# Alisah-Ozcan/HEonGPU

Hardware: AMD Instinct MI355X
Metric: homomorphic mults/sec (CKKS N=2^16, L=16) + NTT GB/s vs HBM roofline (higher is better)
Workload: dtype u64

## Files before the change

heongpu_amd/csrc/cabi.cpp:

```cpp
#include "../../include/hegpu.h"
#include "../../include/hegpu_bench.h"
#include "context.hpp"
#include "host_params.hpp"
#include "ops.hpp"
#include <cmath>
#include "tfhe.hpp"
#include <algorithm>
#include <cerrno>
#include <climits>
#include <mutex>
#include <unordered_map>
#include <vector>
#include <cstring>
#include <sys/random.h>
#include <new>
#include <stdexcept>
#include <string>

using namespace hegpu;

struct hegpu_context {
    Context c;
};

static thread_local std::string g_err;

static int fail(int code, const std::string& msg)
{
    g_err = msg;
    return code;
}

struct DevGuard {
    int prev = -1;
    bool switched = false;
    hipError_t err = hipSuccess;
    explicit DevGuard(int dev)
    {
        if (dev < 0) return;
        if ((err = hipGetDevice(&prev)) != hipSuccess) return;
        if (prev != dev) {
            err = hipSetDevice(dev);
            switched = err == hipSuccess;
        }
    }
    ~DevGuard()
    {
        if (switched) (void) hipSetDevice(prev);
    }
    DevGuard(const DevGuard&) = delete;
    DevGuard& operator=(const DevGuard&) = delete;
};
static int hip_ret(hipError_t e, const char* where)
{
    if (e == hipSuccess) return 0;
    g_err = std::string(where) + ": " + hipGetErrorString(e);
    return (int) e;
}

template <typename F>
static int guarded(F&& f)
{
    try {
        return f();
    } catch (const std::invalid_argument& e) {
        return fail(HEGPU_E_INVALID, e.what());
    } catch (const std::logic_error& e) {
        return fail(HEGPU_E_LOGIC, e.what());
    } catch (const std::runtime_error& e) {
        return fail(HEGPU_E_RUNTIME, e.what());
    } catch (const std::bad_alloc&) {
        return fail(HEGPU_E_RUNTIME, "out of host memory");
    }
}

extern "C" {

const char* hegpu_last_error(void) { return g_err.c_str(); }
const char* hegpu_version(void) { return "hegpu-mi355x 0.1 (gfx950)"; }

static bool coefficient_validator(const int* q, int qn, const int* p, int pn)
{
    int total_p = 0;
    for (int i = 0; i < pn; i++) total_p += p[i];
    int idx = 0;
    for (int g = 0; g < qn / pn; g++) {
        int s = 0;
        for (int j = 0; j < pn; j++) s += q[idx++];
        if (s > total_p) return false;
    }
    int s = 0;
    for (int j = 0; j < qn % pn; j++) s += q[idx++];
    return s <= total_p;
}

static void check_degree(int n, int& n_power)
{
    if (n <= 0 || (n & (n - 1))) throw std::logic_error("Poly modulus degree have to be power of two");
    if (n > 65536 || n < 4096) throw std::logic_error("Poly modulus degree is not supported");
    n_power = 31 - __builtin_clz((unsigned) n);
}

static int finish_create(hegpu_context* h, int scheme, int n_power, uint64_t plain_modulus, int q_count,
                         int p_count, hegpu_context** out)
{
    Context& c = h->c;
    c.scheme = scheme;
    c.n_power = n_power;
    c.Q_size = q_count;
    c.P_size = p_count;
    c.plain_modulus = plain_modulus;
    if (scheme == SCHEME_BFV && plain_modulus < 2) throw std::logic_error("plain modulus is not specified");
    c.build_host();
    c.seed_options_from_env();
    *out = h;
    return 0;
}

int hegpu_context_create(int scheme, int n, const int* qb, int qn, const int* pb, int pn, uint64_t plain_modulus,
                         int sec_level, hegpu_context** out)
{
    return guarded([&]() -> int {
        if (!out) throw std::invalid_argument("null output");
        if (scheme != SCHEME_BFV && scheme != SCHEME_CKKS) throw std::invalid_argument("unknown scheme");
        int n_power;
        check_degree(n, n_power);
        if (pn <= 0 || !pb) throw std::logic_error("log_P_bases_bit_sizes cannot be empty!");
        if (qn <= 0 || !qb) throw std::logic_error("log_Q_bases_bit_sizes cannot be empty!");
        if (!coefficient_validator(qb, qn, pb, pn)) throw std::logic_error("P should be bigger than Q pairs!");
        std::vector<int> bits(qb, qb + qn);
        bits.insert(bits.end(), pb, pb + pn);
        int total = 0;
        for (int b : bits) total += b;
        if (sec_level == HEGPU_SEC_128 || sec_level == HEGPU_SEC_192 || sec_level == HEGPU_SEC_256) {
            if (host::max_logq((u64) n, sec_level) < total)
                throw std::runtime_error("Parameters do not align with the security recommendations "
                                         "provided by the lattice-estimator");
        } else if (sec_level != HEGPU_SEC_NONE) {
            throw std::runtime_error("Invalid security level");
        }
        hegpu_context* h = new hegpu_context();
        try {
            h->c.primes = host::find_primes((u64) n, bits);
            return finish_create(h, scheme, n_power, plain_modulus, qn, pn, out);
        } catch (...) {
            delete h;
            throw;
        }
    });
}

int hegpu_context_create_default(int scheme, int n, int p_count, uint64_t plain_modulus, int sec_level,
                                 hegpu_context** out)
{
    return guarded([&]() -> int {
        if (!out) throw std::invalid_argument("null output");
        if (scheme != SCHEME_BFV && scheme != SCHEME_CKKS) throw std::invalid_argument("unknown scheme");
        int n_power;
        check_degree(n, n_power);
        if (p_count < 1) throw std::logic_error("P_modulus_size cannot be lower than 1!");
        if (sec_level != HEGPU_SEC_128 && sec_level != HEGPU_SEC_192 && sec_level != HEGPU_SEC_256)
            throw std::runtime_error("Invalid security level");
        std::vector<u64> chain = host::default_chain((u64) n, sec_level);
        if (chain.empty() || (int) chain.size() <= p_count) throw std::logic_error("no default chain");
        hegpu_context* h = new hegpu_context();
        try {
            h->c.primes = chain;
            return finish_create(h, scheme, n_power, plain_modulus, (int) chain.size() - p_count, p_count, out);
        } catch (...) {
            delete h;
            throw;
        }
    });
}

int hegpu_context_create_from_primes(int scheme, int n, const uint64_t* primes, int qn, int pn,
                                     uint64_t plain_modulus, hegpu_context** out)
{
    return guarded([&]() -> int {
        if (!out || !primes) throw std::invalid_argument("null argument");
        if (scheme != SCHEME_BFV && scheme != SCHEME_CKKS) throw std::invalid_argument("unknown scheme");
        int n_power;
        check_degree(n, n_power);
        if (pn <= 0 || qn <= 0) throw std::logic_error("log_P_bases_bit_sizes cannot be empty!");
        for (int i = 0; i < qn + pn; i++) {
            if (primes[i] >> 61) throw std::logic_error("invalid modulus bit size");
            if ((primes[i] - 1) % (2 * (u64) n)) throw std::logic_error("no sufficient root unity");
        }
        hegpu_context* h = new hegpu_context();
        try {
            h->c.primes.assign(primes, primes + qn + pn);
            return finish_create(h, scheme, n_power, plain_modulus, qn, pn, out);
        } catch (...) {
            delete h;
            throw;
        }
    });
}

int hegpu_validate_coeff_modulus_values(int n, const uint64_t* primes, int qn, int pn, int sec_level)
{
    return guarded([&]() -> int {
        if (!primes) throw std::invalid_argument("null argument");
        int n_power;
        check_degree(n, n_power);
        if (pn <= 0) throw std::logic_error("log_P_bases_bit_sizes cannot be empty!");
        if (qn <= 0) throw std::logic_error("log_Q_bases_bit_sizes cannot be empty!");
        std::vector<int> bits;
        int total = 0;
        for (int i = 0; i < qn + pn; i++) {
            if (primes[i] < 2 || primes[i] >> 61) throw std::logic_error("invalid modulus bit size");
            if ((primes[i] - 1) % (2 * (u64) n)) throw std::logic_error("no sufficient root unity");
            bits.push_back(64 - __builtin_clzll(primes[i]));
            total += bits.back();
        }
        if (!coefficient_validator(bits.data(), qn, bits.data() + qn, pn))
            throw std::logic_error("Invalid parameters, P should be bigger than Q pairs!");
        if (sec_level == HEGPU_SEC_128 || sec_level == HEGPU_SEC_192 || sec_level == HEGPU_SEC_256) {
            if (host::max_logq((u64) n, sec_level) < total)
                throw std::runtime_error("Parameters do not align with the security recommendations "
                                         "provided by the lattice-estimator");
        } else if (sec_level != HEGPU_SEC_NONE) {
            throw std::runtime_error("Invalid security level");
        }
        return 0;
    });
}

void hegpu_context_destroy(hegpu_context* ctx) { delete ctx; }

int hegpu_context_set_option(hegpu_context* ctx, const char* name, int value)
{
    if (!ctx || !name) return fail(HEGPU_E_INVALID, "null argument");
    switch (ctx->c.set_option(name, value)) {
        case 0: return 0;
        case 1: return fail(HEGPU_E_INVALID, std::string("unknown option: ") + name);
        case 2: return fail(HEGPU_E_INVALID, std::string("value out of range for option ") + name);
        default: return fail(HEGPU_E_LOGIC, std::string("option ") + name + " must be set before hegpu_context_upload");
    }
}

int hegpu_context_get_option(const hegpu_context* ctx, const char* name, int* value)
{
    if (!ctx || !name || !value) return fail(HEGPU_E_INVALID, "null argument");
    if (ctx->c.get_option(name, value)) return fail(HEGPU_E_INVALID, std::string("unknown option: ") + name);
    return 0;
}

int hegpu_context_upload(hegpu_context* ctx)
{
    if (!ctx) return fail(HEGPU_E_INVALID, "null context");
    int cnt = 0;
    if (hipGetDeviceCount(&cnt) != hipSuccess || cnt == 0) {
        (void) hipGetLastError();
        return fail(HEGPU_E_NODEVICE, "no HIP device available: the HIP backend cannot run (no CPU fallback)");
    }
    return hip_ret(ctx->c.upload(), "context upload");
}

int hegpu_context_upload_device(hegpu_context* ctx, int device)
{
    if (!ctx) return fail(HEGPU_E_INVALID, "null context");
    int cnt = 0;
    if (hipGetDeviceCount(&cnt) != hipSuccess || cnt == 0) {
        (void) hipGetLastError();
        return fail(HEGPU_E_NODEVICE, "no HIP device available: the HIP backend cannot run (no CPU fallback)");
    }
    if (device < 0 || device >= cnt) return fail(HEGPU_E_INVALID, "no such device");
    if (ctx->c.uploaded)
        return ctx->c.device == device ? 0 : fail(HEGPU_E_LOGIC, "the context is already uploaded to another device");
    DevGuard g(device);
    return hip_ret(ctx->c.upload(), "context upload");
}

int hegpu_context_device(const hegpu_context* ctx) { return (ctx && ctx->c.uploaded) ? ctx->c.device : -1; }

int hegpu_context_clone(const hegpu_context* src, hegpu_context** out)
{
    return guarded([&]() -> int {
        if (!src || !out) throw std::invalid_argument("null argument");
        hegpu_context* h = new hegpu_context();
        Context& c = h->c;
        const Context& s = src->c;
        c.scheme = s.scheme; c.n_power = s.n_power; c.n = s.n;
        c.Q_size = s.Q_size; c.P_size = s.P_size; c.Qp_size = s.Qp_size; c.bsk_size = s.bsk_size;
        c.plain_modulus = s.plain_modulus; c.primes = s.primes; c.host = s.host;
        c.m2_levels = s.m2_levels; c.m2_width = s.m2_width;
        c.fused_row_mac = s.fused_row_mac; c.fused_moddown = s.fused_moddown; c.col_multi = s.col_multi;
        c.single_pass = s.single_pass; c.ntt_galois = s.ntt_galois; c.galois_scatter = s.galois_scatter;
        c.digit_split = s.digit_split; c.copy_along = s.copy_along; c.fuse_inverse = s.fuse_inverse;
        c.fp_ntt = s.fp_ntt; c.behz_split = s.behz_split; c.fused_tensor = s.fused_tensor;
        *out = h;
        return 0;
    });
}

static thread_local int g_bcast_path = 0;
int hegpu_last_broadcast_path(void) { return g_bcast_path; }

static const size_t kBcastChunk = (size_t) 32 << 20;

static int peer_edge(int src, int dst, hipError_t* e)
{
    if (src == dst) return 1;
    int can = 0;
    if ((*e = hipDeviceCanAccessPeer(&can, dst, src)) != hipSuccess) return -1;
    if (!can) return 0;
    DevGuard g(dst);
    if (g.err != hipSuccess) {
        *e = g.err;
        return -1;
    }
    const hipError_t en = hipDeviceEnablePeerAccess(src, 0);
    if (en != hipSuccess && en != hipErrorPeerAccessAlreadyEnabled) {
        *e = en;
        return -1;
    }
    (void) hipGetLastError();
    return 1;
}

int hegpu_broadcast_bytes(const int* devices, int n, void* const* bufs, size_t bytes, const hegpu_stream* streams,
                          int* path_out)
{
    g_bcast_path = 0;
    if (path_out) *path_out = 0;
    if (!devices || !bufs || n < 1) return fail(HEGPU_E_INVALID, "null argument");
    int cnt = 0;
    if (hipGetDeviceCount(&cnt) != hipSuccess || cnt == 0) {
        (void) hipGetLastError();
        return fail(HEGPU_E_NODEVICE, "no HIP device available: the HIP backend cannot run (no CPU fallback)");
    }
    for (int i = 0; i < n; i++) {
        if (!bufs[i]) return fail(HEGPU_E_INVALID, "null buffer");
        if (devices[i] < 0 || devices[i] >= cnt) return fail(HEGPU_E_INVALID, "no such device");
    }
    if (n == 1 || bytes == 0) return 0;
    hipError_t e = hipSuccess;
    bool flat = true, same = true;
    for (int j = 1; j < n && flat; j++) {
        const int r = peer_edge(devices[0], devices[j], &e);
        if (r < 0) return hip_ret(e, "hegpu_broadcast: peer access");
        flat = r == 1;
    }
    for (int j = 1; j < n; j++) same = same && devices[j] == devices[0];
    std::vector<int> parent(n, 0);
    bool staged = false;
    if (!flat) {
        for (int span = 1; span < n; span <<= 1)
            for (int i = 0; i < span && i + span < n; i++) parent[i + span] = i;
        for (int j = 1; j < n; j++) {
            const int r = peer_edge(devices[parent[j]], devices[j], &e);
            if (r < 0) return hip_ret(e, "hegpu_broadcast: peer access");
            staged = staged || r == 0;
        }
    }
    const size_t nchunks = (bytes + kBcastChunk - 1) / kBcastChunk;
    auto stream_of = [&](int i) { return streams ? (hipStream_t) streams[i] : (hipStream_t) nullptr; };
    std::vector<hipEvent_t> events;
    auto mark = [&](int i, hipEvent_t* ev) {
        DevGuard g(devices[i]);
        if ((e = g.err) != hipSuccess) return;
        if ((e = hipEventCreateWithFlags(ev, hipEventDisableTiming)) != hipSuccess) return;
        events.push_back(*ev);
        e = hipEventRecord(*ev, stream_of(i));
    };
    std::vector<std::vector<hipEvent_t>> arrived(n, std::vector<hipEvent_t>(nchunks, nullptr));
    hipEvent_t src_ready = nullptr;
    mark(0, &src_ready);
    for (size_t c = 0; c < nchunks; c++) arrived[0][c] = src_ready;
    for (size_t c = 0; c < nchunks && e == hipSuccess; c++) {
        const size_t off = c * kBcastChunk, len = std::min(kBcastChunk, bytes - off);
        for (int j = 1; j < n && e == hipSuccess; j++) {
            const int pj = parent[j];
            DevGuard g(devices[j]);
            if ((e = g.err) != hipSuccess) break;
            if ((e = hipStreamWaitEvent(stream_of(j), arrived[pj][c], 0)) != hipSuccess) break;
            if ((e = hipMemcpyPeerAsync((char*) bufs[j] + off, devices[j], (const char*) bufs[pj] + off, devices[pj], len,
                                        stream_of(j))) != hipSuccess)
                break;
            bool has_child = false;
            for (int k = j + 1; k < n; k++) has_child = has_child || parent[k] == j;
            if (has_child) mark(j, &arrived[j][c]);
        }
    }
    for (hipEvent_t ev : events) (void) hipEventDestroy(ev);
    if (e != hipSuccess) return hip_ret(e, "hegpu_broadcast");
    int path = flat ? HEGPU_BCAST_FLAT : HEGPU_BCAST_TREE;
    if (staged) path |= HEGPU_BCAST_STAGED;
    if (same) path |= HEGPU_BCAST_SAME_DEVICE;
    g_bcast_path = path;
    if (path_out) *path_out = path;
    return 0;
}

int hegpu_broadcast_key(hegpu_context* const* ctxs, int n_ctx, uint64_t* const* keys, size_t elems,
                        const hegpu_stream* streams)
{
    g_bcast_path = 0;
    if (!ctxs || !keys || n_ctx < 1) return fail(HEGPU_E_INVALID, "null argument");
    std::vector<int> devs(n_ctx);
    std::vector<void*> bufs(n_ctx);
    for (int i = 0; i < n_ctx; i++) {
        if (!ctxs[i] || !keys[i]) return fail(HEGPU_E_INVALID, "null context or key pointer");
        if (!ctxs[i]->c.uploaded) return fail(HEGPU_E_LOGIC, "every context must be uploaded (hegpu_context_upload_device)");
        devs[i] = ctxs[i]->c.device;
        bufs[i] = keys[i];
    }
    return hegpu_broadcast_bytes(devs.data(), n_ctx, bufs.data(), elems * sizeof(u64), streams, nullptr);
}

long hegpu_context_int(const hegpu_context* ctx, const char* name)
{
    if (!ctx || !name) return -1;
    const Context& c = ctx->c;
    if (!strcmp(name, "n_power")) return c.n_power;
    if (!strcmp(name, "n")) return (long) c.n;
    if (!strcmp(name, "Q_size")) return c.Q_size;
    if (!strcmp(name, "P_size")) return c.P_size;
    if (!strcmp(name, "Q_prime_size")) return c.Qp_size;
    if (!strcmp(name, "bsk_modulus")) return c.bsk_size;
    if (!strcmp(name, "scheme")) return c.scheme;
    if (!strcmp(name, "max_logq_128")) return host::max_logq_128((int) c.n);
    if (!strcmp(name, "max_logq_192")) return host::max_logq(c.n, 192);
    if (!strcmp(name, "max_logq_256")) return host::max_logq(c.n, 256);
    return -1;
}

long hegpu_context_get(const hegpu_context* ctx, const char* name, uint64_t* out, long cap)
{
    if (!ctx || !name) return -1;
    auto it = ctx->c.host.find(name);
    if (it == ctx->c.host.end()) return -1;
    const long cnt = (long) it->second.size();
    if (!out) return cnt;
    if (cnt > cap) return -2;
    memcpy(out, it->second.data(), cnt * sizeof(uint64_t));
    return cnt;
}

const void* hegpu_context_device_ptr(const hegpu_context* ctx, const char* name)
{
    if (!ctx || !name) return nullptr;
    auto it = ctx->c.dev.find(name);
    return it == ctx->c.dev.end() ? nullptr : it->second;
}

int hegpu_steps_to_galois_elt(int steps, int coeff_count, int group_order)
{
    int elt = -1;
    (void) guarded([&]() -> int {
        elt = host::steps_to_galois_elt(steps, coeff_count, group_order);
        return 0;
    });
    return elt;
}

#define NEED_CTX(ctx)                                                                      \
    if (!(ctx)) return fail(HEGPU_E_INVALID, "null context");                              \
    if (!(ctx)->c.uploaded) {                                                              \
        int r__ = hegpu_context_upload(ctx);                                               \
        if (r__) return r__;                                                               \
    }                                                                                      \
    DevGuard dev_guard__((ctx)->c.device);                                                 \
    if (dev_guard__.err != hipSuccess) return hip_ret(dev_guard__.err, "switching to the context's device")

static const Mod* mods_of(const Context& c, int table_set)
{
    return table_set == HEGPU_TABLES_Q_BSK ? c.plan_merge.mods : c.plan_qp.mods;
}

int hegpu_ntt(hegpu_context* ctx, int table_set, const uint64_t* in, uint64_t* out, int inverse, int batch,
              int mod_count, int mod_offset, const int* mod_order, const int* poly_order, hegpu_stream stream)
{
    NEED_CTX(ctx);
    const Context& c = ctx->c;
    if (table_set == HEGPU_TABLES_Q_BSK && c.scheme != SCHEME_BFV)
        return fail(HEGPU_E_INVALID, "q|Bsk tables exist only in a BFV context");
    if (table_set < 0 || table_set > HEGPU_TABLES_PLAIN || (table_set == HEGPU_TABLES_PLAIN && !c.plan_plain.count))
        return fail(HEGPU_E_INVALID, "no such table set in this context");
    NttArgs a = c.ntt_args(table_set);
    const int avail = a.mod_count;
    if (mod_count <= 0 || mod_offset < 0 || (!mod_order && mod_offset + mod_count > avail))
        return fail(HEGPU_E_INVALID, "modulus range outside the table set");
    a.in = (const u64*) in;
    a.out = (u64*) out;
    a.mod_count = mod_count;
    a.mod_offset = mod_offset;
    a.mod_order = mod_order;
    a.poly_order = poly_order;
    return hip_ret(ntt_launch(a, batch, inverse != 0, (hipStream_t) stream), "hegpu_ntt");
}

int hegpu_GPU_NTT(hegpu_context* ctx, int table_set, const uint64_t* in, uint64_t* out, int mod_offset, int batch,
                  int mod_count, hegpu_stream stream)
{
    return hegpu_ntt(ctx, table_set, in, out, 0, batch, mod_count, mod_offset, nullptr, nullptr, stream);
}
int hegpu_GPU_NTT_Inplace(hegpu_context* ctx, int table_set, uint64_t* inout, int mod_offset, int batch, int mod_count,
                          hegpu_stream stream)
{
    return hegpu_ntt(ctx, table_set, inout, inout, 0, batch, mod_count, mod_offset, nullptr, nullptr, stream);
}
int hegpu_GPU_INTT(hegpu_context* ctx, int table_set, const uint64_t* in, uint64_t* out, int mod_offset, int batch,
                   int mod_count, hegpu_stream stream)
{
    return hegpu_ntt(ctx, table_set, in, out, 1, batch, mod_count, mod_offset, nullptr, nullptr, stream);
}
int hegpu_GPU_INTT_Inplace(hegpu_context* ctx, int table_set, uint64_t* inout, int mod_offset, int batch,
                           int mod_count, hegpu_stream stream)
{
    return hegpu_ntt(ctx, table_set, inout, inout, 1, batch, mod_count, mod_offset, nullptr, nullptr, stream);
}
int hegpu_GPU_NTT_Modulus_Ordered_Inplace(hegpu_context* ctx, int table_set, uint64_t* inout, int inverse,
                                          int mod_offset, int batch, int mod_count, const int* order,
                                          hegpu_stream stream)
{
    if (!order) return fail(HEGPU_E_INVALID, "modulus order table is required");
    return hegpu_ntt(ctx, table_set, inout, inout, inverse, batch, mod_count, mod_offset, order, nullptr, stream);
}
int hegpu_GPU_NTT_Poly_Ordered_Inplace(hegpu_context* ctx, int table_set, uint64_t* inout, int inverse, int mod_offset,
                                       int batch, int mod_count, const int* order, hegpu_stream stream)
{
    if (!order) return fail(HEGPU_E_INVALID, "polynomial order table is required");
    return hegpu_ntt(ctx, table_set, inout, inout, inverse, batch, mod_count, mod_offset, nullptr, order, stream);
}

int hegpu_addition(hegpu_context* ctx, const uint64_t* in1, const uint64_t* in2, uint64_t* out, int limbs,
                   int parts, int batch, int op, hegpu_stream stream)
{
    NEED_CTX(ctx);
    const Context& c = ctx->c;
    if (limbs <= 0 || limbs > c.Qp_size || op < 0 || op > 2) return fail(HEGPU_E_INVALID, "bad limbs/op");
    return hip_ret(rns_addition((const u64*) in1, (const u64*) in2, (u64*) out, c.plan_qp.mods, c.n_power, limbs,
                                parts, batch, op, (hipStream_t) stream),
                   "hegpu_addition");
}

int hegpu_cross_multiplication(hegpu_context* ctx, int table_set, const uint64_t* in1, uint64_t s1,
                               const uint64_t* in2, uint64_t s2, uint64_t* out, uint64_t so, int decomp_size,
                               int batch, hegpu_stream stream)
{
    NEED_CTX(ctx);
    const Context& c = ctx->c;
    const Mod* m = mods_of(c, table_set);
    if (!m) return fail(HEGPU_E_INVALID, "table set not available");
    return hip_ret(rns_cross_multiplication((const u64*) in1, s1, (const u64*) in2, s2, (u64*) out, so, m, c.n_power,
                                            decomp_size, batch, (hipStream_t) stream),
                   "hegpu_cross_multiplication");
}

int hegpu_cipher_broadcast(hegpu_context* ctx, const uint64_t* in, uint64_t in_stride, uint64_t* out,
                           uint64_t out_stride, int digits, int nmods, int split, int level, int batch,
                           hegpu_stream stream)
{
    NEED_CTX(ctx);
    const Context& c = ctx->c;
    return hip_ret(rns_decompose((const u64*) in, in_stride, (u64*) out, out_stride, c.plan_qp.mods, c.n_power,
                                 digits, nmods, split, level, batch, (hipStream_t) stream),
                   "hegpu_cipher_broadcast");
}

int hegpu_keyswitch_multiply_accumulate(hegpu_context* ctx, const uint64_t* in, uint64_t in_stride,
                                        const uint64_t* key, uint64_t* out, uint64_t out_stride, int digits,
                                        int nmods, int key_limbs, int split, int level, int batch,
                                        hegpu_stream stream)
{
    NEED_CTX(ctx);
    const Context& c = ctx->c;
    return hip_ret(rns_keyswitch_mac((const u64*) in, in_stride, (const u64*) key, (u64*) out, out_stride,
                                     c.plan_qp.mods, c.n_power, digits, nmods, key_limbs, split, level, batch,
                                     (hipStream_t) stream),
                   "hegpu_keyswitch_multiply_accumulate");
}

int hegpu_base_conversion_DtoQtilde(hegpu_context* ctx, const uint64_t* in, uint64_t in_stride, uint64_t* out,
                                    uint64_t out_stride, int depth, int batch, hegpu_stream stream)
{
    NEED_CTX(ctx);
    const Context& c = ctx->c;
    if (c.P_size < 2) return fail(HEGPU_E_LOGIC, "method II tables exist only when P_size > 1");
    if (depth < 0 || depth >= (int) c.m2_levels.size()) return fail(HEGPU_E_INVALID, "invalid depth");
    const Context::M2Level& L = c.m2_levels[depth];
    return hip_ret(rns_base_conversion_DtoQtilde((const u64*) in, in_stride, (u64*) out, out_stride, c.plan_qp.mods,
                                                 c.d64("m2_matrix_mg") + L.off_matrix, c.d64("m2_Mi_inv") + L.off_mi,
                                                 c.d64("m2_negprod_mg") + L.off_prod, c.d32("m2_I_j") + L.off_digits,
                                                 c.d32("m2_I_location") + L.off_digits, c.n_power, L.d, L.rc,
                                                 c.Q_size - depth, depth, c.m2_width, batch, (hipStream_t) stream),
                   "hegpu_base_conversion_DtoQtilde");
}

int hegpu_divide_round_lastq(hegpu_context* ctx, const uint64_t* in, uint64_t in_stride, const uint64_t* ct,
                             uint64_t ct_stride, uint64_t* out, uint64_t out_stride, int switchkey, int batch,
                             hegpu_stream stream)
// ... 1074 lines not shown
```

heongpu_amd/csrc/context.cpp:

```cpp
#include "context.hpp"
#include <cerrno>
#include <climits>
#include <cstdlib>
#include "host_params.hpp"
#include <algorithm>
#include <cmath>
#include <cstdlib>
#include <cstring>
#include <stdexcept>

namespace hegpu {

using host::inv_mod_prime;
using host::mul_mod;

typedef std::vector<u64> vec;

static void append(vec& dst, const vec& src) { dst.insert(dst.end(), src.begin(), src.end()); }

void Context::build_host()
{
    n = ((u64) 1) << n_power;
    Qp_size = Q_size + P_size;
    const int Q = Q_size, P = P_size, Qp = Qp_size;
// ... 386 lines not shown
                loc.push_back(brev((pos - 1) >> 1));
                pos = (pos * 3) & (m - 1);
            }
            for (u64 i = n / 2; i < n; i++) {
                loc.push_back(brev((m - pos - 1) >> 1));
                pos = (pos * 3) & (m - 1);
            }
            host["encoding_location"] = loc;
        }

        {
            u64 Q_mod_t = 1;
            for (int i = 0; i < Q; i++) Q_mod_t = mul_mod(Q_mod_t, primes[i] % t, t);
            host["Q_mod_t"] = vec{Q_mod_t};
            host["upper_threshold"] = vec{(t + 1) >> 1};
            vec inc;
            for (int i = 0; i < Q; i++) inc.push_back(primes[i] - t);
            host["upper_halfincrement"] = inc;
            std::vector<u64> big{1};
            for (int i = 0; i < Q; i++) {
                unsigned __int128 carry = 0;
                for (u64& w : big) {
                    unsigned __int128 v = (unsigned __int128) w * primes[i] + carry;
                    w = (u64) v;
                    carry = v >> 64;
                }
                if (carry) big.push_back((u64) carry);
            }
            {
                unsigned __int128 rem = 0;
                for (size_t k = big.size(); k-- > 0;) {
                    unsigned __int128 cur = (rem << 64) | big[k];
                    big[k] = (u64) (cur / t);
                    rem = cur % t;
                }
            }
            vec cdiv;
            for (int i = 0; i < Q; i++) {
                unsigned __int128 rem = 0;
                for (size_t k = big.size(); k-- > 0;) rem = ((rem << 64) | big[k]) % primes[i];
                cdiv.push_back((u64) rem);
            }
            host["coeff_div_plain_modulus"] = cdiv;
            vec Qi_t, Qi_gamma, Qi_inverse;
            for (int i = 0; i < Q; i++) {
                u64 a = 1, b = 1, c = 1;
                for (int j = 0; j < Q; j++)
                    if (j != i) {
                        a = mul_mod(a, primes[j] % t, t);
                        b = mul_mod(b, primes[j] % gamma, gamma);
                        c = mul_mod(c, inv_mod_prime(primes[j] % primes[i], primes[i]), primes[i]);
                    }
                Qi_t.push_back(a);
                Qi_gamma.push_back(b);
                Qi_inverse.push_back(c);
            }
            host["Qi_t"] = Qi_t;
            host["Qi_gamma"] = Qi_gamma;
            host["Qi_inverse"] = Qi_inverse;
            u64 mt_ = 1, mg_ = 1;
            for (int i = 0; i < Q; i++) {
                mt_ = mul_mod(mt_, inv_mod_prime(primes[i] % t, t), t);
                mg_ = mul_mod(mg_, inv_mod_prime(primes[i] % gamma, gamma), gamma);
            }
            host["mulq_inv_t"] = vec{t - mt_};
            host["mulq_inv_gamma"] = vec{gamma - mg_};
            host["inv_gamma"] = vec{inv_mod_prime(gamma % t, t)};
        }
    }
}

template <typename T>
static hipError_t to_device(const std::vector<T>& h, T** d)
{
    *d = nullptr;
    if (h.empty()) return hipSuccess;
    hipError_t e = hipMalloc((void**) d, h.size() * sizeof(T));
    if (e != hipSuccess) return e;
    return hipMemcpy(*d, h.data(), h.size() * sizeof(T), hipMemcpyHostToDevice);
}

static hipError_t build_plan(NttPlan& p, const vec& mods, const vec& fwd, const vec& inv, const vec& ninv,
                             int n_power, bool fp_on)
{
    const u64 n = ((u64) 1) << n_power;
    const int cnt = (int) mods.size();
    std::vector<Mod> hm(cnt);
    std::vector<ulonglong2> htw((size_t) cnt * n), hitw((size_t) cnt * n), hn(cnt), hw(cnt);
    const u64 rows = n / 256, perB = rows * 15 * 16;
    std::vector<ulonglong2> htwB((size_t) cnt * perB), hitwB((size_t) cnt * perB);
    std::vector<double> htwB8((size_t) cnt * perB, 0.0);
    for (int k = 0; k < cnt; k++) {
        const u64 q = mods[k];
        hm[k] = make_mod(q);
        static_assert(FP_MAX_MODULUS_BITS == 50, "the bounds in fpmod.cuh, ntt.hip and tests/fp_model.py are derived for q < 2^50");
        hm[k].fp = (fp_on && hm[k].bit <= FP_MAX_MODULUS_BITS && (q >> FP_MAX_MODULUS_BITS) == 0) ? 1 : 0;
        for (u64 j = 0; j < n; j++) {
            const u64 w = fwd[k * n + j], iw = inv[k * n + j];
            if (hm[k].fp) {
                const double wd = (double) w, wi = wd / (double) q;
                u64 a, b;
                memcpy(&a, &wd, 8);
                memcpy(&b, &wi, 8);
                htw[k * n + j] = make_ulonglong2(a, b);
            } else {
                htw[k * n + j] = make_ulonglong2(w, shoup_companion(w, q));
            }
            if (hm[k].fp) {
                const double wd = (double) iw, wi = wd / (double) q;
                u64 a, b;
                memcpy(&a, &wd, 8);
                memcpy(&b, &wi, 8);
                hitw[k * n + j] = make_ulonglong2(a, b);
            } else {
                hitw[k * n + j] = make_ulonglong2(iw, shoup_companion(iw, q));
            }
        }
        for (u64 c = 0; c < rows; c++)
            for (int st = 0; st < 4; st++)
                for (int b = 0; b < (1 << st); b++)
                    for (int j = 0; j < 16; j++) {
                        const u64 src = ((((rows + c) * 16 + j) << st) + b);
                        const u64 dst = k * perB + (c * 15 + ((1 << st) - 1 + b)) * 16 + j;
                        htwB[dst] = htw[k * n + src];
                        hitwB[dst] = hitw[k * n + src];
                        if (hm[k].fp) htwB8[dst] = (double) fwd[k * n + src];
                    }
        const u64 w1n = host::mul_mod(inv[k * n + 1], ninv[k], q);
        if (hm[k].fp) {
            auto pair = [&](u64 v) {
                const double vd = (double) v, vi = vd / (double) q;
                u64 a, b;
                memcpy(&a, &vd, 8);
                memcpy(&b, &vi, 8);
                return make_ulonglong2(a, b);
            };
            hn[k] = pair(ninv[k]);
            hw[k] = pair(w1n);
        } else {
            hn[k] = make_ulonglong2(ninv[k], shoup_companion(ninv[k], q));
            hw[k] = make_ulonglong2(w1n, shoup_companion(w1n, q));
        }
    }
    p.count = cnt;
    p.has_fp = p.has_int = 0;
    for (int k = 0; k < cnt; k++) (hm[k].fp ? p.has_fp : p.has_int) = 1;
    p.fp.assign(cnt, 0);
    for (int k = 0; k < cnt; k++) p.fp[k] = hm[k].fp ? 1 : 0;
    u64 qmax = 0;
    for (int k = 0; k < cnt; k++) qmax = mods[k] > qmax ? mods[k] : qmax;
    p.lazy_q_max = (~0ull - 2 * qmax) / (4ull * (u64) n_power);
    hipError_t e;
    if ((e = to_device(hm, &p.mods)) != hipSuccess) return e;
    if ((e = to_device(htw, &p.tw)) != hipSuccess) return e;
    if ((e = to_device(hitw, &p.itw)) != hipSuccess) return e;
    if ((e = to_device(htwB, &p.twB)) != hipSuccess) return e;
    if ((e = to_device(hitwB, &p.itwB)) != hipSuccess) return e;
    if ((e = to_device(htwB8, &p.twB8)) != hipSuccess) return e;
    if ((e = to_device(hn, &p.ninv)) != hipSuccess) return e;
    return to_device(hw, &p.w1ninv);
}

static void free_plan(NttPlan& p)
{
    if (p.mods) (void) hipFree(p.mods);
    if (p.tw) (void) hipFree(p.tw);
    if (p.itw) (void) hipFree(p.itw);
    if (p.twB) (void) hipFree(p.twB);
    if (p.itwB) (void) hipFree(p.itwB);
    if (p.twB8) (void) hipFree(p.twB8);
    if (p.ninv) (void) hipFree(p.ninv);
    if (p.w1ninv) (void) hipFree(p.w1ninv);
    p = NttPlan();
}

hipError_t Context::upload()
{
    if (uploaded) return hipSuccess;
    for (int k = 0; k < DRBG_GAUSS_MAX; k++)
        gauss_cdt.t[k] = (u64) (erf(((double) k + 0.5) / (3.2 * 1.4142135623730951)) * 9223372036854775808.0);
    hipError_t e = hipGetDevice(&device);
    if (e != hipSuccess) return e;
    if ((e = build_plan(plan_qp, host["modulus"], host["ntt_table"], host["intt_table"], host["n_inverse"],
                        n_power, fp_ntt)) != hipSuccess)
        return e;
    static const char* u64_tables[] = {"psi_half",
                                       "last_q_modinv",
                                       "half",
                                       "half_mod",
                                       "factor",
                                       "m2_md_W0",
                                       "m2_md_G",
                                       "m2_md_C",
                                       "rescaled_last_q_modinv",
                                       "rescaled_half_mod",
                                       "rescaled_half",
                                       "base_change_matrix_Bsk",
                                       "inv_punctured_prod_mod_base_array",
                                       "base_change_matrix_m_tilde",
                                       "inv_m_tilde_mod_Bsk",
                                       "prod_q_mod_Bsk",
                                       "inv_prod_q_mod_Bsk",
                                       "base_change_matrix_q",
                                       "base_change_matrix_msk",
                                       "inv_punctured_prod_mod_B_array",
                                       "behz_mtilde_inv_punct",
                                       "behz_t_inv_punct",
                                       "behz_invq_inv_punct_B",
                                       "behz_msk_mod_q",
                                       "behz_fc_matrix",
                                       "behz_fc_c1",
                                       "behz_ff_matrix",
                                       "behz_ff_tc",
                                       "behz_ff_q_matrix",
                                       "behz_ff_msk_matrix",
                                       "behz_ff_prod_B",
                                       "behz_ff_neg_prod_B",
                                       "prod_B_mod_q",
                                       "Mi",
                                       "Mi_inv",
                                       "upper_half_threshold",
                                       "decryption_modulus",
                                       "special_fft_roots_table",
                                       "special_ifft_roots_table",
                                       "coeff_div_plain_modulus",
                                       "upper_halfincrement",
                                       "Qi_t",
                                       "Qi_gamma",
                                       "Qi_inverse",
                                       "m2_Mi_inv",
                                       "m2_matrix",
                                       "m2_prod",
                                       "m2_matrix_mg",
                                       "m2_negprod_mg"};
    for (const char* nm : u64_tables) {
        auto it = host.find(nm);
        if (it == host.end()) continue;
        u64* d = nullptr;
        if ((e = to_device(it->second, &d)) != hipSuccess) return e;
        dev[nm] = d;
    }
    for (const char* nm : {"new_prime_locations", "new_input_locations", "m2_I_j", "m2_I_location", "encoding_location",
                           "reverse_order"}) {
        auto it = host.find(nm);
        if (it == host.end()) continue;
        std::vector<int> v(it->second.begin(), it->second.end());
        int* d = nullptr;
        if ((e = to_device(v, &d)) != hipSuccess) return e;
        dev[nm] = d;
    }
    if (scheme == SCHEME_BFV) {
        if ((e = build_plan(plan_merge, host["q_Bsk_merge_modulus"], host["q_Bsk_merge_ntt_tables"],
                            host["q_Bsk_merge_intt_tables"], host["q_Bsk_n_inverse"], n_power, fp_ntt)) != hipSuccess)
            return e;
        if (host.count("plain_modulus2") &&
            (e = build_plan(plan_plain, host["plain_modulus2"], host["plain_ntt_tables"], host["plain_intt_tables"],
                            host["n_plain_inverse"], n_power, fp_ntt)) != hipSuccess)
            return e;
        behz.ibase = plan_merge.mods;
        behz.obase = plan_merge.mods + Q_size;
        behz.m_tilde = make_mod(((u64) 1) << 32);
        behz.plain = make_mod(plain_modulus);
        behz.inv_prod_q_mod_m_tilde = host["inv_prod_q_mod_m_tilde"][0];
        behz.inv_prod_B_mod_m_sk = host["inv_prod_B_mod_m_sk"][0];
        behz.inv_m_tilde_mod_Bsk = d64("inv_m_tilde_mod_Bsk");
        behz.prod_q_mod_Bsk = d64("prod_q_mod_Bsk");
        behz.base_change_matrix_Bsk = d64("base_change_matrix_Bsk");
        behz.base_change_matrix_m_tilde = d64("base_change_matrix_m_tilde");
        behz.inv_punctured_prod_mod_base_array = d64("inv_punctured_prod_mod_base_array");
        behz.inv_prod_q_mod_Bsk = d64("inv_prod_q_mod_Bsk");
        behz.inv_punctured_prod_mod_B_array = d64("inv_punctured_prod_mod_B_array");
        behz.base_change_matrix_q = d64("base_change_matrix_q");
        behz.base_change_matrix_msk = d64("base_change_matrix_msk");
        behz.prod_B_mod_q = d64("prod_B_mod_q");
        behz.mtilde_inv_punct = d64("behz_mtilde_inv_punct");
        behz.t_inv_punct = d64("behz_t_inv_punct");
        behz.invq_inv_punct_B = d64("behz_invq_inv_punct_B");
        behz.msk_mod_q = d64("behz_msk_mod_q");
        behz.fc_matrix = d64("behz_fc_matrix");
        behz.fc_c1 = d64("behz_fc_c1");
        behz.ff_matrix = d64("behz_ff_matrix");
        behz.ff_tc = d64("behz_ff_tc");
        behz.ff_q_matrix = d64("behz_ff_q_matrix");
        behz.ff_msk_matrix = d64("behz_ff_msk_matrix");
        behz.ff_prod_B = d64("behz_ff_prod_B");
        behz.ff_neg_prod_B = d64("behz_ff_neg_prod_B");
        behz.ibase_size = Q_size;
        behz.obase_size = bsk_size;
        behz.split = behz_split;
    }
    uploaded = true;
    return hipDeviceSynchronize();
}

namespace {
struct OptDesc { const char* name; const char* env; int lo, hi; };
const OptDesc kOptions[] = {
    {"fused_row_mac", "HEGPU_FUSED_ROW_MAC", -1, 1}, {"fused_moddown", "HEGPU_FUSED_MODDOWN", 0, 1},
    {"col_multi", "HEGPU_COL_MULTI", -1, 1},         {"single_pass", "HEGPU_SINGLE_PASS", -1, 1},
    {"ntt_galois", "HEGPU_NTT_GALOIS", 0, 1},        {"galois_scatter", "HEGPU_GALOIS_SCATTER", 0, 1},
    {"fuse_inverse", "HEGPU_FUSE_INVERSE", 0, 1},    {"copy_along", "HEGPU_COPY_ALONG", 0, 1},
    {"digit_split", "HEGPU_DIGIT_SPLIT", -1, 4},     {"fp_ntt", "HEGPU_FP_NTT", 0, 1},
    {"behz_split", "HEGPU_BEHZ_SPLIT", -1, 1},       {"fused_tensor", "HEGPU_FUSED_TENSOR", 0, 1},
};
}

int Context::set_option(const char* name, int value)
{
    if (!name) return 1;
    const OptDesc* d = nullptr;
    for (const OptDesc& o : kOptions)
        if (!strcmp(o.name, name)) d = &o;
    if (!d) return 1;
    if (value < d->lo || value > d->hi) return 2;
    const std::string nm(name);
    if (nm == "fp_ntt") {
        if (uploaded) return 3;
        fp_ntt = value != 0;
    } else if (nm == "fused_row_mac") fused_row_mac = value;
    else if (nm == "fused_moddown") fused_moddown = value != 0;
    else if (nm == "col_multi") col_multi = value;
    else if (nm == "single_pass") single_pass = value;
    else if (nm == "ntt_galois") ntt_galois = value != 0;
    else if (nm == "galois_scatter") galois_scatter = value != 0;
    else if (nm == "fuse_inverse") fuse_inverse = value != 0;
    else if (nm == "copy_along") copy_along = value != 0;
    else if (nm == "fused_tensor") fused_tensor = value != 0;
    else if (nm == "digit_split") {
        if (value == 1 || value == 3) return 2;
        digit_split = value;
    } else if (nm == "behz_split") {
        behz_split = value;
        behz.split = value;
    }
    return 0;
}

int Context::get_option(const char* name, int* value) const
{
    if (!name || !value) return 1;
    const std::string nm(name);
    if (nm == "fp_ntt") *value = fp_ntt;
    else if (nm == "fused_row_mac") *value = fused_row_mac;
    else if (nm == "fused_moddown") *value = fused_moddown;
    else if (nm == "col_multi") *value = col_multi;
    else if (nm == "single_pass") *value = single_pass;
    else if (nm == "ntt_galois") *value = ntt_galois;
    else if (nm == "galois_scatter") *value = galois_scatter;
    else if (nm == "fuse_inverse") *value = fuse_inverse;
    else if (nm == "copy_along") *value = copy_along;
    else if (nm == "fused_tensor") *value = fused_tensor;
    else if (nm == "digit_split") *value = digit_split;
    else if (nm == "behz_split") *value = behz_split;
    else return 1;
    return 0;
}

bool env_long(const char* name, long* out)
{
    const char* e = getenv(name);
    if (!e || !*e) return false;
    char* end = nullptr;
    errno = 0;
    const long v = strtol(e, &end, 10);
    if (errno || end == e || *end) return false;
    *out = v;
    return true;
}

void Context::seed_options_from_env()
{
    for (const OptDesc& o : kOptions) {
        long v;
        if (env_long(o.env, &v) && v >= INT_MIN && v <= INT_MAX)
            (void) set_option(o.name, (int) v);
    }
}

void Context::release_device()
{
    free_plan(plan_qp);
    free_plan(plan_merge);
    free_plan(plan_plain);
    for (auto& kv : dev)
        if (kv.second) (void) hipFree(kv.second);
    dev.clear();
    uploaded = false;
}

Context::~Context()
{
    if (uploaded) release_device();
}

const u64* Context::d64(const char* name) const
{
    auto it = dev.find(name);
    return it == dev.end() ? nullptr : (const u64*) it->second;
}
const int* Context::d32(const char* name) const
{
    auto it = dev.find(name);
    return it == dev.end() ? nullptr : (const int*) it->second;
}

NttArgs Context::ntt_args(int table_set) const
{
    const NttPlan& p = table_set == 2 ? plan_plain : (table_set ? plan_merge : plan_qp);
    NttArgs a{};
    a.mods = p.mods;
    a.tw = p.tw;
    a.itw = p.itw;
    a.twB = p.twB;
    a.itwB = p.itwB;
    a.twB8 = p.twB8;
    a.ninv = p.ninv;
    a.w1ninv = p.w1ninv;
    a.n_power = n_power;
    a.mod_count = p.count;
    a.col_multi = col_multi;
    a.single_pass = single_pass;
    a.plan_has_fp = p.has_fp;
    a.plan_has_int = p.has_int;
    a.lazy_q_max = p.lazy_q_max;
    return a;
}

}
```

heongpu_amd/csrc/context.hpp:

```cpp
#pragma once
#include "modarith.cuh"
#include "ntt.hpp"
#include "rns.hpp"
#include <map>
#include <string>
#include "drbg.hpp"
#include <vector>

namespace hegpu {

bool env_long(const char* name, long* out);


enum Scheme { SCHEME_BFV = 1, SCHEME_CKKS = 2 };

struct NttPlan {
    Mod* mods = nullptr;
    ulonglong2* tw = nullptr;
    ulonglong2* itw = nullptr;
    ulonglong2* twB = nullptr;
    ulonglong2* itwB = nullptr;
    double* twB8 = nullptr;
    ulonglong2* ninv = nullptr;
    ulonglong2* w1ninv = nullptr;
    int count = 0;
    int has_fp = 0, has_int = 0;
    std::vector<unsigned char> fp;
    u64 lazy_q_max = 0;
};

struct Context {
    int scheme = 0;
    int n_power = 0;
    u64 n = 0;
    int Q_size = 0, P_size = 0, Qp_size = 0;
    int bsk_size = 0;
    u64 plain_modulus = 0;
    std::vector<u64> primes;
    std::map<std::string, std::vector<u64>> host;
    struct M2Level {
        int d = 0, rc = 0;
        int off_digits = 0;
        int off_mi = 0;
        int off_matrix = 0;
        int off_prod = 0;
    };
    std::vector<M2Level> m2_levels;
    int m2_width = 0;
    int fused_row_mac = -1;
    bool fused_moddown = true;
    int col_multi = -1;
    int single_pass = -1;
    bool ntt_galois = true;
    bool galois_scatter = true;
    int digit_split = -1;
    bool copy_along = true;
    bool fuse_inverse = true;
    bool fused_tensor = true;
    bool fp_ntt = true;
    int behz_split = -1;
    void seed_options_from_env();
    int set_option(const char* name, int value);
    int get_option(const char* name, int* value) const;
    GaussCdt gauss_cdt{};

    bool uploaded = false;
    int device = -1;
    NttPlan plan_qp;
    NttPlan plan_merge;
    NttPlan plan_plain;
    std::map<std::string, void*> dev;
    Mod* bsk_mods = nullptr;
    BehzDev behz{};

    ~Context();
    void build_host();
    hipError_t upload();
    void release_device();

    const u64* d64(const char* name) const;
    const std::vector<u64>& h64(const char* name) const { return host.at(name); }
    const int* d32(const char* name) const;
    NttArgs ntt_args(int table_set) const;
};

}
```

heongpu_amd/csrc/ntt.hip:

```cpp
#include "ntt.hpp"
#define HEGPU_FP_TU ntt
#include "fpmod.cuh"

namespace hegpu {

#define NTT_THREADS 256

#ifdef NTT_ABLATION_HEADER
#include NTT_ABLATION_HEADER
#else
__device__ __forceinline__ u64 gld(const u64* p) { return *p; }
__device__ __forceinline__ void gst(u64* p, u64 v) { *p = v; }
#define NTT_ABLATE_BFLY(x, y, w)
#define NTT_ABLATE_FPBFLY(x, y, w)
#define NTT_ABLATE_TW(load, root0, s) (load)
#define NTT_FP_TW(t, i, c) ((t)[i])
#endif

__device__ __forceinline__ u64 csub(u64 x, u64 m) { return (x >= m) ? x - m : x; }

typedef unsigned long long u64x2_t __attribute__((ext_vector_type(2)));
struct ConstTw {
    const u64x2_t __attribute__((address_space(4)))* p;
    __device__ __forceinline__ ulonglong2 operator[](u32 i) const
// ... 15 lines not shown
#pragma clang diagnostic push
#pragma clang diagnostic ignored "-Wold-style-cast"
    return *(const int __attribute__((address_space(4)))*) p;
#pragma clang diagnostic pop
}
__device__ __forceinline__ Mod ld_const_mod(const Mod* p)
{
#pragma clang diagnostic push
#pragma clang diagnostic ignored "-Wold-style-cast"
    const u64 __attribute__((address_space(4)))* w = (const u64 __attribute__((address_space(4)))*) reinterpret_cast<const u64*>(p);
#pragma clang diagnostic pop
    static_assert(sizeof(Mod) == 56, "seven words");
    Mod m;
    m.q = w[0];
    m.mu = w[1];
    m.r_hi = w[2];
    m.r_lo = w[3];
    m.r64 = w[4];
    m.qinv = w[5];
    const u64 bf = w[6];
    m.bit = (u32) bf;
    m.fp = (u32) (bf >> 32);
    return m;
}

__device__ __forceinline__ void fp_ct_bfly(double& x, double& y, ulonglong2 w, const FC& c)
{
    NTT_ABLATE_FPBFLY(x, y, w);
    const double t = fp_mul(y, as_f64(w.x), as_f64(w.y), c);
    y = x - t;
    x = x + t;
    FP_AUDIT_VAL(c, FPM_SUM, x);
    FP_AUDIT_VAL(c, FPM_SUM, y);
}
struct FpSched { unsigned before; bool at_end; };
#define FP_STAGE_GROW(b) (1.25 * (b) + 0.5)
#define FP_BOUND_LIMIT 7.9
#define FP_HANDOVER 0.51
#define FP_UNREDUCED_IN 1.05
constexpr FpSched fp_sched(int stages, double b_in, double b_out_max)
{
    unsigned m = 0;
    double b = b_in;
    for (int s = 0; s < stages; s++) {
        if (FP_STAGE_GROW(b) > FP_BOUND_LIMIT) {
            m |= 1u << s;
            b = 0.5;
        }
        b = FP_STAGE_GROW(b);
    }
    return FpSched{m, b > b_out_max};
}
template <int LOGR, typename TW>
__device__ __forceinline__ void fp_ct_radix(double (&x)[1 << LOGR], TW tw, u32 root0,
                                            const FC& c, unsigned before, bool at_end)
{
#pragma unroll
    for (int s = 0; s < LOGR; s++) {
        FP_STAGE(c, 31 - __builtin_clz(root0) + s);
        if ((before >> s) & 1u) {
#pragma unroll
            for (int k = 0; k < (1 << LOGR); k++) x[k] = fp_reduce(x[k], c);
        }
        const int half = (1 << LOGR) >> (s + 1);
#pragma unroll
        for (int b = 0; b < (1 << s); b++) {
            const ulonglong2 w = NTT_ABLATE_TW(NTT_FP_TW(tw, (root0 << s) + b, c), root0, s);
#pragma unroll
            for (int j = 0; j < half; j++) fp_ct_bfly(x[b * 2 * half + j], x[b * 2 * half + j + half], w, c);
        }
    }
    FP_STAGE(c, 31 - __builtin_clz(root0) + LOGR);
    if (at_end) {
#pragma unroll
        for (int k = 0; k < (1 << LOGR); k++) x[k] = fp_reduce(x[k], c);
    }
}
template <int S1> struct FpColSched {
    static constexpr FpSched s = fp_sched(S1, FP_UNREDUCED_IN, FP_HANDOVER);
    static constexpr unsigned a_before = s.before & ((1u << (S1 - 4)) - 1u);
    static constexpr unsigned b_before = (s.before >> (S1 - 4)) & 15u;
    static constexpr bool b_at_end = s.at_end;
};
__device__ __forceinline__ void fp_ct_radix16_tb(double (&x)[16], const ulonglong2* __restrict__ tb, const FC& c)
{
#pragma unroll
    for (int s = 0; s < 4; s++) {
        const int half = 8 >> s;
        if (s > 0) FP_STAGE(c, (c).stage + 1);
#pragma unroll
        for (int b = 0; b < (1 << s); b++) {
            const ulonglong2 w = NTT_ABLATE_TW(NTT_FP_TW(tb, ((1 << s) - 1 + b) * 16, c), (u32) b, s);
#pragma unroll
            for (int j = 0; j < half; j++) fp_ct_bfly(x[b * 2 * half + j], x[b * 2 * half + j + half], w, c);
        }
    }
    FP_STAGE(c, (c).stage + 1);
#pragma unroll
    for (int k = 0; k < 16; k++) x[k] = fp_canon(x[k], c);
}

__device__ __forceinline__ void fp_ct_radix16_tb8(double (&x)[16], const double* __restrict__ tb, const FC& c)
{
#pragma unroll
    for (int s = 0; s < 4; s++) {
        const int half = 8 >> s;
        if (s > 0) __builtin_amdgcn_sched_barrier(0);
        if (s > 0) FP_STAGE(c, (c).stage + 1);
#pragma unroll
        for (int b = 0; b < (1 << s); b++) {
            const double wd = tb[((1 << s) - 1 + b) * 16];
            const ulonglong2 w = make_ulonglong2(as_bits(wd), as_bits(wd * c.qi));
#pragma unroll
            for (int j = 0; j < half; j++) fp_ct_bfly(x[b * 2 * half + j], x[b * 2 * half + j + half], w, c);
        }
    }
    FP_STAGE(c, (c).stage + 1);
#pragma unroll
    for (int k = 0; k < 16; k++) x[k] = fp_canon(x[k], c);
}

struct QC {
    u64 q;
    u64 q4;
    u32 nq0, nq1;
};
__device__ __forceinline__ QC make_qc(u64 q)
{
    QC c;
    c.q = q;
    c.q4 = 4 * q;
    u64 nq = 0 - q;
    c.nq0 = (u32) nq;
    c.nq1 = (u32) (nq >> 32);
    return c;
}

__device__ __forceinline__ u64 shoup_lazy(u64 y, ulonglong2 w, const QC& c)
{
    const u32 y0 = (u32) y, y1 = (u32) (y >> 32);
    const u32 w0 = (u32) w.x, w1 = (u32) (w.x >> 32), p0 = (u32) w.y, p1 = (u32) (w.y >> 32);
    const u64 A = (u64) y0 * p1;
    const u64 B = (u64) y1 * p0 + (u32) A;
    const u64 qh = (u64) y1 * p1 + (A >> 32) + (B >> 32);
    const u32 h0 = (u32) qh, h1 = (u32) (qh >> 32);
    u64 acc = (u64) y0 * w0;
    acc += (u64) h0 * c.nq0;
    const u32 hi = y0 * w1 + y1 * w0 + h0 * c.nq1 + h1 * c.nq0;
    return acc + ((u64) hi << 32);
}

__device__ __forceinline__ u64 shoup_full(u64 y, ulonglong2 w, const QC& c)
{
    u64 r = shoup_lazy(y, w, c);
    r = csub(r, 2 * c.q);
    return csub(r, c.q);
}

template <bool LAZY>
__device__ __forceinline__ void ct_bfly(u64& x, u64& y, ulonglong2 w, const QC& c)
{
    NTT_ABLATE_BFLY(x, y, w);
    u64 u = LAZY ? x : csub(x, c.q4);
    u64 t = shoup_lazy(y, w, c);
    x = u + t;
    y = u + c.q4 - t;
}

__device__ __forceinline__ void gs_bfly(u64& x, u64& y, ulonglong2 w, const QC& c)
{
    NTT_ABLATE_BFLY(x, y, w);
    u64 s = x + y;
    u64 d = x + c.q4 - y;
    x = csub(s, c.q4);
    y = shoup_lazy(d, w, c);
}

template <int LOGR, bool LAZY, typename TW>
__device__ __forceinline__ void ct_radix(u64 (&x)[1 << LOGR], TW tw,
                                         u32 root0, const QC& c)
{
#pragma unroll
    for (int s = 0; s < LOGR; s++) {
        const int half = (1 << LOGR) >> (s + 1);
#pragma unroll
        for (int b = 0; b < (1 << s); b++) {
            ulonglong2 w = NTT_ABLATE_TW(tw[(root0 << s) + b], root0, s);
#pragma unroll
            for (int j = 0; j < half; j++)
                ct_bfly<LAZY>(x[b * 2 * half + j], x[b * 2 * half + j + half], w, c);
        }
    }
}

template <bool LAZY>
__device__ __forceinline__ void ct_radix16_tb(u64 (&x)[16], const ulonglong2* __restrict__ tb, const QC& c)
{
#pragma unroll
    for (int s = 0; s < 4; s++) {
        const int half = 8 >> s;
#pragma unroll
        for (int b = 0; b < (1 << s); b++) {
            ulonglong2 w = tb[((1 << s) - 1 + b) * 16];
#pragma unroll
            for (int j = 0; j < half; j++)
                ct_bfly<LAZY>(x[b * 2 * half + j], x[b * 2 * half + j + half], w, c);
        }
    }
}

template <int LOGR>
__device__ __forceinline__ void gs_radix(u64 (&x)[1 << LOGR], const ulonglong2* __restrict__ tw,
                                         u32 root0, const QC& c)
{
#pragma unroll
    for (int s = LOGR - 1; s >= 0; s--) {
        const int half = (1 << LOGR) >> (s + 1);
#pragma unroll
        for (int b = 0; b < (1 << s); b++) {
            ulonglong2 w = NTT_ABLATE_TW(tw[(root0 << s) + b], root0, s);
#pragma unroll
            for (int j = 0; j < half; j++)
                gs_bfly(x[b * 2 * half + j], x[b * 2 * half + j + half], w, c);
        }
    }
}

__device__ __forceinline__ void gs_radix16_tb(u64 (&x)[16], const ulonglong2* __restrict__ tb, const QC& c)
{
#pragma unroll
    for (int s = 3; s >= 0; s--) {
        const int half = 8 >> s;
#pragma unroll
        for (int b = 0; b < (1 << s); b++) {
            ulonglong2 w = tb[((1 << s) - 1 + b) * 16];
#pragma unroll
            for (int j = 0; j < half; j++)
                gs_bfly(x[b * 2 * half + j], x[b * 2 * half + j + half], w, c);
        }
    }
}

template <int LOGR>
__device__ __forceinline__ void gs_radix_last(u64 (&x)[1 << LOGR], const ulonglong2* __restrict__ tw,
                                              u32 root0, ulonglong2 ninv, ulonglong2 w1ninv, const QC& c)
{
#pragma unroll
    for (int s = LOGR - 1; s >= 1; s--) {
        const int half = (1 << LOGR) >> (s + 1);
#pragma unroll
        for (int b = 0; b < (1 << s); b++) {
            ulonglong2 w = NTT_ABLATE_TW(tw[(root0 << s) + b], root0, s);
#pragma unroll
            for (int j = 0; j < half; j++)
                gs_bfly(x[b * 2 * half + j], x[b * 2 * half + j + half], w, c);
        }
    }
    const int half = (1 << LOGR) >> 1;
#pragma unroll
    for (int j = 0; j < half; j++) {
        u64 s = x[j] + x[j + half];
        u64 d = x[j] + c.q4 - x[j + half];
        x[j] = shoup_full(s, ninv, c);
        x[j + half] = shoup_full(d, w1ninv, c);
    }
}

struct PolySel {
    u64 in_off, out_off;
    int mod;
    int digit;
    int item, j;
};

__device__ __forceinline__ int udiv16(int x, unsigned magic)
{
    return magic ? (int) __umulhi((unsigned) x, magic) : x;
}

__device__ __forceinline__ PolySel select_poly(const NttArgs& a, int poly)
{
    PolySel s;
    if (a.group_span) {
        const int k = udiv16(poly, a.mg_group_span), r = poly - k * a.group_span;
        if (a.polys_per_item) {
            const int per_item = udiv16(a.polys_per_item, a.mg_mod_count);
            const int it = udiv16(r, a.mg_per_item), d = r - it * per_item;
            poly = it * a.polys_per_item + d * a.mod_count + k;
        } else {
            poly = r * a.mod_count + k;
        }
    }
    int item = 0, j = poly;
    if (a.polys_per_item) {
        item = udiv16(poly, a.mg_polys_per_item);
        j = poly - item * a.polys_per_item;
    }
    int k = j - udiv16(j, a.mg_mod_count) * a.mod_count;
    if (a.mod_order) k = a.mod_order[k];
    s.mod = a.mod_offset + k;
    u64 slot = a.poly_order ? (u64) a.poly_order[j] : (u64) j;
    s.digit = a.decomp_mods ? udiv16(j, a.mg_decomp_mods) : -1;
    u64 in_slot = a.decomp_mods ? (u64) s.digit * (a.decomp_in_mul ? a.decomp_in_mul : 1) + a.decomp_in_add : slot;
    s.in_off = (u64) item * a.in_item_stride + (in_slot << a.n_power);
    s.out_off = (u64) item * a.out_item_stride + (slot << a.n_power);
    s.item = item;
    s.j = j;
    return s;
}

__device__ __forceinline__ int col_phys(int e) { return e ^ (((e >> 8) & 1) << 4); }
__device__ __forceinline__ int row_phys(int e) { return e ^ (((e >> 5) & 7) << 1); }

__device__ __forceinline__ void wave_lds_fence()
{
    __builtin_amdgcn_fence(__ATOMIC_RELEASE, "wavefront");
    __builtin_amdgcn_wave_barrier();
    __builtin_amdgcn_fence(__ATOMIC_ACQUIRE, "wavefront");
}

#define COL_LDS_ELEMS 4096
#define ROW_LDS_ELEMS 4096

__device__ __forceinline__ bool fwd_stages_lazy(const Mod& md, u64 lazy_q_max) { return md.q <= lazy_q_max; }
#define NTT_ROW_LAZY_MAX_Q 0x0666666666666666ull
__device__ __forceinline__ bool row_stages_lazy(const Mod& md, u64 lazy_q_max) { return md.q <= lazy_q_max || md.q <= NTT_ROW_LAZY_MAX_Q; }

template <int S1, bool DECOMP, bool LAZY, bool SREG = false>
__device__ __forceinline__ void fwd_col_body(const NttArgs& a, const PolySel& ps, const Mod& md, u64* lds,
                                             const u64* sreg = nullptr)
{
    constexpr int R = 1 << S1;
    constexpr int CT = 4096 / R;
    constexpr int NSA = S1 - 4;
    constexpr int RA = 1 << NSA;
    constexpr int G = 16 / RA;
    const int t = threadIdx.x;
    const QC qc = make_qc(md.q);
    const ulonglong2* __restrict__ tw = a.tw + ((u64) ps.mod << a.n_power);
    const u64* __restrict__ src = a.in + ps.in_off + blockIdx.x * CT;
    u64* __restrict__ dst = a.out + ps.out_off + blockIdx.x * CT;

    const u64 half_qP = a.half_on ? a.mods[a.half_src_mod].q : 0;
    const u64 half_hm = a.half_on ? a.half_mod[ps.mod] : 0;
    u64 x[16];
    const int col = t % CT, r1 = t / CT;
    u64 v[16];
    if constexpr (NSA > 0) {
#pragma unroll
        for (int g = 0; g < G; g++) {
            const int L = t + NTT_THREADS * g;
            const int c = L % CT, rb = L / CT;
#pragma unroll
            for (int k = 0; k < RA; k++) v[g * RA + k] = SREG ? sreg[g * RA + k] : gld(&src[(u64) (rb + 16 * k) * 256 + c]);
        }
    } else {
#pragma unroll
        for (int k = 0; k < 16; k++) v[k] = SREG ? sreg[k] : gld(&src[(u64) k * 256 + col]);
    }
    if (DECOMP && a.half_on) {
#pragma unroll
        for (int k = 0; k < 16; k++) v[k] = sub_mod(reduce64(add_mod(v[k], a.half, half_qP), md), half_hm, md.q);
    } else if (DECOMP && !LAZY && a.mods[ps.digit].q > 8 * md.q) {
#pragma unroll
        for (int k = 0; k < 16; k++) v[k] = reduce64(v[k], md);
    }
    if constexpr (NSA > 0) {
#pragma unroll
        for (int g = 0; g < G; g++) {
            const int L = t + NTT_THREADS * g;
            const int c = L % CT, rb = L / CT;
            u64 y[RA];
#pragma unroll
            for (int k = 0; k < RA; k++) y[k] = v[g * RA + k];
            ct_radix<NSA, LAZY>(y, tw, 1u, qc);
#pragma unroll
            for (int k = 0; k < RA; k++) lds[col_phys((rb + 16 * k) * CT + c)] = y[k];
        }
        __syncthreads();
#pragma unroll
        for (int k = 0; k < 16; k++) x[k] = lds[col_phys((16 * r1 + k) * CT + col)];
        if (SREG) __syncthreads();
    } else {
#pragma unroll
        for (int k = 0; k < 16; k++) x[k] = v[k];
    }
    ct_radix<4, LAZY>(x, tw, (u32) (RA + r1), qc);
#pragma unroll
    for (int k = 0; k < 16; k++) gst(&dst[(u64) (16 * r1 + k) * 256 + col], x[k]);
}

template <int S1, bool DECOMP, bool WIDE, bool SREG = false>
__device__ __forceinline__ void fwd_col_body_fp(const NttArgs& a, const PolySel& ps, const Mod& md, u64* lds,
                                                ulonglong2* twl, const u64* sreg = nullptr)
{
    constexpr int R = 1 << S1;
    constexpr int CT = 4096 / R;
    constexpr int NSA = S1 - 4;
    constexpr int RA = 1 << NSA;
    constexpr int G = 16 / RA;
    const int t = threadIdx.x;
    const FC fc = make_fc(md.q, FP_SITE(DECOMP ? FPS_FWD_COL_DECOMP : FPS_FWD_COL, S1 - 4));
    const ulonglong2* __restrict__ tw = a.tw + ((u64) ps.mod << a.n_power);
    const u64* __restrict__ src = a.in + ps.in_off + blockIdx.x * CT;
    u64* __restrict__ dst = a.out + ps.out_off + blockIdx.x * CT;

    double c32 = 0.0, c32i = 0.0;
    if constexpr (DECOMP && WIDE) {
        c32 = (double) reduce64(1ull << 32, md);
        c32i = c32 * fc.qi;
    }
    const u64 half_qP = (DECOMP && a.half_on) ? a.mods[a.half_src_mod].q : 0;
    const double half_hm = (DECOMP && a.half_on) ? fp_from_u64(a.half_mod[ps.mod]) : 0.0;
    const bool in_small = S1 != 7 && DECOMP && !WIDE && !a.half_on && a.mods[ps.digit].q <= md.q + (md.q >> 6);
    typedef FpColSched<S1> CS;
    auto load_all = [&](auto& y, auto addr, int si0) {
        constexpr int CNT = sizeof(y) / sizeof(y[0]);
        FP_STAGE(fc, FP_STAGE_INPUT);
        if constexpr (SREG && !WIDE) {
            if (in_small) {
#pragma unroll
                for (int k = 0; k < CNT; k++) y[k] = as_f64(sreg[si0 + k]);
            } else {
#pragma unroll
                for (int k = 0; k < CNT; k++) y[k] = fp_reduce(as_f64(sreg[si0 + k]), fc);
            }
        } else {
            u64 v[CNT];
#pragma unroll
            for (int k = 0; k < CNT; k++) {
                v[k] = SREG ? sreg[si0 + k] : *addr(k);
                if constexpr (SREG) asm volatile("" : "+v"(v[k]));
            }
            if (!SREG && DECOMP && a.half_on) {
#pragma unroll
                for (int k = 0; k < CNT; k++) v[k] = add_mod(v[k], a.half, half_qP);
            }
#pragma unroll
            for (int k = 0; k < CNT; k++) {
                if constexpr (DECOMP && WIDE) y[k] = fp_mul(fp_from_u32((u32) (v[k] >> 32)), c32, c32i, fc) + fp_from_u32((u32) v[k]);
                else if constexpr (DECOMP) y[k] = in_small ? fp_from_u64(v[k]) : fp_reduce(fp_from_u64(v[k]), fc);
                else y[k] = fp_from_u64(v[k]);
            }
        }
        if (DECOMP && a.half_on) {
#pragma unroll
            for (int k = 0; k < CNT; k++) y[k] = fp_reduce(y[k] - half_hm, fc);
        }
#pragma unroll
        for (int k = 0; k < CNT; k++) FP_AUDIT_VAL(fc, FPM_SUM, y[k]);
    };

    double x[16];
    const int col = t % CT, r1 = t / CT;
    if constexpr (NSA > 0) {
        const ulonglong2 mine = tw[t];
#pragma unroll
        for (int g = 0; g < G; g++) {
            const int L = t + NTT_THREADS * g;
            const int c = L % CT, rb = L / CT;
            double y[RA];
            load_all(y, [&](int k) { return &src[(u64) (rb + 16 * k) * 256 + c]; }, g * RA);
            if constexpr (SREG) fp_ct_radix<NSA>(y, const_tw(tw), 1u, fc, CS::a_before, false);
            else fp_ct_radix<NSA>(y, tw, 1u, fc, CS::a_before, false);
#pragma unroll
            for (int k = 0; k < RA; k++) lds[col_phys((rb + 16 * k) * CT + c)] = as_bits(y[k]);
        }
        twl[t] = mine;
        __syncthreads();
#pragma unroll
        for (int k = 0; k < 16; k++) x[k] = as_f64(lds[col_phys((16 * r1 + k) * CT + col)]);
        if (SREG) __syncthreads();
        fp_ct_radix<4>(x, twl, (u32) (RA + r1), fc, CS::b_before, CS::b_at_end);
    } else {
        load_all(x, [&](int k) { return &src[(u64) k * 256 + col]; }, 0);
        fp_ct_radix<4>(x, tw, (u32) (RA + r1), fc, CS::b_before, CS::b_at_end);
    }
#pragma unroll
    for (int k = 0; k < 16; k++) {
        if constexpr (SREG) __builtin_nontemporal_store(as_bits(x[k]), &dst[(u64) (16 * r1 + k) * 256 + col]);
        else dst[(u64) (16 * r1 + k) * 256 + col] = as_bits(x[k]);
    }
}

template <int S1, bool DECOMP>
__global__ __launch_bounds__(NTT_THREADS) void ntt_fwd_col(NttArgs a)
{
    __shared__ u64 lds[(S1 > 4) ? COL_LDS_ELEMS : 1];
    __shared__ ulonglong2 twl[(S1 > 4) ? 256 : 1];
    int poly = blockIdx.y;
    if (DECOMP && a.only_int && a.int_slot_count > 0) {
        const int cnt = a.int_slot_count, digits = a.polys_per_item / a.decomp_mods;
        const int per_item = digits * cnt;
        const int item = poly / per_item, r = poly - item * per_item;
        const int digit = r / cnt, w = r - digit * cnt;
        poly = item * a.polys_per_item + digit * a.decomp_mods + a.int_slots[w];
    }
    const PolySel ps = select_poly(a, poly);
    if (DECOMP && a.skip_identity && ps.mod == ps.digit) return;
    const Mod md = a.mods[ps.mod];
    if (DECOMP && a.only_int && md.fp) return;
    if (DECOMP && a.copy_src) {
        constexpr int CT = 4096 >> S1;
        const int t = threadIdx.x, col = t % CT, r1 = t / CT;
        const u64 limb = ((u64) (ps.digit * a.copy_part_limbs + (ps.j - ps.digit * a.decomp_mods)) << a.n_power) +
                         blockIdx.x * CT;
        const u64* __restrict__ cs = a.copy_src + (u64) ps.item * a.copy_src_item_stride + limb;
        u64* __restrict__ cd = a.copy_dst + (u64) ps.item * a.copy_dst_item_stride + limb;
        u64 c[16];
#pragma unroll
        for (int k = 0; k < 16; k++) c[k] = cs[(u64) (16 * r1 + k) * 256 + col];
#pragma unroll
        for (int k = 0; k < 16; k++) cd[(u64) (16 * r1 + k) * 256 + col] = c[k];
    }
    if (md.fp) {
        if (DECOMP && a.mods[a.half_on ? a.half_src_mod : ps.digit].bit > 52)
            fwd_col_body_fp<S1, DECOMP, true>(a, ps, md, lds, twl);
        else fwd_col_body_fp<S1, DECOMP, false>(a, ps, md, lds, twl);
    } else if (fwd_stages_lazy(md, a.lazy_q_max)) fwd_col_body<S1, DECOMP, true>(a, ps, md, lds);
    else fwd_col_body<S1, DECOMP, false>(a, ps, md, lds);
}

__device__ __forceinline__ void row_store_all(const NttArgs& a, const PolySel& ps, const Mod& md, u64* __restrict__ p,
                                              u64 e0, const u64* lds, int row, int i0)
{
    if (!a.epi.on) {
#pragma unroll
        for (int k = 0; k < 16; k++) gst(&p[e0 + 16 * k], lds[row_phys(row * 256 + i0 + 16 * k)]);
        return;
    }
    const NttEpilogue& ep = a.epi;
    const int part = udiv16(ps.j, ep.mg_limbs), limb = ps.j - part * ep.limbs;
    const u64* __restrict__ ks = ep.ks + ep.ks_item_stride * ps.item + ((u64) (part * ep.ks_part_limbs + limb) << a.n_power) + e0;
    const u64 off = ((u64) (part * ep.limbs + limb) << a.n_power);
    const bool with_ct = ep.ct && (!ep.ct_parts || part < ep.ct_parts);
    const u64* ct = with_ct ? ep.ct + ep.ct_item_stride * ps.item + off + e0 : nullptr;
    u64* out = ep.out + ep.out_item_stride * ps.item + off;
    const u64 inv = ep.inv[ps.mod];
#pragma unroll
    for (int h = 0; h < 2; h++) {
        u64 kv[8], cv[8];
#pragma unroll
        for (int k = 0; k < 8; k++) kv[k] = ks[16 * (8 * h + k)];
        if (with_ct) {
#pragma unroll
            for (int k = 0; k < 8; k++) cv[k] = ct[16 * (8 * h + k)];
        }
        u64 r[8];
#pragma unroll
        for (int k = 0; k < 8; k++)
            r[k] = mul_barrett(sub_mod(kv[k], lds[row_phys(row * 256 + i0 + 16 * (8 * h + k))], md.q), inv, md);
        if (with_ct) {
#pragma unroll
            for (int k = 0; k < 8; k++) r[k] = add_mod(cv[k], r[k], md.q);
        }
        if (ep.galois_inv) {
#pragma unroll
            for (int k = 0; k < 8; k++) {
                const u32 e = (u32) e0 + 16 * (8 * h + k);
                const u32 ex = ((2u * (__brev(e) >> (32 - a.n_power)) + 1u) * ep.galois_inv) & ((2u << a.n_power) - 1u);
                out[__brev((ex - 1u) >> 1) >> (32 - a.n_power)] = r[k];
            }
        } else {
#pragma unroll
            for (int k = 0; k < 8; k++) out[e0 + 16 * (8 * h + k)] = r[k];
        }
    }
}

template <bool LAZY>
__device__ __forceinline__ void fwd_row_body(const NttArgs& a, const PolySel& ps, const Mod& md, u64* lds)
{
    const int t = threadIdx.x;
    const QC qc = make_qc(md.q);
    const int s1 = a.n_power - 8;
    const ulonglong2* __restrict__ tw = a.tw + ((u64) ps.mod << a.n_power);
    u64* __restrict__ p = a.out + ps.out_off + (u64) blockIdx.x * 4096;

    const int row = t >> 4, i0 = t & 15;
    const u32 crow = blockIdx.x * 16 + row;
    u64 x[16];
#pragma unroll
    for (int k = 0; k < 16; k++) x[k] = gld(&p[row * 256 + i0 + 16 * k]);
    ct_radix<4, LAZY>(x, tw, (1u << s1) + crow, qc);
#pragma unroll
    for (int k = 0; k < 16; k++) lds[row_phys(row * 256 + i0 + 16 * k)] = x[k];
    wave_lds_fence();
#pragma unroll
    for (int k = 0; k < 8; k++) {
        ulonglong2 v = *reinterpret_cast<const ulonglong2*>(&lds[row_phys(row * 256 + 16 * i0 + 2 * k)]);
        x[2 * k] = v.x;
        x[2 * k + 1] = v.y;
    }
    ct_radix16_tb<LAZY>(x, a.twB + ((u64) ps.mod * (15u << (a.n_power - 4))) + ((u64) crow * 15 * 16 + i0), qc);
    if (LAZY) {
#pragma unroll
        for (int k = 0; k < 16; k++) x[k] = reduce64(x[k], md);
    } else {
#pragma unroll
        for (int k = 0; k < 16; k++) x[k] = csub(csub(csub(x[k], qc.q4), 2 * qc.q), qc.q);
    }
    wave_lds_fence();
#pragma unroll
    for (int k = 0; k < 8; k++)
        *reinterpret_cast<ulonglong2*>(&lds[row_phys(row * 256 + 16 * i0 + 2 * k)]) =
            make_ulonglong2(x[2 * k], x[2 * k + 1]);
    wave_lds_fence();
    row_store_all(a, ps, md, a.out + ps.out_off, (u64) blockIdx.x * 4096 + row * 256 + i0, lds, row, i0);
}

__device__ __forceinline__ void fwd_row_body_fp(const NttArgs& a, const PolySel& ps, const Mod& md, u64* lds)
{
    const int t = threadIdx.x;
    const FC fc = make_fc(md.q, FP_SITE(FPS_FWD_ROW, a.n_power - 12));
    const int s1 = a.n_power - 8;
    const ulonglong2* __restrict__ tw = a.tw + ((u64) ps.mod << a.n_power);
    u64* __restrict__ p = a.out + ps.out_off + (u64) blockIdx.x * 4096;

    const int row = t >> 4, i0 = t & 15;
    const u32 crow = blockIdx.x * 16 + row;
    double x[16];
#pragma unroll
    for (int k = 0; k < 16; k++) x[k] = as_f64(p[row * 256 + i0 + 16 * k]);
    fp_ct_radix<4>(x, tw, (1u << s1) + crow, fc, 0u, true);
#pragma unroll
    for (int k = 0; k < 16; k++) lds[row_phys(row * 256 + i0 + 16 * k)] = as_bits(x[k]);
    wave_lds_fence();
#pragma unroll
    for (int k = 0; k < 8; k++) {
        ulonglong2 v = *reinterpret_cast<const ulonglong2*>(&lds[row_phys(row * 256 + 16 * i0 + 2 * k)]);
        x[2 * k] = as_f64(v.x);
        x[2 * k + 1] = as_f64(v.y);
    }
    fp_ct_radix16_tb8(x, a.twB8 + ((u64) ps.mod * (15u << (a.n_power - 4))) + ((u64) crow * 15 * 16 + i0), fc);
    wave_lds_fence();
#pragma unroll
    for (int k = 0; k < 8; k++)
        *reinterpret_cast<ulonglong2*>(&lds[row_phys(row * 256 + 16 * i0 + 2 * k)]) =
            make_ulonglong2(fp_to_u64(x[2 * k]), fp_to_u64(x[2 * k + 1]));
    wave_lds_fence();
    row_store_all(a, ps, md, a.out + ps.out_off, (u64) blockIdx.x * 4096 + row * 256 + i0, lds, row, i0);
}

__global__ __launch_bounds__(NTT_THREADS) void ntt_fwd_row(NttArgs a)
{
    __shared__ __attribute__((aligned(16))) u64 lds[ROW_LDS_ELEMS];
    const PolySel ps = select_poly(a, blockIdx.y);
    if (a.skip_identity && ps.mod == ps.digit) return;
    const Mod md = a.mods[ps.mod];
    if (md.fp) fwd_row_body_fp(a, ps, md, lds);
    else if (row_stages_lazy(md, a.lazy_q_max)) fwd_row_body<true>(a, ps, md, lds);
    else fwd_row_body<false>(a, ps, md, lds);
}

template <int S1>
__device__ __forceinline__ int single_pos(int row, int col)
{
    return (row >> 4) * 4096 + row_phys((row & 15) * 256 + col);
}

template <int S1, bool FP, bool LAZY, bool DECOMP = false>
__device__ __forceinline__ void fwd_single_body(const NttArgs& a, const PolySel& ps, const Mod& md, u64* limb)
{
    constexpr int R = 1 << S1;
    constexpr int CT = 4096 / R;
    constexpr int NSA = S1 - 4;
    constexpr int RA = 1 << NSA;
    constexpr int G = 16 / RA;
    const int t = threadIdx.x, g = t >> 8, tt = t & 255;
    const QC qc = make_qc(md.q);
    const FC fc = make_fc(md.q, FP_SITE(FPS_FWD_SINGLE, S1 - 4));
    const ulonglong2* __restrict__ tw = a.tw + ((u64) ps.mod << a.n_power);
    const u64* __restrict__ src = a.in + ps.in_off + g * CT;
    const int col = tt % CT, r1 = tt / CT;
    u64 dv[DECOMP ? 16 : 1];
    double dy[(DECOMP && FP) ? 16 : 1];
    if constexpr (DECOMP) {
        if constexpr (NSA > 0) {
#pragma unroll
            for (int gi = 0; gi < G; gi++) {
                const int L = tt + 256 * gi;
                const int c = L % CT, rb = L / CT;
#pragma unroll
                for (int k = 0; k < RA; k++) dv[gi * RA + k] = src[(u64) (rb + 16 * k) * 256 + c];
            }
        } else {
#pragma unroll
            for (int k = 0; k < 16; k++) dv[k] = src[(u64) k * 256 + col];
        }
        const u64 half_qP = a.half_on ? a.mods[a.half_src_mod].q : 0;
        if constexpr (FP) {
            FP_STAGE(fc, FP_STAGE_INPUT);
            if (a.half_on) {
#pragma unroll
                for (int k = 0; k < 16; k++) dv[k] = add_mod(dv[k], a.half, half_qP);
            }
            if (a.mods[a.half_on ? a.half_src_mod : ps.digit].bit > 52) {
                const double c32 = (double) reduce64(1ull << 32, md), c32i = c32 * fc.qi;
#pragma unroll
                for (int k = 0; k < 16; k++)
                    dy[k] = fp_mul(fp_from_u32((u32) (dv[k] >> 32)), c32, c32i, fc) + fp_from_u32((u32) dv[k]);
            } else {
#pragma unroll
                for (int k = 0; k < 16; k++) dy[k] = fp_reduce(fp_from_u64(dv[k]), fc);
            }
            if (a.half_on) {
                const double half_hm = fp_from_u64(a.half_mod[ps.mod]);
#pragma unroll
                for (int k = 0; k < 16; k++) dy[k] = fp_reduce(dy[k] - half_hm, fc);
            }
#pragma unroll
            for (int k = 0; k < 16; k++) FP_AUDIT_VAL(fc, FPM_SUM, dy[k]);
        } else {
            if (a.half_on) {
                const u64 half_hm = a.half_mod[ps.mod];
#pragma unroll
                for (int k = 0; k < 16; k++) dv[k] = sub_mod(reduce64(add_mod(dv[k], a.half, half_qP), md), half_hm, md.q);
            } else if (!LAZY && a.mods[ps.digit].q > 8 * md.q) {
#pragma unroll
                for (int k = 0; k < 16; k++) dv[k] = reduce64(dv[k], md);
            }
        }
    }
    if constexpr (FP) {
        double x[16];
        if constexpr (NSA > 0) {
#pragma unroll
            for (int gi = 0; gi < G; gi++) {
                const int L = tt + 256 * gi;
                const int c = L % CT, rb = L / CT;
                double y[RA];
#pragma unroll
                for (int k = 0; k < RA; k++) {
                    if constexpr (DECOMP) y[k] = dy[gi * RA + k];
                    else y[k] = fp_from_u64(gld(&src[(u64) (rb + 16 * k) * 256 + c]));
                }
                fp_ct_radix<NSA>(y, tw, 1u, fc, FpColSched<S1>::a_before, false);
#pragma unroll
                for (int k = 0; k < RA; k++) limb[single_pos<S1>(rb + 16 * k, g * CT + c)] = as_bits(y[k]);
            }
            __syncthreads();
#pragma unroll
            for (int k = 0; k < 16; k++) x[k] = as_f64(limb[single_pos<S1>(16 * r1 + k, g * CT + col)]);
        } else {
#pragma unroll
            for (int k = 0; k < 16; k++) {
                if constexpr (DECOMP) x[k] = dy[k];
                else x[k] = fp_from_u64(src[(u64) k * 256 + col]);
            }
        }
        fp_ct_radix<4>(x, tw, (u32) (RA + r1), fc, FpColSched<S1>::b_before, FpColSched<S1>::b_at_end);
#pragma unroll
        for (int k = 0; k < 16; k++) limb[single_pos<S1>(16 * r1 + k, g * CT + col)] = as_bits(x[k]);
    } else {
        u64 x[16];
        if constexpr (NSA > 0) {
#pragma unroll
            for (int gi = 0; gi < G; gi++) {
                const int L = tt + 256 * gi;
                const int c = L % CT, rb = L / CT;
                u64 y[RA];
#pragma unroll
                for (int k = 0; k < RA; k++) {
                    if constexpr (DECOMP) y[k] = dv[gi * RA + k];
                    else y[k] = gld(&src[(u64) (rb + 16 * k) * 256 + c]);
                }
                ct_radix<NSA, LAZY>(y, tw, 1u, qc);
#pragma unroll
                for (int k = 0; k < RA; k++) limb[single_pos<S1>(rb + 16 * k, g * CT + c)] = y[k];
            }
            __syncthreads();
#pragma unroll
            for (int k = 0; k < 16; k++) x[k] = limb[single_pos<S1>(16 * r1 + k, g * CT + col)];
        } else {
#pragma unroll
            for (int k = 0; k < 16; k++) {
                if constexpr (DECOMP) x[k] = dv[k];
                else x[k] = src[(u64) k * 256 + col];
            }
        }
        ct_radix<4, LAZY>(x, tw, (u32) (RA + r1), qc);
#pragma unroll
        for (int k = 0; k < 16; k++) limb[single_pos<S1>(16 * r1 + k, g * CT + col)] = x[k];
    }
    __syncthreads();
    u64* lds = limb + g * 4096;
    const int row = tt >> 4, i0 = tt & 15;
    const u32 crow = g * 16 + row;
    const ulonglong2* __restrict__ tb = a.twB + ((u64) ps.mod * (15u << (a.n_power - 4))) + ((u64) crow * 15 * 16 + i0);
    u64 r[16];
    if constexpr (FP) {
        double x[16];
#pragma unroll
        for (int k = 0; k < 16; k++) x[k] = as_f64(lds[row_phys(row * 256 + i0 + 16 * k)]);
        fp_ct_radix<4>(x, tw, (1u << S1) + crow, fc, 0u, true);
#pragma unroll
        for (int k = 0; k < 16; k++) lds[row_phys(row * 256 + i0 + 16 * k)] = as_bits(x[k]);
        wave_lds_fence();
#pragma unroll
        for (int k = 0; k < 8; k++) {
            ulonglong2 v = *reinterpret_cast<const ulonglong2*>(&lds[row_phys(row * 256 + 16 * i0 + 2 * k)]);
            x[2 * k] = as_f64(v.x);
            x[2 * k + 1] = as_f64(v.y);
        }
        fp_ct_radix16_tb8(x, a.twB8 + ((u64) ps.mod * (15u << (a.n_power - 4))) + ((u64) crow * 15 * 16 + i0), fc);
#pragma unroll
        for (int k = 0; k < 16; k++) r[k] = fp_to_u64(x[k]);
    } else {
        u64 x[16];
#pragma unroll
        for (int k = 0; k < 16; k++) x[k] = lds[row_phys(row * 256 + i0 + 16 * k)];
        ct_radix<4, LAZY>(x, tw, (1u << S1) + crow, qc);
#pragma unroll
        for (int k = 0; k < 16; k++) lds[row_phys(row * 256 + i0 + 16 * k)] = x[k];
        wave_lds_fence();
#pragma unroll
        for (int k = 0; k < 8; k++) {
            ulonglong2 v = *reinterpret_cast<const ulonglong2*>(&lds[row_phys(row * 256 + 16 * i0 + 2 * k)]);
            x[2 * k] = v.x;
            x[2 * k + 1] = v.y;
        }
        ct_radix16_tb<LAZY>(x, tb, qc);
        if (LAZY) {
#pragma unroll
            for (int k = 0; k < 16; k++) r[k] = reduce64(x[k], md);
        } else {
#pragma unroll
            for (int k = 0; k < 16; k++) r[k] = csub(csub(csub(x[k], qc.q4), 2 * qc.q), qc.q);
        }
    }
    wave_lds_fence();
#pragma unroll
    for (int k = 0; k < 8; k++)
        *reinterpret_cast<ulonglong2*>(&lds[row_phys(row * 256 + 16 * i0 + 2 * k)]) = make_ulonglong2(r[2 * k], r[2 * k + 1]);
    wave_lds_fence();
    row_store_all(a, ps, md, a.out + ps.out_off, (u64) g * 4096 + row * 256 + i0, lds, row, i0);
}

template <int S1, bool DECOMP = false>
__global__ __launch_bounds__(16 << S1, 4) void ntt_fwd_single(NttArgs a)
{
    extern __shared__ __attribute__((aligned(16))) u64 limb[];
    const PolySel ps = select_poly(a, blockIdx.x);
    if (DECOMP && a.skip_identity && ps.mod == ps.digit) return;
    const Mod md = a.mods[ps.mod];
    if (md.fp) fwd_single_body<S1, true, false, DECOMP>(a, ps, md, limb);
    else if (fwd_stages_lazy(md, a.lazy_q_max)) fwd_single_body<S1, false, true, DECOMP>(a, ps, md, limb);
    else fwd_single_body<S1, false, false, DECOMP>(a, ps, md, limb);
}

__device__ __forceinline__ void acc128(u64& hi, u64& lo, u64 a, u64 b)
{
    u64 h, l;
    mul64wide(a, b, h, l);
    lo += l;
    hi += h + (lo < l);
}

template <bool LAZY>
__device__ __forceinline__ void ks_row_digit(u64 (&x)[16], const u64* __restrict__ p, u64* lds,
                                             const ulonglong2* twa, const ulonglong2* __restrict__ tb,
                                             const QC& qc, const Mod& md, int row, int i0)
{
#pragma unroll
    for (int k = 0; k < 16; k++) x[k] = gld(&p[row * 256 + i0 + 16 * k]);
#pragma unroll
    for (int s = 0; s < 4; s++) {
        const int half = 8 >> s;
#pragma unroll
        for (int b = 0; b < (1 << s); b++) {
            const ulonglong2 w = twa[((1 << s) - 1 + b) * 16 + row];
#pragma unroll
            for (int j = 0; j < half; j++) ct_bfly<LAZY>(x[b * 2 * half + j], x[b * 2 * half + j + half], w, qc);
        }
    }
#pragma unroll
    for (int k = 0; k < 16; k++) lds[row_phys(row * 256 + i0 + 16 * k)] = x[k];
    wave_lds_fence();
#pragma unroll
    for (int k = 0; k < 8; k++) {
        ulonglong2 v = *reinterpret_cast<const ulonglong2*>(&lds[row_phys(row * 256 + 16 * i0 + 2 * k)]);
        x[2 * k] = v.x;
        x[2 * k + 1] = v.y;
    }
    ct_radix16_tb<LAZY>(x, tb, qc);
    if (!LAZY) {
#pragma unroll
        for (int k = 0; k < 16; k++) x[k] = csub(csub(csub(x[k], qc.q4), 2 * qc.q), qc.q);
    }
    wave_lds_fence();
#pragma unroll
    for (int k = 0; k < 8; k++)
        *reinterpret_cast<ulonglong2*>(&lds[row_phys(row * 256 + 16 * i0 + 2 * k)]) =
            make_ulonglong2(x[2 * k], x[2 * k + 1]);
    wave_lds_fence();
#pragma unroll
    for (int k = 0; k < 16; k++) x[k] = lds[row_phys(row * 256 + i0 + 16 * k)];
    wave_lds_fence();
}

struct KsIdx { int item, tile, slot; bool valid; int d0, d1; };
__host__ __device__ __forceinline__ unsigned ks_slots(const KsMacArgs& a, int kind)
{
    if (a.int_slot_count <= 0 || kind == 0) return (unsigned) a.rc;
    return kind == 1 ? (unsigned) a.int_slot_count : (unsigned) (a.rc - a.int_slot_count);
}
template <bool SPLIT, int KIND = 0>
__device__ __forceinline__ KsIdx ks_index(const KsMacArgs& a)
{
    const unsigned b = blockIdx.x, xcd = b & 7u, j = b >> 3;
    const unsigned splits = SPLIT ? (unsigned) a.splits : 1u;
    const unsigned units = (unsigned) a.items * splits;
    const unsigned tiles = 1u << (a.n_power - 12);
    const unsigned total = ks_slots(a, KIND) * tiles * units, chunk = (total + 7u) >> 3;
    const unsigned lin = xcd * chunk + j;
    const unsigned g = lin / units, unit = lin - g * units;
    const unsigned item = SPLIT ? unit / splits : unit, sp = SPLIT ? unit - item * splits : 0u;
    const unsigned nslots = ks_slots(a, KIND), gt = g / nslots;
    KsIdx r;
    r.valid = lin < total;
    r.item = (int) item;
    r.tile = (int) gt;
    int si = (int) (g - gt * nslots);
    if (KIND == 1 && a.int_slot_count > 0) {
        si = a.int_slots[r.valid ? si : 0];
    } else if (KIND == 2 && a.int_slot_count > 0) {
#pragma unroll
        for (int q = 0; q < 8; q++)
            if (q < a.int_slot_count && a.int_slots[q] <= si) si++;
    }
    r.slot = si;
    r.d0 = SPLIT ? (int) (sp * (unsigned) a.digits / splits) : 0;
    r.d1 = SPLIT ? (int) ((sp + 1) * (unsigned) a.digits / splits) : a.digits;
    return r;
}

#define KS_TW_LDS_BYTES ((15 * 256 + 15 * 16) * 8)
template <bool SPLIT>
__device__ __forceinline__ void ks_row_mac_int_body(const KsMacArgs& a, const KsIdx& ki, const Mod& md, int midx,
                                                    u64* lds, void* twbuf)
{
    const int t = threadIdx.x;
    const int item = ki.item, tile = ki.tile, slot = ki.slot;
    const QC qc = make_qc(md.q);
    const int s1 = a.n_power - 8;
    const ulonglong2* __restrict__ tw = a.tw + ((u64) midx << a.n_power);
    const int row = t >> 4, i0 = t & 15;
    const u32 crow = tile * 16 + row;
    const ulonglong2* __restrict__ tb = a.twB + ((u64) midx * (15u << (a.n_power - 4))) + ((u64) crow * 15 * 16 + i0);
    const u64 n = (u64) 1 << a.n_power;
    const u64* __restrict__ pin = a.in + a.in_item_stride * item + ((u64) slot << a.n_power) + (u64) tile * 4096;
    const u64* __restrict__ pk = a.key + ((u64) midx << a.n_power) + (u64) tile * 4096 + row * 256 + i0;
    const u64 dig_off = (u64) a.rc << a.n_power;
    const u64 key_off1 = (u64) a.key_limbs << a.n_power, key_off2 = (u64) a.key_limbs << (a.n_power + 1);
    const bool lazy = row_stages_lazy(md, a.lazy_q_max) && md.q <= ~0ull / (u64) a.digits;
    ulonglong2* twa = reinterpret_cast<ulonglong2*>(twbuf);
    if (i0 < 15) {
        const int s = (i0 >= 7) ? 3 : (i0 >= 3) ? 2 : (i0 >= 1) ? 1 : 0;
        twa[i0 * 16 + row] = tw[((((u32) 1 << s1) + crow) << s) + (i0 - ((1 << s) - 1))];
    }
    wave_lds_fence();

    u64 h0[16], l0[16], h1[16], l1[16];
#pragma unroll
    for (int k = 0; k < 16; k++) h0[k] = l0[k] = h1[k] = l1[k] = 0;
    for (int i = ki.d0; i < ki.d1; i++) {
        u64 x[16];
        const u64* p = pin + dig_off * i;
        if (a.skip_identity && i == midx) {
            const u64* pi = a.ident + a.ident_item_stride * item + ((u64) i << a.n_power) + (u64) tile * 4096;
#pragma unroll
            for (int k = 0; k < 16; k++) x[k] = gld(&pi[row * 256 + i0 + 16 * k]);
        } else if (lazy) {
            ks_row_digit<true>(x, p, lds, twa, tb, qc, md, row, i0);
        } else {
            ks_row_digit<false>(x, p, lds, twa, tb, qc, md, row, i0);
        }
        const u64* k0 = pk + key_off2 * i;
        const u64* k1 = k0 + key_off1;
#pragma unroll
        for (int k = 0; k < 16; k++) {
            acc128(h0[k], l0[k], x[k], k0[16 * k]);
            acc128(h1[k], l1[k], x[k], k1[16 * k]);
        }
    }
    u64* po = (SPLIT ? const_cast<u64*>(pin) + dig_off * ki.d0 - (u64) tile * 4096
                     : a.out + a.out_item_stride * item + ((u64) slot << a.n_power)) +
              (u64) tile * 4096 + row * 256 + i0;
#pragma unroll
    for (int k = 0; k < 16; k++) {
        po[16 * k] = reduce128(h0[k], l0[k], md);
        po[dig_off + 16 * k] = reduce128(h1[k], l1[k], md);
    }
    (void) n;
}

template <bool SPLIT>
__global__ __launch_bounds__(NTT_THREADS, SPLIT ? 2 : 1) void ks_row_mac(KsMacArgs a)
{
    __shared__ __attribute__((aligned(16))) u64 lds[ROW_LDS_ELEMS];
    __shared__ ulonglong2 twa[15 * 16];
    const KsIdx ki = ks_index<SPLIT, SPLIT ? 0 : 1>(a);
    if (!ki.valid) return;
    const int midx = a.mod_order ? a.mod_order[ki.slot] : ki.slot;
    const Mod md = a.mods[midx];
    if (md.fp) return;
    ks_row_mac_int_body<SPLIT>(a, ki, md, midx, lds, twa);
}

template <bool SPLIT>
__device__ __forceinline__ void ks_row_mac_fp_body(const KsMacArgs& a, const KsIdx& ki, const Mod& md, int midx,
                                                   u64* lds, void* twbuf)
{
    const int t = threadIdx.x;
    const int item = ki.item, tile = ki.tile, slot = ki.slot;
    const FC fc = make_fc(md.q, FP_SITE(SPLIT ? FPS_KS_ROW_SPLIT : FPS_KS_ROW, a.n_power - 12));
    const int s1 = a.n_power - 8;
    const ulonglong2* __restrict__ tw = a.tw + ((u64) midx << a.n_power);
    const int row = t >> 4, i0 = t & 15;
    const u32 crow = tile * 16 + row;
    const double* __restrict__ tb8 = a.twB8 + ((u64) midx * (15u << (a.n_power - 4))) + ((u64) crow * 15 * 16 + i0);
    const u64* __restrict__ pin = a.in + a.in_item_stride * item + ((u64) slot << a.n_power) + (u64) tile * 4096;
    const u64* __restrict__ pk = a.key + ((u64) midx << a.n_power) + (u64) tile * 4096 + row * 256 + i0;
    const u64 dig_off = (u64) a.rc << a.n_power;
    const u64 key_off1 = (u64) a.key_limbs << a.n_power, key_off2 = (u64) a.key_limbs << (a.n_power + 1);

    double* twl = reinterpret_cast<double*>(twbuf);
#pragma unroll
    for (int k = 0; k < 15; k++) twl[k * 256 + t] = tb8[k * 16];
    if (i0 < 15) {
        const int s = (i0 >= 7) ? 3 : (i0 >= 3) ? 2 : (i0 >= 1) ? 1 : 0;
        const int b = i0 - ((1 << s) - 1);
        twl[15 * 256 + i0 * 16 + row] = as_f64(tw[((((u32) 1 << s1) + crow) << s) + b].x);
    }
    wave_lds_fence();

    double a0[16], a1[16];
#pragma unroll
    for (int k = 0; k < 16; k++) a0[k] = a1[k] = 0.0;
    int since = 0;
    for (int i = ki.d0; i < ki.d1; i++) {
        double x[16];
        const u64* p = pin + dig_off * i;
        const bool ident = a.skip_identity && i == midx;
        const u64* px = ident ? a.ident + a.ident_item_stride * item + ((u64) i << a.n_power) + (u64) tile * 4096 : p;
        u64 xr[16];
#pragma unroll
        for (int k = 0; k < 16; k++) {
            if constexpr (!SPLIT) xr[k] = __builtin_nontemporal_load(&px[row * 256 + i0 + 16 * k]);
            else xr[k] = px[row * 256 + i0 + 16 * k];
        }
        const u64* k0 = pk + key_off2 * i;
        const u64* k1 = k0 + key_off1;
        u64 kv0[16], kv1[16];
#pragma unroll
        for (int k = 0; k < 16; k++) {
            kv0[k] = k0[16 * k];
            kv1[k] = k1[16 * k];
        }
        if (ident) {
            FP_STAGE(fc, FP_STAGE_INPUT);
#pragma unroll
            for (int k = 0; k < 16; k++) x[k] = fp_reduce(fp_from_u64(xr[k]), fc);
        } else {
            if constexpr (SPLIT) {
#pragma unroll
                for (int k = 0; k < 16; k++) x[k] = as_f64(xr[k]);
#pragma unroll
                for (int s = 0; s < 4; s++) {
                    const int half = 8 >> s;
                    FP_STAGE(fc, s1 + s);
#pragma unroll
                    for (int b = 0; b < (1 << s); b++) {
                        const double w = twl[15 * 256 + ((1 << s) - 1 + b) * 16 + row];
                        const ulonglong2 wp = make_ulonglong2(as_bits(w), as_bits(w * fc.qi));
#pragma unroll
                        for (int j = 0; j < half; j++) fp_ct_bfly(x[b * 2 * half + j], x[b * 2 * half + j + half], wp, fc);
                    }
                }
                FP_STAGE(fc, s1 + 4);
#pragma unroll
                for (int k = 0; k < 16; k++) x[k] = fp_reduce(x[k], fc);
#pragma unroll
                for (int k = 0; k < 16; k++) lds[row_phys(row * 256 + i0 + 16 * k)] = as_bits(x[k]);
                wave_lds_fence();
#pragma unroll
                for (int k = 0; k < 8; k++) {
                    ulonglong2 v = *reinterpret_cast<const ulonglong2*>(&lds[row_phys(row * 256 + 16 * i0 + 2 * k)]);
                    x[2 * k] = as_f64(v.x);
                    x[2 * k + 1] = as_f64(v.y);
                }
#pragma unroll
                for (int s = 0; s < 4; s++) {
                    const int half = 8 >> s;
                    FP_STAGE(fc, s1 + 4 + s);
#pragma unroll
                    for (int b = 0; b < (1 << s); b++) {
                        const double wd = twl[((1 << s) - 1 + b) * 256 + t];
                        const ulonglong2 w = make_ulonglong2(as_bits(wd), as_bits(wd * fc.qi));
#pragma unroll
                        for (int j = 0; j < half; j++) fp_ct_bfly(x[b * 2 * half + j], x[b * 2 * half + j + half], w, fc);
                    }
                }
            } else {
                int row_o = row, t_o = t;
                asm volatile("" : "+v"(row_o), "+v"(t_o));
                const double* twa = twl + 15 * 256 + row_o;
                const double* twb = twl + t_o;
                double wn[8], wc[8];
                wc[0] = twa[0];
                wn[0] = twa[16];
                wn[1] = twa[32];
                __builtin_amdgcn_sched_barrier(0);
#pragma unroll
                for (int k = 0; k < 16; k++) x[k] = as_f64(xr[k]);
#pragma unroll
                for (int s = 0; s < 4; s++) {
                    const int half = 8 >> s;
                    FP_STAGE(fc, s1 + s);
                    if (s > 0) {
#pragma unroll
                        for (int b = 0; b < (1 << s); b++) wc[b] = wn[b];
                    }
                    if (s < 3) {
                        if (s > 0) {
#pragma unroll
                            for (int b = 0; b < (2 << s); b++) wn[b] = twa[((2 << s) - 1 + b) * 16];
                        }
                    } else {
                        wn[0] = twb[0];
                    }
                    __builtin_amdgcn_sched_barrier(0);
#pragma unroll
                    for (int b = 0; b < (1 << s); b++) {
                        const double w = wc[b];
                        const ulonglong2 wp = make_ulonglong2(as_bits(w), as_bits(w * fc.qi));
#pragma unroll
                        for (int j = 0; j < half; j++) fp_ct_bfly(x[b * 2 * half + j], x[b * 2 * half + j + half], wp, fc);
                    }
                }
                FP_STAGE(fc, s1 + 4);
#pragma unroll
                for (int k = 0; k < 16; k++) x[k] = fp_reduce(x[k], fc);
#pragma unroll
                for (int k = 0; k < 16; k++) lds[row_phys(row * 256 + i0 + 16 * k)] = as_bits(x[k]);
                wave_lds_fence();
#pragma unroll
                for (int k = 0; k < 8; k++) {
                    ulonglong2 v = *reinterpret_cast<const ulonglong2*>(&lds[row_phys(row * 256 + 16 * i0 + 2 * k)]);
                    x[2 * k] = as_f64(v.x);
                    x[2 * k + 1] = as_f64(v.y);
                }
#pragma unroll
                for (int s = 0; s < 4; s++) {
                    const int half = 8 >> s;
                    FP_STAGE(fc, s1 + 4 + s);
#pragma unroll
                    for (int b = 0; b < (1 << s); b++) wc[b] = wn[b];
                    if (s < 3) {
#pragma unroll
                        for (int b = 0; b < (2 << s); b++) wn[b] = twb[((2 << s) - 1 + b) * 256];
                    }
                    __builtin_amdgcn_sched_barrier(0);
#pragma unroll
                    for (int b = 0; b < (1 << s); b++) {
                        const double wd = wc[b];
                        const ulonglong2 w = make_ulonglong2(as_bits(wd), as_bits(wd * fc.qi));
#pragma unroll
                        for (int j = 0; j < half; j++) fp_ct_bfly(x[b * 2 * half + j], x[b * 2 * half + j + half], w, fc);
                    }
                }
            }
            wave_lds_fence();
#pragma unroll
            for (int k = 0; k < 8; k++)
                *reinterpret_cast<ulonglong2*>(&lds[row_phys(row * 256 + 16 * i0 + 2 * k)]) =
                    make_ulonglong2(as_bits(x[2 * k]), as_bits(x[2 * k + 1]));
            wave_lds_fence();
#pragma unroll
            for (int k = 0; k < 16; k++) x[k] = as_f64(lds[row_phys(row * 256 + i0 + 16 * k)]);
            wave_lds_fence();
        }
#pragma unroll
        for (int k = 0; k < 16; k++) {
            const double xi = x[k] * fc.qi;
            FP_STAGE(fc, FP_STAGE_PRODUCT);
            a0[k] += fp_mul(fp_from_u64(kv0[k]), x[k], xi, fc);
            a1[k] += fp_mul(fp_from_u64(kv1[k]), x[k], xi, fc);
            FP_STAGE(fc, FP_STAGE_SUMS + since);
            FP_AUDIT_VAL(fc, FPM_SUM, a0[k]);
            FP_AUDIT_VAL(fc, FPM_SUM, a1[k]);
        }
        if (++since == 3) {
            since = 0;
            FP_STAGE(fc, FP_STAGE_SUMS + 3);
#pragma unroll
            for (int k = 0; k < 16; k++) {
                a0[k] = fp_reduce(a0[k], fc);
                a1[k] = fp_reduce(a1[k], fc);
            }
        }
    }
    u64* po = (SPLIT ? const_cast<u64*>(pin) + dig_off * ki.d0 - (u64) tile * 4096
                     : a.out + a.out_item_stride * item + ((u64) slot << a.n_power)) +
              (u64) tile * 4096 + row * 256 + i0;
    FP_STAGE(fc, FP_STAGE_OUT);
#pragma unroll
    for (int k = 0; k < 16; k++) {
        if constexpr (!SPLIT) {
            __builtin_nontemporal_store(fp_to_u64(fp_canon(a0[k], fc)), &po[16 * k]);
            __builtin_nontemporal_store(fp_to_u64(fp_canon(a1[k], fc)), &po[dig_off + 16 * k]);
        } else {
            po[16 * k] = fp_to_u64(fp_canon(a0[k], fc));
            po[dig_off + 16 * k] = fp_to_u64(fp_canon(a1[k], fc));
        }
    }
}

template <bool SPLIT>
__global__ __launch_bounds__(NTT_THREADS) void ks_row_mac_fp(KsMacArgs a)
{
    __shared__ __attribute__((aligned(16))) u64 lds[ROW_LDS_ELEMS];
    __shared__ double twl[15 * 256 + 15 * 16];
    const KsIdx ki = ks_index<SPLIT, SPLIT ? 0 : 2>(a);
    if (!ki.valid) return;
    const int midx = a.mod_order ? a.mod_order[ki.slot] : ki.slot;
    const Mod md = a.mods[midx];
    if (!md.fp) return;
    ks_row_mac_fp_body<SPLIT>(a, ki, md, midx, lds, twl);
}

__global__ __launch_bounds__(NTT_THREADS, 2) void ks_row_mac_split(KsMacArgs a)
{
    __shared__ __attribute__((aligned(16))) u64 lds[ROW_LDS_ELEMS];
    __shared__ double twl[15 * 256 + 15 * 16];
    const KsIdx ki = ks_index<true>(a);
    if (!ki.valid) return;
    const int midx = a.mod_order ? a.mod_order[ki.slot] : ki.slot;
    const Mod md = a.mods[midx];
    if (md.fp) ks_row_mac_fp_body<true>(a, ki, md, midx, lds, twl);
    else ks_row_mac_int_body<true>(a, ki, md, midx, lds, twl);
}

hipError_t ks_row_mac_launch(const KsMacArgs& a, int items, hipStream_t st)
{
    if (a.digits > 64 || items <= 0) return hipErrorInvalidValue;
    if (a.splits > 1 && a.digits < 2 * a.splits) return hipErrorInvalidValue;
    KsMacArgs k = a;
    k.items = items;
    if (k.int_slot_count < 0 || k.int_slot_count > 8) k.int_slot_count = 0;
    const unsigned tiles = (1u << a.n_power) / 4096, units = (unsigned) items * (a.splits > 1 ? (unsigned) a.splits : 1u);
    auto grid_of = [&](int kind) { return dim3(8u * ((ks_slots(k, kind) * tiles * units + 7u) / 8u)); };
    if (a.splits > 1) {
        hipLaunchKernelGGL(ks_row_mac_split, grid_of(0), dim3(NTT_THREADS), 0, st, k);
    } else {
        if (!a.no_fp && ks_slots(k, 2) > 0)
            hipLaunchKernelGGL(ks_row_mac_fp<false>, grid_of(2), dim3(NTT_THREADS), 0, st, k);
        if (!a.no_int && ks_slots(k, 1) > 0)
            hipLaunchKernelGGL(ks_row_mac<false>, grid_of(1), dim3(NTT_THREADS), 0, st, k);
    }
    return hipGetLastError();
}

__device__ __forceinline__ void fp_gs_bfly(double& x, double& y, ulonglong2 w, const FC& c)
{
    const double s = x + y, d = x - y;
    x = s;
    y = fp_mul(d, as_f64(w.x), as_f64(w.y), c);
    FP_AUDIT_VAL(c, FPM_SUM, s);
}

struct ArInt {
    typedef u64 T;
    QC qc;
    __device__ __forceinline__ explicit ArInt(const Mod& md) : qc(make_qc(md.q)) {}
    __device__ __forceinline__ T from_canon(u64 v) const { return v; }
    __device__ __forceinline__ T from_bits(u64 v) const { return v; }
    __device__ __forceinline__ u64 to_bits(T v) const { return v; }
    template <int LOGR>
    __device__ __forceinline__ void radix(T (&x)[1 << LOGR], const ulonglong2* __restrict__ tw, u32 root0) const
    {
        gs_radix<LOGR>(x, tw, root0, qc);
    }
    __device__ __forceinline__ void radix16_tb(T (&x)[16], const ulonglong2* __restrict__ tb) const { gs_radix16_tb(x, tb, qc); }
    template <int LOGR>
    __device__ __forceinline__ void radix_last(T (&x)[1 << LOGR], const ulonglong2* __restrict__ tw, ulonglong2 ninv,
                                               ulonglong2 w1ninv, u64 (&out)[1 << LOGR]) const
    {
        gs_radix_last<LOGR>(x, tw, 1u, ninv, w1ninv, qc);
#pragma unroll
        for (int k = 0; k < (1 << LOGR); k++) out[k] = x[k];
    }
};

struct ArFp {
    typedef double T;
    FC fc;
    int s1;
    __device__ __forceinline__ explicit ArFp(const Mod& md, int n_power) : fc(make_fc(md.q, FP_SITE(FPS_INV, n_power - 12))), s1(n_power - 8) {}
    __device__ __forceinline__ T from_canon(u64 v) const { return fp_from_u64(v); }
    __device__ __forceinline__ T from_bits(u64 v) const { return as_f64(v); }
    __device__ __forceinline__ u64 to_bits(T v) const { return as_bits(v); }
    template <int N>
    __device__ __forceinline__ void reduce_all(T (&x)[N]) const
    {
#pragma unroll
        for (int k = 0; k < N; k++) x[k] = fp_reduce(x[k], fc);
    }
    template <int LOGR>
    __device__ __forceinline__ void radix(T (&x)[1 << LOGR], const ulonglong2* __restrict__ tw, u32 root0) const
    {
        int done = 0;
#pragma unroll
        for (int s = LOGR - 1; s >= 0; s--) {
            const int half = (1 << LOGR) >> (s + 1);
            FP_STAGE(fc, 31 - __builtin_clz(root0) + s);
#pragma unroll
            for (int b = 0; b < (1 << s); b++) {
                const ulonglong2 w = tw[(root0 << s) + b];
#pragma unroll
                for (int j = 0; j < half; j++) fp_gs_bfly(x[b * 2 * half + j], x[b * 2 * half + j + half], w, fc);
            }
            if ((++done & 1) == 0 || s == 0) reduce_all(x);
        }
    }
    __device__ __forceinline__ void radix16_tb(T (&x)[16], const ulonglong2* __restrict__ tb) const
    {
#pragma unroll
        for (int s = 3; s >= 0; s--) {
            const int half = 8 >> s;
            FP_STAGE(fc, s1 + 4 + s);
#pragma unroll
            for (int b = 0; b < (1 << s); b++) {
                const ulonglong2 w = tb[((1 << s) - 1 + b) * 16];
#pragma unroll
                for (int j = 0; j < half; j++) fp_gs_bfly(x[b * 2 * half + j], x[b * 2 * half + j + half], w, fc);
            }
            if (s == 2 || s == 0) reduce_all(x);
        }
    }
    template <int LOGR>
    __device__ __forceinline__ void radix_last(T (&x)[1 << LOGR], const ulonglong2* __restrict__ tw, ulonglong2 ninv,
                                               ulonglong2 w1ninv, u64 (&out)[1 << LOGR]) const
    {
        int done = 0;
#pragma unroll
        for (int s = LOGR - 1; s >= 1; s--) {
            const int half = (1 << LOGR) >> (s + 1);
            FP_STAGE(fc, s);
#pragma unroll
            for (int b = 0; b < (1 << s); b++) {
                const ulonglong2 w = tw[(1u << s) + b];
#pragma unroll
                for (int j = 0; j < half; j++) fp_gs_bfly(x[b * 2 * half + j], x[b * 2 * half + j + half], w, fc);
            }
            if ((++done & 1) == 0) reduce_all(x);
        }
        constexpr int half = (1 << LOGR) >> 1;
        FP_STAGE(fc, 0);
#pragma unroll
        for (int j = 0; j < half; j++) {
            const double sum = x[j] + x[j + half], d = x[j] - x[j + half];
            out[j] = fp_to_u64(fp_canon(fp_mul(sum, as_f64(ninv.x), as_f64(ninv.y), fc), fc));
            out[j + half] = fp_to_u64(fp_canon(fp_mul(d, as_f64(w1ninv.x), as_f64(w1ninv.y), fc), fc));
        }
    }
};

template <typename AR, bool TO_LDS, bool TENSOR = false>
__device__ __forceinline__ void inv_row_part(const AR& ar, const NttArgs& a, int mod, int tt, u32 crow0,
                                             const u64* __restrict__ src, u64* __restrict__ dst, u64* lds,
                                             int tensor_part = 0)
{
    typedef typename AR::T T;
    const int s1 = a.n_power - 8;
    const ulonglong2* __restrict__ tw = a.itw + ((u64) mod << a.n_power);
    const int row = tt >> 4, i0 = tt & 15;
    const u32 crow = crow0 + row;
    if (TENSOR) {
        const Mod md = a.mods[mod];
        const u64 part_off = (u64) a.tensor_limbs << a.n_power;
        const u64* __restrict__ a0 = src, * __restrict__ a1 = src + part_off, * __restrict__ b0 = src + 2 * part_off,
                 * __restrict__ b1 = src + 3 * part_off;
#pragma unroll
        for (int k0 = 0; k0 < 16; k0 += 4) {
            u64 r[4];
            if (tensor_part == 1) {
                u64 va0[4], va1[4], vb0[4], vb1[4];
#pragma unroll
                for (int k = 0; k < 4; k++) {
                    const int e = row * 256 + i0 + 16 * (k0 + k);
                    va0[k] = a0[e]; va1[k] = a1[e]; vb0[k] = b0[e]; vb1[k] = b1[e];
                }
#pragma unroll
                for (int k = 0; k < 4; k++) {
                    u64 h1, l1, h2, l2;
                    mul64wide(va0[k], vb1[k], h1, l1);
                    mul64wide(va1[k], vb0[k], h2, l2);
                    const u64 lo = l1 + l2;
                    r[k] = reduce128(h1 + h2 + (lo < l1), lo, md);
                }
            } else {
                const u64* __restrict__ pa = tensor_part == 0 ? a0 : a1;
                const u64* __restrict__ pb = tensor_part == 0 ? b0 : b1;
                u64 va[4], vb[4];
#pragma unroll
                for (int k = 0; k < 4; k++) {
                    const int e = row * 256 + i0 + 16 * (k0 + k);
                    va[k] = pa[e]; vb[k] = pb[e];
                }
#pragma unroll
                for (int k = 0; k < 4; k++) r[k] = mul_barrett(va[k], vb[k], md);
            }
#pragma unroll
            for (int k = 0; k < 4; k++) lds[row_phys(row * 256 + i0 + 16 * (k0 + k))] = r[k];
        }
    } else {
#pragma unroll
        for (int k = 0; k < 16; k++) lds[row_phys(row * 256 + i0 + 16 * k)] = gld(&src[row * 256 + i0 + 16 * k]);
    }
    wave_lds_fence();
    T x[16];
#pragma unroll
    for (int k = 0; k < 8; k++) {
        ulonglong2 v = *reinterpret_cast<const ulonglong2*>(&lds[row_phys(row * 256 + 16 * i0 + 2 * k)]);
        x[2 * k] = ar.from_canon(v.x);
        x[2 * k + 1] = ar.from_canon(v.y);
    }
    ar.radix16_tb(x, a.itwB + ((u64) mod * (15u << (a.n_power - 4))) + ((u64) crow * 15 * 16 + i0));
    wave_lds_fence();
#pragma unroll
    for (int k = 0; k < 8; k++)
        *reinterpret_cast<ulonglong2*>(&lds[row_phys(row * 256 + 16 * i0 + 2 * k)]) =
            make_ulonglong2(ar.to_bits(x[2 * k]), ar.to_bits(x[2 * k + 1]));
    wave_lds_fence();
#pragma unroll
    for (int k = 0; k < 16; k++) x[k] = ar.from_bits(lds[row_phys(row * 256 + i0 + 16 * k)]);
    ar.template radix<4>(x, tw, (1u << s1) + crow);
    if constexpr (TO_LDS) {
#pragma unroll
        for (int k = 0; k < 16; k++) lds[row_phys(row * 256 + i0 + 16 * k)] = ar.to_bits(x[k]);
    } else {
#pragma unroll
        for (int k = 0; k < 16; k++) gst(&dst[row * 256 + i0 + 16 * k], ar.to_bits(x[k]));
    }
}

struct InvEpi {
    const u64* last;
    const u64* ct;
    u64* out;
    Mod md;
    u64 half, qP, hm, inv;
    int galois, n_power;
    bool pre;
};
__device__ __forceinline__ bool inv_epi_setup(const NttArgs& a, const PolySel& ps, InvEpi& e, bool& skip)
{
    skip = false;
    if (!a.iepi.on) return false;
    const NttInvEpilogue& ep = a.iepi;
    const int pc = ep.p_count ? ep.p_count : 1;
    const int part = udiv16(ps.j, ep.mg_slots), limb = ps.j - part * (ep.limbs + pc);
    if (limb >= ep.limbs) { skip = true; return true; }
    const u64 item_in = a.out_item_stride * ps.item;
    const u64 off = (u64) (part * ep.limbs + limb) << a.n_power;
    e.pre = ep.u != nullptr;
    e.last = e.pre ? ep.u + ep.u_item_stride * ps.item + off
                   : a.out + item_in + ((u64) (part * (ep.limbs + 1) + ep.limbs) << a.n_power);
    e.ct = (ep.ct && part < ep.add_parts) ? ep.ct + ep.ct_item_stride * ps.item + off : nullptr;
    e.out = ep.out + ep.out_item_stride * ps.item + off;
    e.md = a.mods[ps.mod];
    e.half = ep.half;
    e.qP = a.mods[ep.p_mod].q;
    e.hm = e.pre ? 0 : ep.half_mod[limb];
    e.inv = ep.inv[limb];
    e.galois = ep.galois_elt;
    e.n_power = a.n_power;
    return true;
}
template <int CNT, bool EPI, typename POS>
__device__ __forceinline__ void inv_store(const InvEpi& epr, u64* __restrict__ p, u32 e0, POS pos, const u64 (&o)[CNT])
{
    if constexpr (!EPI) {
#pragma unroll
        for (int k = 0; k < CNT; k++) gst(&p[pos(k)], o[k]);
        return;
    }
    const InvEpi* ep = &epr;
    u64 lv[CNT], cv[CNT], r[CNT];
#pragma unroll
    for (int k = 0; k < CNT; k++) lv[k] = ep->last[e0 + pos(k)];
    if (ep->ct) {
#pragma unroll
        for (int k = 0; k < CNT; k++) cv[k] = ep->ct[e0 + pos(k)];
    }
    if (!ep->pre) {
#pragma unroll
        for (int k = 0; k < CNT; k++) {
            u64 l = add_mod(lv[k], ep->half, ep->qP);
            l = reduce64(l, ep->md);
            lv[k] = sub_mod(l, ep->hm, ep->md.q);
        }
    }
#pragma unroll
    for (int k = 0; k < CNT; k++) r[k] = mul_barrett(sub_mod(o[k], lv[k], ep->md.q), ep->inv, ep->md);
    if (ep->ct) {
#pragma unroll
        for (int k = 0; k < CNT; k++) r[k] = add_mod(cv[k], r[k], ep->md.q);
    }
    if (ep->galois) {
#pragma unroll
        for (int k = 0; k < CNT; k++) {
            const u32 raw = (e0 + (u32) pos(k)) * (u32) ep->galois;
            ep->out[raw & ((1u << ep->n_power) - 1u)] = ((raw >> ep->n_power) & 1u) ? ep->md.q - r[k] : r[k];
        }
    } else {
#pragma unroll
        for (int k = 0; k < CNT; k++) ep->out[e0 + pos(k)] = r[k];
    }
}

template <int S1, typename AR, bool FROM_LDS, bool KEEP = false, bool EPI = false>
__device__ __forceinline__ void inv_col_part(const AR& ar, const NttArgs& a, int mod, int tt, int g, u64* __restrict__ p,
                                             u64* buf, u64 (&keep)[16], const InvEpi& ep = InvEpi(), u32 e0 = 0)
{
    typedef typename AR::T T;
    constexpr int R = 1 << S1;
    constexpr int CT = 4096 / R;
    constexpr int NSA = S1 - 4;
    constexpr int RA = 1 << NSA;
    constexpr int G = 16 / RA;
    const ulonglong2* __restrict__ tw = a.itw + ((u64) mod << a.n_power);
    const ulonglong2 ninv = a.ninv[mod], w1ninv = a.w1ninv[mod];
    const int col = tt % CT, r1 = tt / CT;
    auto pos = [&](int row, int c) -> int {
        if constexpr (FROM_LDS) return single_pos<S1>(row, g * CT + c);
        else return col_phys(row * CT + c);
    };
    T x[16];
#pragma unroll
    for (int k = 0; k < 16; k++)
        x[k] = ar.from_bits(FROM_LDS ? buf[pos(16 * r1 + k, col)] : gld(&p[(u64) (16 * r1 + k) * 256 + col]));
    if constexpr (NSA > 0) {
        ar.template radix<4>(x, tw, (u32) (RA + r1));
#pragma unroll
        for (int k = 0; k < 16; k++) buf[pos(16 * r1 + k, col)] = ar.to_bits(x[k]);
        __syncthreads();
#pragma unroll
        for (int gi = 0; gi < G; gi++) {
            const int L = tt + NTT_THREADS * gi;
            const int c = L % CT, rb = L / CT;
            T y[RA];
            u64 o[RA];
#pragma unroll
            for (int k = 0; k < RA; k++) y[k] = ar.from_bits(buf[pos(rb + 16 * k, c)]);
            ar.template radix_last<NSA>(y, tw, ninv, w1ninv, o);
            if constexpr (RA == 16) {
                u64 oa[8], ob[8];
#pragma unroll
                for (int k = 0; k < 8; k++) { oa[k] = o[k]; ob[k] = o[8 + k]; }
                inv_store<8, EPI>(ep, p, e0, [&](int k) { return (u32) ((rb + 16 * k) * 256 + c); }, oa);
                inv_store<8, EPI>(ep, p, e0, [&](int k) { return (u32) ((rb + 16 * (8 + k)) * 256 + c); }, ob);
            } else {
                inv_store<RA, EPI>(ep, p, e0, [&](int k) { return (u32) ((rb + 16 * k) * 256 + c); }, o);
            }
            if constexpr (KEEP) {
#pragma unroll
                for (int k = 0; k < RA; k++) keep[gi * RA + k] = o[k];
            }
        }
    } else {
        u64 o[16];
        ar.template radix_last<4>(x, tw, ninv, w1ninv, o);
        {
            u64 oa[8], ob[8];
#pragma unroll
            for (int k = 0; k < 8; k++) { oa[k] = o[k]; ob[k] = o[8 + k]; }
            inv_store<8, EPI>(ep, p, e0, [&](int k) { return (u32) (k * 256 + col); }, oa);
            inv_store<8, EPI>(ep, p, e0, [&](int k) { return (u32) ((8 + k) * 256 + col); }, ob);
        }
        if constexpr (KEEP) {
#pragma unroll
            for (int k = 0; k < 16; k++) keep[k] = o[k];
        }
    }
}

__global__ __launch_bounds__(NTT_THREADS) void ntt_inv_row(NttArgs a)
{
    __shared__ __attribute__((aligned(16))) u64 lds[ROW_LDS_ELEMS];
    const PolySel ps = select_poly(a, blockIdx.y);
    if (a.iepi.on && ps.j - udiv16(ps.j, a.iepi.mg_slots) * (a.iepi.limbs + (a.iepi.p_count ? a.iepi.p_count : 1)) >= a.iepi.limbs)
        return;
    const Mod md = a.mods[ps.mod];
    const u64* __restrict__ src = a.in + ps.in_off + (u64) blockIdx.x * 4096;
    u64* __restrict__ dst = a.out + ps.out_off + (u64) blockIdx.x * 4096;
    if (md.fp) inv_row_part<ArFp, false>(ArFp(md, a.n_power), a, ps.mod, threadIdx.x, blockIdx.x * 16, src, dst, lds);
    else inv_row_part<ArInt, false>(ArInt(md), a, ps.mod, threadIdx.x, blockIdx.x * 16, src, dst, lds);
}

__device__ __forceinline__ const u64* tensor_src(const NttArgs& a, const PolySel& ps, int& part)
{
    part = udiv16(ps.j, a.mg_tensor_limbs);
    const int limb = ps.j - part * a.tensor_limbs;
    return a.tensor_in + (u64) ps.item * a.tensor_item_stride + ((u64) limb << a.n_power);
}
__global__ __launch_bounds__(NTT_THREADS) void ntt_inv_row_tensor(NttArgs a)
{
    __shared__ __attribute__((aligned(16))) u64 lds[ROW_LDS_ELEMS];
    const PolySel ps = select_poly(a, blockIdx.y);
    const Mod md = a.mods[ps.mod];
    int part;
    const u64* __restrict__ src = tensor_src(a, ps, part) + (u64) blockIdx.x * 4096;
    u64* __restrict__ dst = a.out + ps.out_off + (u64) blockIdx.x * 4096;
    if (md.fp) inv_row_part<ArFp, false, true>(ArFp(md, a.n_power), a, ps.mod, threadIdx.x, blockIdx.x * 16, src, dst, lds, part);
    else inv_row_part<ArInt, false, true>(ArInt(md), a, ps.mod, threadIdx.x, blockIdx.x * 16, src, dst, lds, part);
}

template <int S1, bool EPI = false>
__global__ __launch_bounds__(NTT_THREADS) void ntt_inv_col(NttArgs a)
{
    constexpr int CT = 4096 >> S1;
    __shared__ u64 lds[(S1 > 4) ? COL_LDS_ELEMS : 1];
    const PolySel ps = select_poly(a, blockIdx.y);
    const Mod md = a.mods[ps.mod];
    if (a.only_int && md.fp) return;
    u64* __restrict__ p = a.out + ps.out_off + blockIdx.x * CT;
    u64 unused[16];
    if constexpr (EPI) {
        InvEpi epi;
        bool skip;
        inv_epi_setup(a, ps, epi, skip);
        if (skip) return;
        if (md.fp) inv_col_part<S1, ArFp, false, false, true>(ArFp(md, a.n_power), a, ps.mod, threadIdx.x, 0, p, lds, unused, epi, blockIdx.x * CT);
        else inv_col_part<S1, ArInt, false, false, true>(ArInt(md), a, ps.mod, threadIdx.x, 0, p, lds, unused, epi, blockIdx.x * CT);
    } else {
        if (md.fp) inv_col_part<S1, ArFp, false>(ArFp(md, a.n_power), a, ps.mod, threadIdx.x, 0, p, lds, unused);
        else inv_col_part<S1, ArInt, false>(ArInt(md), a, ps.mod, threadIdx.x, 0, p, lds, unused);
    }
}

template <int S1, bool EPI, bool TENSOR, typename AR>
__device__ __forceinline__ void inv_single_body(const AR& ar, const NttArgs& a, const PolySel& ps, u64* limb)
{
    constexpr int CT = 4096 >> S1;
    const int t = threadIdx.x, g = t >> 8, tt = t & 255;
    InvEpi epi;
    if constexpr (EPI) {
        bool skip;
        inv_epi_setup(a, ps, epi, skip);
        if (skip) return;
    }
    if constexpr (TENSOR) {
        int part;
        const u64* src = tensor_src(a, ps, part) + (u64) g * 4096;
        inv_row_part<AR, true, true>(ar, a, ps.mod, tt, g * 16, src, nullptr, limb + g * 4096, part);
    } else {
        inv_row_part<AR, true>(ar, a, ps.mod, tt, g * 16, a.in + ps.in_off + (u64) g * 4096, nullptr, limb + g * 4096);
    }
    __syncthreads();
    u64 unused[16];
    if constexpr (EPI) inv_col_part<S1, AR, true, false, true>(ar, a, ps.mod, tt, g, a.out + ps.out_off + g * CT, limb, unused, epi, g * CT);
    else inv_col_part<S1, AR, true>(ar, a, ps.mod, tt, g, a.out + ps.out_off + g * CT, limb, unused);
}

template <int S1, bool EPI = false, bool TENSOR = false>
__global__ __launch_bounds__(16 << S1, 4) void ntt_inv_single(NttArgs a)
{
    extern __shared__ __attribute__((aligned(16))) u64 limb[];
    const PolySel ps = select_poly(a, blockIdx.x);
    const Mod md = a.mods[ps.mod];
    if (md.fp) inv_single_body<S1, EPI, TENSOR>(ArFp(md, a.n_power), a, ps, limb);
    else inv_single_body<S1, EPI, TENSOR>(ArInt(md), a, ps, limb);
}

template <int S1>
__global__ __launch_bounds__(NTT_THREADS) void ntt_fwd_col_multi(NttArgs a)
{
    constexpr int R = 1 << S1;
    constexpr int CT = 4096 / R;
    constexpr int NSA = S1 - 4;
    constexpr int RA = 1 << NSA;
    constexpr int G = 16 / RA;
    __shared__ u64 lds[(S1 > 4) ? COL_LDS_ELEMS : 1];
    __shared__ ulonglong2 twl[(S1 > 4) ? 512 : 1];
    const int t = threadIdx.x;
    const int rc = a.decomp_mods;
    const int digits = udiv16(a.polys_per_item, a.mg_decomp_mods);
    const int item = udiv16(blockIdx.y, a.mg_per_item), digit = blockIdx.y - item * digits;
    const u64 in_slot = (u64) digit * (a.decomp_in_mul ? a.decomp_in_mul : 1) + a.decomp_in_add;
    const u64* __restrict__ src = a.in + (u64) item * a.in_item_stride + (in_slot << a.n_power) + blockIdx.x * CT;
    u64 sreg[16];
    const int smod = a.half_on ? a.half_src_mod : digit;
    if (a.src_inv && a.mods[smod].fp) {
        const Mod im = a.mods[smod];
        inv_col_part<S1, ArFp, false, true>(ArFp(im, a.n_power), a, smod, t, 0, const_cast<u64*>(src), lds, sreg);
        __syncthreads();
    } else if constexpr (NSA > 0) {
#pragma unroll
        for (int g = 0; g < G; g++) {
            const int L = t + NTT_THREADS * g;
            const int c = L % CT, rb = L / CT;
#pragma unroll
            for (int k = 0; k < RA; k++) sreg[g * RA + k] = src[(u64) (rb + 16 * k) * 256 + c];
        }
    } else {
#pragma unroll
        for (int k = 0; k < 16; k++) sreg[k] = src[(u64) k * 256 + (t % CT)];
    }
    const Mod smd = a.mods[a.half_on ? a.half_src_mod : digit];
    if (a.half_on) {
#pragma unroll
        for (int k = 0; k < 16; k++) sreg[k] = add_mod(sreg[k], a.half, smd.q);
    }
    const bool wide = smd.bit > 52;
    if (!wide) {
#pragma unroll
        for (int k = 0; k < 16; k++) sreg[k] = as_bits(fp_from_u64(sreg[k]));
    }
    int done = 0;
    for (int k = 0; k < rc; k++) {
        PolySel ps;
        ps.mod = a.mod_offset + (a.mod_order ? ld_const_i32(a.mod_order + k) : k);
        ps.digit = digit;
        ps.item = item;
        ps.j = digit * rc + k;
        ps.in_off = 0;
        ps.out_off = (u64) item * a.out_item_stride + ((u64) ps.j << a.n_power);
        if (a.skip_identity && ps.mod == digit) continue;
        const Mod md = ld_const_mod(a.mods + ps.mod);
        if (!md.fp) continue;
        ulonglong2* tl = twl + ((S1 > 4) ? 256 * (done & 1) : 0);
        done++;
        if (wide) fwd_col_body_fp<S1, true, true, true>(a, ps, md, lds, tl, sreg);
        else fwd_col_body_fp<S1, true, false, true>(a, ps, md, lds, tl, sreg);
    }
}

template <int S1>
static bool use_col_multi(const NttArgs& a, int batch)
{
    constexpr int CT = 4096 >> S1;
    if (!a.decomp_mods || a.col_multi == 0 || batch % a.decomp_mods) return false;
    if (a.copy_src) return false;
    if (a.col_multi == 1) return true;
    return (long) (256 / CT) * (batch / a.decomp_mods) >= 2048;
}

template <int S1>
static void launch_col_multi(const NttArgs& a, int batch, hipStream_t st)
{
    constexpr int CT = 4096 >> S1;
    if (a.plan_has_fp)
        hipLaunchKernelGGL((ntt_fwd_col_multi<S1>), dim3(256 / CT, batch / a.decomp_mods), dim3(NTT_THREADS), 0, st, a);
    if ((a.plan_has_int || !a.plan_has_fp) && !(a.plan_has_fp && a.int_slot_count < 0)) {
        NttArgs c = a;
        c.group_span = 0;
        c.mg_group_span = 0;
        c.only_int = a.plan_has_fp;
        int polys = batch;
        if (c.only_int && a.int_slot_count > 0) polys = batch / a.decomp_mods * a.int_slot_count;
        else c.int_slot_count = 0;
        hipLaunchKernelGGL((ntt_fwd_col<S1, true>), dim3(256 / CT, polys), dim3(NTT_THREADS), 0, st, c);
    }
}

static bool use_single_pass(const NttArgs& a, int batch)
{
    if (a.single_pass == 1) return true;
    if (a.single_pass == 0) return false;
    const int s1 = a.n_power - 8;
    if (s1 <= 4) return true;
    if (s1 == 5) return batch >= 64;
    if (batch < 48) return false;
    const long rounds = ((long) batch + 255) / 256;
    return (long) batch * 4 >= rounds * 256 * 3;
}

template <int S1>
static void launch_fwd_col_only(const NttArgs& a, int batch, hipStream_t st)
{
    constexpr int CT = 4096 >> S1;
    if (use_col_multi<S1>(a, batch)) launch_col_multi<S1>(a, batch, st);
    else if (a.decomp_mods)
        hipLaunchKernelGGL((ntt_fwd_col<S1, true>), dim3(256 / CT, batch), dim3(NTT_THREADS), 0, st, a);
    else
        hipLaunchKernelGGL((ntt_fwd_col<S1, false>), dim3(256 / CT, batch), dim3(NTT_THREADS), 0, st, a);
}

template <int S1>
static void launch_fwd(const NttArgs& a, int batch, hipStream_t st)
{
    constexpr int CT = 4096 >> S1;
    if constexpr (S1 <= 6) {
        if (!a.decomp_mods && use_single_pass(a, batch)) {
            static const hipError_t attr = hipFuncSetAttribute((const void*) ntt_fwd_single<S1>,
                                                               hipFuncAttributeMaxDynamicSharedMemorySize, 8 << (S1 + 8));
            (void) attr;
            hipLaunchKernelGGL((ntt_fwd_single<S1>), dim3(batch), dim3(16 << S1), (size_t) 8 << (S1 + 8), st, a);
            return;
        }
        if (a.decomp_mods && a.single_decomp_ok && !a.copy_src && !a.src_inv && !use_col_multi<S1>(a, batch) &&
            use_single_pass(a, batch)) {
            static const hipError_t attr_d = hipFuncSetAttribute((const void*) ntt_fwd_single<S1, true>,
                                                                 hipFuncAttributeMaxDynamicSharedMemorySize, 8 << (S1 + 8));
            (void) attr_d;
            NttArgs c = a;
            c.group_span = 0;
            c.mg_group_span = 0;
            hipLaunchKernelGGL((ntt_fwd_single<S1, true>), dim3(batch), dim3(16 << S1), (size_t) 8 << (S1 + 8), st, c);
            return;
        }
    }
    if (use_col_multi<S1>(a, batch)) {
        launch_col_multi<S1>(a, batch, st);
    } else if (a.decomp_mods) {
        NttArgs c = a;
        c.group_span = 0;
        c.mg_group_span = 0;
        hipLaunchKernelGGL((ntt_fwd_col<S1, true>), dim3(256 / CT, batch), dim3(NTT_THREADS), 0, st, c);
    } else
        hipLaunchKernelGGL((ntt_fwd_col<S1, false>), dim3(256 / CT, batch), dim3(NTT_THREADS), 0, st, a);
    NttArgs b = a;
    b.in = a.out;
    b.in_item_stride = a.out_item_stride;
    hipLaunchKernelGGL(ntt_fwd_row, dim3((1u << a.n_power) / 4096, batch), dim3(NTT_THREADS), 0, st, b);
}

template <int S1>
static void launch_inv(const NttArgs& a, int batch, hipStream_t st)
{
    constexpr int CT = 4096 >> S1;
    if constexpr (S1 <= 6) {
        if (use_single_pass(a, batch) && !a.poly_order) {
            static const hipError_t attr = hipFuncSetAttribute((const void*) ntt_inv_single<S1, false>,
                                                               hipFuncAttributeMaxDynamicSharedMemorySize, 8 << (S1 + 8));
            static const hipError_t attr_e = hipFuncSetAttribute((const void*) ntt_inv_single<S1, true>,
                                                                 hipFuncAttributeMaxDynamicSharedMemorySize, 8 << (S1 + 8));
            static const hipError_t attr_t = hipFuncSetAttribute((const void*) ntt_inv_single<S1, false, true>,
                                                                 hipFuncAttributeMaxDynamicSharedMemorySize, 8 << (S1 + 8));
            (void) attr;
            (void) attr_e;
            (void) attr_t;
            if (a.tensor_in)
                hipLaunchKernelGGL((ntt_inv_single<S1, false, true>), dim3(batch), dim3(16 << S1), (size_t) 8 << (S1 + 8), st, a);
            else if (a.iepi.on)
                hipLaunchKernelGGL((ntt_inv_single<S1, true>), dim3(batch), dim3(16 << S1), (size_t) 8 << (S1 + 8), st, a);
            else
                hipLaunchKernelGGL((ntt_inv_single<S1, false>), dim3(batch), dim3(16 << S1), (size_t) 8 << (S1 + 8), st, a);
            return;
        }
    }
    if (a.tensor_in) hipLaunchKernelGGL(ntt_inv_row_tensor, dim3((1u << a.n_power) / 4096, batch), dim3(NTT_THREADS), 0, st, a);
    else hipLaunchKernelGGL(ntt_inv_row, dim3((1u << a.n_power) / 4096, batch), dim3(NTT_THREADS), 0, st, a);
    NttArgs b = a;
    b.in = a.out;
    b.in_item_stride = a.out_item_stride;
    if (a.iepi.on) hipLaunchKernelGGL((ntt_inv_col<S1, true>), dim3(256 / CT, batch), dim3(NTT_THREADS), 0, st, b);
    else hipLaunchKernelGGL((ntt_inv_col<S1, false>), dim3(256 / CT, batch), dim3(NTT_THREADS), 0, st, b);
}

static unsigned magic16(int d) { return d <= 1 ? 0u : (unsigned) ((0x100000000ull + (unsigned) d - 1) / (unsigned) d); }
static void fill_magics(NttArgs& g)
{
    g.mg_group_span = magic16(g.group_span);
    g.mg_mod_count = magic16(g.mod_count);
    g.mg_per_item = magic16(g.mod_count ? g.polys_per_item / g.mod_count : 0);
    g.mg_polys_per_item = magic16(g.polys_per_item);
    g.mg_decomp_mods = magic16(g.decomp_mods);
    g.epi.mg_limbs = magic16(g.epi.limbs);
    g.iepi.mg_slots = magic16(g.iepi.limbs + (g.iepi.p_count ? g.iepi.p_count : 1));
    g.mg_tensor_limbs = magic16(g.tensor_limbs);
}

bool ntt_decomp_uses_multi(const NttArgs& a, int batch)
{
    if (!a.plan_has_fp) return false;
    switch (a.n_power - 8) {
        case 4: return use_col_multi<4>(a, batch);
        case 5: return use_col_multi<5>(a, batch);
        case 6: return use_col_multi<6>(a, batch);
        case 7: return use_col_multi<7>(a, batch);
        case 8: return use_col_multi<8>(a, batch);
    }
    return false;
}

hipError_t ntt_launch_inv_rows(const NttArgs& a, int batch, hipStream_t st)
{
    if (batch <= 0) return hipSuccess;
    if (a.n_power < 12 || a.n_power > 16 || batch > 65535) return hipErrorInvalidValue;
    NttArgs g = a;
    g.group_span = 0;
    if (!a.poly_order && a.mod_count > 1 && batch % a.mod_count == 0 &&
        (!a.polys_per_item || a.polys_per_item % a.mod_count == 0))
        g.group_span = batch / a.mod_count;
    fill_magics(g);
    hipLaunchKernelGGL(ntt_inv_row, dim3((1u << a.n_power) / 4096, batch), dim3(NTT_THREADS), 0, st, g);
    if (a.plan_has_int) {
        NttArgs b = g;
        b.in = g.out;
        b.in_item_stride = g.out_item_stride;
        b.only_int = 1;
        switch (a.n_power - 8) {
#define CASE(S) case S: hipLaunchKernelGGL((ntt_inv_col<S, false>), dim3(256 / (4096 >> S), batch), dim3(NTT_THREADS), 0, st, b); break;
            CASE(4) CASE(5) CASE(6) CASE(7) CASE(8)
#undef CASE
        }
    }
    return hipGetLastError();
}

hipError_t ntt_launch_fwd_col(const NttArgs& a, int batch, hipStream_t st)
{
    if (batch <= 0) return hipSuccess;
    if (a.n_power < 12 || a.n_power > 16 || batch > 65535 || a.poly_order) return hipErrorInvalidValue;
    if (a.src_inv && !ntt_decomp_uses_multi(a, batch)) return hipErrorInvalidValue;
    NttArgs g = a;
    g.group_span = 0;
    if (!a.decomp_mods && a.mod_count > 1 && batch % a.mod_count == 0 &&
        (!a.polys_per_item || a.polys_per_item % a.mod_count == 0))
        g.group_span = batch / a.mod_count;
    fill_magics(g);
    switch (a.n_power - 8) {
        case 4: launch_fwd_col_only<4>(g, batch, st); break;
        case 5: launch_fwd_col_only<5>(g, batch, st); break;
        case 6: launch_fwd_col_only<6>(g, batch, st); break;
        case 7: launch_fwd_col_only<7>(g, batch, st); break;
        case 8: launch_fwd_col_only<8>(g, batch, st); break;
    }
    return hipGetLastError();
}

hipError_t ntt_launch(const NttArgs& a, int batch, bool inverse, hipStream_t st)
{
    if (batch <= 0) return hipSuccess;
    if (a.n_power < 12 || a.n_power > 16) return hipErrorInvalidValue;
    if (a.decomp_mods && (inverse || a.poly_order || !a.polys_per_item)) return hipErrorInvalidValue;
    if (a.src_inv && (!a.decomp_mods || batch > 65535 || !ntt_decomp_uses_multi(a, batch))) return hipErrorInvalidValue;
    if (a.copy_src && (!a.decomp_mods || inverse)) return hipErrorInvalidValue;
    if (a.tensor_in && (!inverse || a.poly_order || a.iepi.on || a.polys_per_item != 3 * a.tensor_limbs || batch % a.polys_per_item))
        return hipErrorInvalidValue;
    if (a.iepi.on && (!inverse || a.poly_order || batch % a.polys_per_item ||
                      a.polys_per_item != 2 * (a.iepi.limbs + (a.iepi.p_count ? a.iepi.p_count : 1)) ||
                      ((a.iepi.p_count > 1) != (a.iepi.u != nullptr))))
        return hipErrorInvalidValue;
    if (batch > 65535) {
        const int unit = a.polys_per_item ? a.polys_per_item : a.mod_count;
        if ((!a.polys_per_item && a.poly_order) || (batch % unit) || unit > 65535) return hipErrorInvalidValue;
        int done = 0;
        while (done < batch) {
            int chunk = batch - done;
            int maxc = (65535 / unit) * unit;
            if (chunk > maxc) chunk = maxc;
            NttArgs c = a;
            if (a.polys_per_item) {
                const u64 items_done = (u64) (done / unit);
                c.in = a.in + items_done * a.in_item_stride;
                c.out = a.out + items_done * a.out_item_stride;
                if (a.epi.on) {
                    c.epi.ks = a.epi.ks + items_done * a.epi.ks_item_stride;
                    if (a.epi.ct) c.epi.ct = a.epi.ct + items_done * a.epi.ct_item_stride;
                    c.epi.out = a.epi.out + items_done * a.epi.out_item_stride;
                }
                if (a.iepi.on) {
                    if (a.iepi.ct) c.iepi.ct = a.iepi.ct + items_done * a.iepi.ct_item_stride;
                    c.iepi.out = a.iepi.out + items_done * a.iepi.out_item_stride;
                    if (a.iepi.u) c.iepi.u = a.iepi.u + items_done * a.iepi.u_item_stride;
                }
                if (a.copy_src) {
                    c.copy_src = a.copy_src + items_done * a.copy_src_item_stride;
                    c.copy_dst = a.copy_dst + items_done * a.copy_dst_item_stride;
                }
                if (a.tensor_in) c.tensor_in = a.tensor_in + items_done * a.tensor_item_stride;
            } else {
                c.in = a.in + ((u64) done << a.n_power);
                c.out = a.out + ((u64) done << a.n_power);
            }
            hipError_t e = ntt_launch(c, chunk, inverse, st);
            if (e != hipSuccess) return e;
            done += chunk;
        }
        return hipSuccess;
    }
    NttArgs g = a;
    g.group_span = 0;
    if (!a.poly_order && a.mod_count > 1 && batch % a.mod_count == 0 &&
        (!a.polys_per_item || a.polys_per_item % a.mod_count == 0))
        g.group_span = batch / a.mod_count;
    fill_magics(g);
    switch (a.n_power - 8) {
#define CASE(S)                                   \
    case S:                                       \
        if (inverse) launch_inv<S>(g, batch, st); \
        else launch_fwd<S>(g, batch, st);         \
        break;
        CASE(4) CASE(5) CASE(6) CASE(7) CASE(8)
#undef CASE
    }
    return hipGetLastError();
}

}
```

heongpu_amd/csrc/ntt.hpp:

```cpp
#pragma once
#include "modarith.cuh"

namespace hegpu {

struct NttEpilogue {
    const u64* ks;
    u64 ks_item_stride;
    int ks_part_limbs;
    const u64* ct;
    u64 ct_item_stride;
    int ct_parts;
    unsigned galois_inv;
    u64* out;
    u64 out_item_stride;
    const u64* inv;
    int limbs;
    int on;
    unsigned mg_limbs;
};

struct NttInvEpilogue {
    int on;
    int limbs;
    int add_parts;
    int p_mod;
    int galois_elt;
    unsigned mg_slots;
    u64 half;
    const u64* half_mod;
    const u64* inv;
    const u64* ct;
    u64 ct_item_stride;
    u64* out;
    u64 out_item_stride;
    int p_count;
    const u64* u;
    u64 u_item_stride;
};

struct NttArgs {
    const u64* in;
    u64* out;
    const Mod* mods;
    const ulonglong2* tw;
    const ulonglong2* itw;
    const ulonglong2* twB;
    const ulonglong2* itwB;
    const double* twB8;
    const ulonglong2* ninv;
    const ulonglong2* w1ninv;
    const int* mod_order;
    const int* poly_order;
    int n_power;
    int mod_count;
    int mod_offset;
    int polys_per_item;
    u64 in_item_stride;
    u64 out_item_stride;
    int decomp_mods;
    int skip_identity;
    int group_span;
    unsigned mg_group_span, mg_per_item, mg_polys_per_item, mg_mod_count, mg_decomp_mods;
    NttEpilogue epi;
    NttInvEpilogue iepi;
    int decomp_in_mul, decomp_in_add;
    int half_on, half_src_mod;
    u64 half;
    const u64* half_mod;
    int col_multi;
    int single_pass;
    int plan_has_fp, plan_has_int;
    u64 lazy_q_max;
    int only_int;
    int single_decomp_ok;
    int int_slot_count;
    int int_slots[8];
    int src_inv;
    const u64* copy_src;
    u64* copy_dst;
    u64 copy_src_item_stride, copy_dst_item_stride;
    int copy_part_limbs;
    const u64* tensor_in;
    u64 tensor_item_stride;
    int tensor_limbs;
    unsigned mg_tensor_limbs;
};

hipError_t ntt_launch(const NttArgs& a, int batch, bool inverse, hipStream_t st);
bool ntt_decomp_uses_multi(const NttArgs& a, int batch);
hipError_t ntt_launch_inv_rows(const NttArgs& a, int batch, hipStream_t st);
hipError_t ntt_launch_fwd_col(const NttArgs& a, int batch, hipStream_t st);

struct KsMacArgs {
    const u64* in;
    u64 in_item_stride;
    const u64* key;
    u64* out;
    u64 out_item_stride;
    const Mod* mods;
    const ulonglong2* tw;
    const ulonglong2* twB;
    const double* twB8;
    const int* mod_order;
    int n_power, digits, rc, key_limbs;
    u64 lazy_q_max;
    int skip_identity;
    const u64* ident;
    u64 ident_item_stride;
    int items;
    int splits;
    int no_fp, no_int;
    int int_slot_count;
    int int_slots[8];
};
hipError_t ks_row_mac_launch(const KsMacArgs& a, int items, hipStream_t st);

}
```

heongpu_amd/csrc/ops.cpp:

```cpp
#include "ops.hpp"
#include <vector>
#include <utility>

namespace hegpu {

#define TRY(x)                           \
    do {                                 \
        hipError_t e__ = (x);            \
        if (e__ != hipSuccess) return e__; \
    } while (0)

static u64 inv_mod_2n(u64 g, u64 two_n)
{
    u64 x = g;
    for (int i = 0; i < 6; i++) x *= 2 - g * x;
    return x & (two_n - 1);
}

static long fused_row_mac_need(const Context& c)
{
    size_t fp = 0;
    for (unsigned char f : c.plan_qp.fp) fp += f ? 1 : 0;
    return (2 * fp > c.plan_qp.fp.size()) ? 768 : 400;
}
static int fused_digit_splits(const Context& c, int rc, int digits, int batch)
{
    if (c.digit_split == 0) return 0;
    if (c.digit_split > 0) return digits >= 2 * c.digit_split ? c.digit_split : 0;
    if (c.fused_row_mac >= 0 || c.n_power < 16 || digits < 8) return 0;
    const long wgs = (long) batch * rc * (long) (c.n >> 12), need = fused_row_mac_need(c);
    return (need == 768 && wgs < 2 * need && 4 * wgs >= need) ? 4 : 0;
}
static bool use_fused_row_mac(const Context& c, int rc, int batch)
{
    if (c.fused_row_mac >= 0) return c.fused_row_mac != 0;
    return (long) batch * rc * (long) (c.n >> 12) >= fused_row_mac_need(c);
}

static void fill_int_slots(const Context& c, NttArgs& a, const u64* order)
{
    int cnt = 0;
    for (int k = 0; k < a.decomp_mods; k++) {
        const int m = a.mod_offset + (order ? (int) order[k] : k);
        if (m < 0 || m >= (int) c.plan_qp.fp.size()) { a.int_slot_count = 0; return; }
        if (c.plan_qp.fp[m]) continue;
        if (cnt == 8) { a.int_slot_count = 0; return; }
        a.int_slots[cnt++] = k;
    }
    a.int_slot_count = cnt ? cnt : -1;
}

static hipError_t keyswitch_ntt_mac(const Context& c, NttArgs a, const u64* key, u64* acc, u64 acc_stride,
                                    int digits, int rc, int split, int level, const u64* ident, u64 ident_stride,
                                    int batch, hipStream_t st, int which = 3)
{
    const int ppi = digits * rc;
    const int skip_identity = ident ? 1 : 0;
    a.skip_identity = skip_identity;
    const int splits = fused_digit_splits(c, rc, digits, batch);
    if (!splits && !use_fused_row_mac(c, rc, batch)) {
        if (ident && c.fused_row_mac == 0)
            TRY(rns_copy_diag(ident, ident_stride, a.out, a.out_item_stride, c.n_power, digits, rc, batch, st));
        else a.skip_identity = 0;
        TRY(ntt_launch(a, ppi * batch, false, st));
        return rns_keyswitch_mac(a.out, a.out_item_stride, key, acc, acc_stride, c.plan_qp.mods, c.n_power, digits, rc,
                                 c.Qp_size, split, level, batch, st);
    }
    const int chunk = 65535 / ppi;
    if (chunk < 1) return hipErrorInvalidValue;
    for (int b0 = 0; b0 < batch; b0 += chunk) {
        const int nb = (batch - b0 < chunk) ? batch - b0 : chunk;
        NttArgs ca = a;
        ca.in = a.in + (u64) b0 * a.in_item_stride;
        ca.out = a.out + (u64) b0 * a.out_item_stride;
        if (which & 1) TRY(ntt_launch_fwd_col(ca, ppi * nb, st));
        if (!(which & 2)) continue;
        KsMacArgs k{};
        k.in = ca.out; k.in_item_stride = a.out_item_stride; k.key = key;
        k.out = acc + (u64) b0 * acc_stride; k.out_item_stride = acc_stride;
        k.mods = c.plan_qp.mods; k.tw = c.plan_qp.tw; k.twB = c.plan_qp.twB; k.twB8 = c.plan_qp.twB8; k.mod_order = a.mod_order;
        k.lazy_q_max = a.lazy_q_max; k.n_power = c.n_power; k.digits = digits; k.rc = rc; k.key_limbs = c.Qp_size; k.skip_identity = skip_identity;
        k.ident = ident ? ident + (u64) b0 * ident_stride : nullptr; k.ident_item_stride = ident_stride;
        k.splits = splits;
        k.no_fp = !a.plan_has_fp;
        k.no_int = !a.plan_has_int || a.int_slot_count < 0;
        k.int_slot_count = a.int_slot_count > 0 ? a.int_slot_count : 0;
        for (int q = 0; q < 8; q++) k.int_slots[q] = a.int_slots[q];
        TRY(ks_row_mac_launch(k, nb, st));
        if (splits > 1)
            TRY(rns_sum_partials(ca.out, a.out_item_stride, k.out, acc_stride, c.plan_qp.mods, a.mod_order, c.n_power,
                                 digits, rc, splits, nb, st));
    }
    return hipSuccess;
}

size_t ops_workspace_elems(const Context& c, int op, int depth, int batch)
{
    const u64 n = c.n;
    const int Q = c.Q_size, Qp = c.Qp_size;
    const int l = Q - depth, rc = Qp - depth;
    const int L = Q + c.bsk_size;
    u64 per = 0;
    switch (op) {
        case OP_CKKS_RELIN: per = ((u64) l * rc + 2 * rc) * n; break;
        case OP_CKKS_RESCALE: per = ((u64) 2 * (l - 1) + 2 * l) * n; break;
        case OP_CKKS_GALOIS: per = ((u64) 2 * l + (u64) l * rc + 2 * rc) * n; break;
        case OP_CKKS_ROTATE_HOISTED: per = ((u64) 2 * l + (u64) l * rc + 4 * 2 * rc) * n; break;
        case OP_BFV_MULTIPLY: per = (u64) 7 * L * n; break;
        case OP_BFV_RELIN: per = ((u64) Q * Qp + 2 * Qp) * n; break;
        case OP_BFV_GALOIS: per = ((u64) Q * Qp + 2 * Qp) * n; break;
        case OP_KEYGEN_SECRET: per = n; break;
        case OP_KEYGEN_PUBLIC: per = (u64) 2 * Qp * n; break;
        case OP_KEYGEN_SWITCH: per = (u64) 2 * Q * Qp * n; break;
        case OP_CKKS_ENCRYPT:
        case OP_BFV_ENCRYPT: per = (u64) 5 * Qp * n; break;
        case OP_BFV_DECRYPT: per = (u64) Q * n; break;
        case OP_BFV_DECODE: per = n; break;
        case OP_BFV_MULTIPLY_PLAIN: per = (u64) Q * n; break;
        case OP_CKKS_ENCODE: per = n; break;
        case OP_CKKS_DECODE: per = (u64) (l + 1) * n; break;
        default: return 0;
    }
    return per * (u64) batch;
}

hipError_t op_ckks_multiply(const Context& c, const u64* ct1, u64 s1, const u64* ct2, u64 s2, u64* out, u64 so,
                            int depth, int batch, hipStream_t st)
{
    if (batch <= 0) return hipSuccess;
    return rns_cross_multiplication(ct1, s1, ct2, s2, out, so, c.plan_qp.mods, c.n_power, c.Q_size - depth, batch,
                                    st);
}

static hipError_t ckks_keyswitch_core(const Context& c, const u64* src, u64 src_stride, const u64* add, u64 add_stride,
                                      int add_parts, u64* outp, u64 out_stride, const u64* key, int depth, int batch,
                                      u64* temp1, u64* temp2, u64 per, hipStream_t st, unsigned phases,
                                      int galois_elt = 0)
{
    const int np = c.n_power;
    const int Q = c.Q_size, Qp = c.Qp_size;
    const int l = Q - depth, rc = Qp - depth;
    const Mod* mods = c.plan_qp.mods;

    NttArgs a = c.ntt_args(0);
    a.in = src; a.out = temp2; a.mod_count = l; a.polys_per_item = l;
    a.in_item_stride = src_stride; a.out_item_stride = per;
    NttArgs dgt = c.ntt_args(0);
    dgt.in = temp2; dgt.out = temp1; dgt.mod_count = rc; dgt.polys_per_item = l * rc; dgt.decomp_mods = rc;
    dgt.in_item_stride = per; dgt.out_item_stride = per;
    dgt.mod_order = c.d32("new_prime_locations") + triangle_offset(Qp, depth);
    fill_int_slots(c, dgt, c.h64("new_prime_locations").data() + triangle_offset(Qp, depth));
    const bool fuse_inv = use_fused_row_mac(c, rc, batch) && c.fuse_inverse && (long) l * rc * batch <= 65535 &&
                          ntt_decomp_uses_multi(dgt, l * rc * batch);
    if (phases & RELIN_PHASE_INTT_C2) {
        if (fuse_inv) TRY(ntt_launch_inv_rows(a, l * batch, st));
        else TRY(ntt_launch(a, l * batch, true, st));
    }
    dgt.src_inv = fuse_inv ? 1 : 0;
    dgt.single_decomp_ok = 1;
    a = dgt;
    const int which = ((phases & RELIN_PHASE_COLUMN) ? 1 : 0) | ((phases & RELIN_PHASE_ROW_MAC) ? 2 : 0);
    if (which) TRY(keyswitch_ntt_mac(c, a, key, temp2, per, l, rc, l, depth, src, src_stride, batch, st, which));
    a = c.ntt_args(0);
    a.in = temp2; a.out = temp2; a.mod_count = 1; a.mod_offset = Q; a.polys_per_item = 2;
    a.in_item_stride = a.out_item_stride = per;
    a.poly_order = c.d32("new_input_locations") + 2 * depth;
    NttArgs md = c.ntt_args(0);
    md.in = temp2; md.out = temp1; md.mod_count = l; md.polys_per_item = 2 * l;
    md.in_item_stride = md.out_item_stride = per;
    md.decomp_mods = l; md.decomp_in_mul = l + 1; md.decomp_in_add = l;
    md.half_on = 1; md.half_src_mod = Q;
    fill_int_slots(c, md, nullptr);
    const bool fuse_inv_p = c.fused_moddown && c.fuse_inverse && (long) 2 * l * batch <= 65535 &&
                            ntt_decomp_uses_multi(md, 2 * l * batch);
    if (phases & RELIN_PHASE_INTT_P) {
        if (fuse_inv_p) TRY(ntt_launch_inv_rows(a, 2 * batch, st));
        else TRY(ntt_launch(a, 2 * batch, true, st));
    }
    if (!(phases & RELIN_PHASE_MODDOWN)) return hipSuccess;
    if (!c.fused_moddown)
        TRY(rns_moddown_stage_one(temp2, per, temp1, per, mods, c.d64("half"), c.d64("half_mod"), np, Q, l, batch,
                                  st));
    a = c.ntt_args(0);
    a.in = temp1; a.out = temp1; a.mod_count = l; a.polys_per_item = 2 * l;
    a.in_item_stride = a.out_item_stride = per;
    if (c.fused_moddown) {
        a.in = temp2; a.decomp_mods = l; a.decomp_in_mul = l + 1; a.decomp_in_add = l;
        a.half_on = 1; a.half_src_mod = Q; a.half = c.h64("half")[0]; a.half_mod = c.d64("half_mod");
        a.epi.on = 1;
        a.epi.ks = temp2; a.epi.ks_item_stride = per; a.epi.ks_part_limbs = l + 1;
        a.epi.ct = add; a.epi.ct_item_stride = add_stride; a.epi.ct_parts = add_parts;
        a.epi.out = outp; a.epi.out_item_stride = out_stride;
        a.epi.inv = c.d64("last_q_modinv");
        a.epi.limbs = l;
        a.epi.galois_inv = galois_elt ? (unsigned) inv_mod_2n((u64) galois_elt, 2 * c.n) : 0u;
        a.src_inv = fuse_inv_p ? 1 : 0;
        a.single_decomp_ok = 1;
        fill_int_slots(c, a, nullptr);
        return ntt_launch(a, 2 * l * batch, false, st);
    }
    if (add_parts != 2 || galois_elt) return hipErrorInvalidValue;
    TRY(ntt_launch(a, 2 * l * batch, false, st));
    return rns_moddown_stage_two(temp1, per, temp2, per, l + 1, add, add_stride, outp, out_stride, mods,
                                 c.d64("last_q_modinv"), np, l, 1, batch, st);
}

static hipError_t dtoq(const Context& c, int lvl, const u64* in, u64 in_stride, u64* out, u64 out_stride, int l,
                       int level, int batch, hipStream_t st)
{
    const Context::M2Level& L = c.m2_levels[lvl];
    return rns_base_conversion_DtoQtilde(in, in_stride, out, out_stride, c.plan_qp.mods,
                                         c.d64("m2_matrix_mg") + L.off_matrix, c.d64("m2_Mi_inv") + L.off_mi,
                                         c.d64("m2_negprod_mg") + L.off_prod, c.d32("m2_I_j") + L.off_digits,
                                         c.d32("m2_I_location") + L.off_digits, c.n_power, L.d, L.rc, l, level,
                                         c.m2_width, batch, st);
}

static hipError_t ckks_moddown_multi(const Context& c, u64* acc, u64* scratch, u64 per, const u64* ct, u64 cs,
                                     int add_parts, u64* out, u64 so, int depth, int galois_elt, int batch,
                                     hipStream_t st)
{
    const u64 n = c.n;
    const int Q = c.Q_size, Qp = c.Qp_size, P = c.P_size;
    const int l = Q - depth, rc = Qp - depth;
    for (int part = 0; part < 2; part++) {
        NttArgs a = c.ntt_args(0);
        a.in = a.out = acc + (u64) (part * rc + l) * n;
        a.mod_count = P; a.mod_offset = Q; a.polys_per_item = P;
        a.in_item_stride = a.out_item_stride = per;
        TRY(ntt_launch(a, P * batch, true, st));
    }
    TRY(rns_moddown_multi_stage_one(acc, per, scratch, per, c.plan_qp.mods, c.d64("half"), c.d64("half_mod"),
                                    c.d64("last_q_modinv"), c.d64("m2_md_G"), c.d64("m2_md_C"), c.n_power, rc, l, Qp, Q,
                                    P, batch, st));
    NttArgs a = c.ntt_args(0);
    a.in = a.out = scratch; a.mod_count = l; a.polys_per_item = 2 * l;
    a.in_item_stride = a.out_item_stride = per;
    a.epi.on = 1;
    a.epi.ks = acc; a.epi.ks_item_stride = per; a.epi.ks_part_limbs = rc;
    a.epi.ct = ct; a.epi.ct_item_stride = cs; a.epi.ct_parts = add_parts;
    a.epi.out = out; a.epi.out_item_stride = so;
    a.epi.inv = c.d64("m2_md_W0");
    a.epi.limbs = l;
    a.epi.galois_inv = galois_elt ? (unsigned) inv_mod_2n((u64) galois_elt, 2 * c.n) : 0u;
    return ntt_launch(a, 2 * l * batch, false, st);
}

static hipError_t ckks_rotate_tail(const Context& c, u64* acc, const u64* coef, u64 per, u64* out, u64 so, int galois_elt,
                                   int depth, int batch, hipStream_t st)
{
    const int Q = c.Q_size, Qp = c.Qp_size;
    const int l = Q - depth, rc = Qp - depth;
    NttArgs a = c.ntt_args(0);
    a.in = acc; a.out = acc; a.mod_count = rc; a.polys_per_item = 2 * rc;
    a.mod_order = c.d32("new_prime_locations") + triangle_offset(Qp, depth);
    a.in_item_stride = a.out_item_stride = per;
    TRY(ntt_launch(a, 2 * rc * batch, true, st));
    TRY(rns_moddown_permute(acc, per, coef, per, out, so, c.plan_qp.mods, c.d64("half"), c.d64("half_mod"),
                            c.d64("last_q_modinv"), galois_elt, c.n_power, rc, l, Qp, Q, c.P_size, batch, st));
    a = c.ntt_args(0);
    a.in = out; a.out = out; a.mod_count = l; a.polys_per_item = 2 * l;
    a.in_item_stride = a.out_item_stride = so;
    return ntt_launch(a, 2 * l * batch, false, st);
}

static hipError_t ckks_keyswitch_II(const Context& c, const u64* ct, u64 cs, int add_parts, u64* out, u64 so,
                                    const u64* key, int galois_elt, int depth, int batch, u64* ws, hipStream_t st)
{
    const int np = c.n_power;
    const u64 n = c.n;
    const int Q = c.Q_size, Qp = c.Qp_size;
    const int l = Q - depth, rc = Qp - depth;
    const int d = c.m2_levels[depth].d;
    const bool relin = add_parts == 2;
    const bool ntt_domain = c.fused_moddown && (relin || c.ntt_galois);
    const u64 copy = relin ? 0 : (u64) 2 * l * n;
    const u64 per = copy + ((u64) l * rc + 2 * rc) * n;
    u64* coef = relin ? out : ws;
    const u64 coef_stride = relin ? so : per;
    u64* digits = ws + copy;
    u64* acc = digits + (u64) l * rc * n;
    const int first = (relin || ntt_domain) ? add_parts : 0;
    NttArgs a = c.ntt_args(0);
    a.in = ct + (u64) first * l * n; a.out = coef + (u64) first * l * n; a.mod_count = l;
    a.polys_per_item = (add_parts + 1 - first) * l;
    a.in_item_stride = cs; a.out_item_stride = coef_stride;
    TRY(ntt_launch(a, a.polys_per_item * batch, true, st));
    TRY(dtoq(c, depth, coef + (u64) add_parts * l * n, coef_stride, digits, per, l, depth, batch, st));
    a = c.ntt_args(0);
    a.in = digits; a.out = digits; a.mod_count = rc; a.polys_per_item = d * rc;
    a.mod_order = c.d32("new_prime_locations") + triangle_offset(Qp, depth);
    a.in_item_stride = a.out_item_stride = per;
    TRY(keyswitch_ntt_mac(c, a, key, acc, per, d, rc, l, depth, nullptr, 0, batch, st));
    if (ntt_domain)
        return ckks_moddown_multi(c, acc, ws, per, ct, cs, relin ? 0 : add_parts, out, so, depth, galois_elt, batch, st);
    if (!relin) return ckks_rotate_tail(c, acc, ws, per, out, so, galois_elt, depth, batch, st);
    a.in = acc; a.out = acc; a.polys_per_item = 2 * rc;
    TRY(ntt_launch(a, 2 * rc * batch, true, st));
    TRY(rns_moddown_extended(acc, per, nullptr, 0, ws, per, c.plan_qp.mods, c.d64("half"), c.d64("half_mod"),
                             c.d64("last_q_modinv"), np, rc, l, Qp, Q, c.P_size, 0, batch, st));
    a = c.ntt_args(0);
    a.in = ws; a.out = ws; a.mod_count = l; a.polys_per_item = 2 * l;
    a.in_item_stride = a.out_item_stride = per;
    TRY(ntt_launch(a, 2 * l * batch, false, st));
    return rns_addition_strided(ws, per, ct, cs, out, so, c.plan_qp.mods, np, l, 2, batch, st);
}

hipError_t op_ckks_relinearize(const Context& c, u64* ct, u64 cs, const u64* key, int depth, int batch, u64* ws,
                               hipStream_t st, unsigned phases)
{
    if (batch <= 0) return hipSuccess;
    if (c.P_size > 1) return ckks_keyswitch_II(c, ct, cs, 2, ct, cs, key, 0, depth, batch, ws, st);
    const u64 n = c.n;
    const int l = c.Q_size - depth, rc = c.Qp_size - depth;
    const u64 per = ((u64) l * rc + 2 * rc) * n;
    u64* temp1 = ws;
    u64* temp2 = ws + (u64) l * rc * n;
    return ckks_keyswitch_core(c, ct + ((u64) l << (c.n_power + 1)), cs, ct, cs, 2, ct, cs, key, depth, batch, temp1,
                               temp2, per, st, phases);
}

hipError_t op_ckks_rescale(const Context& c, u64* ct, u64 cs, int depth, int batch, u64* ws, hipStream_t st)
{
    if (batch <= 0) return hipSuccess;
    const int np = c.n_power;
    const u64 n = c.n;
    const int Q = c.Q_size, P = c.P_size;
    const int l = Q - depth;
    const int location = triangle_offset(Q - 1, depth);
    const u64 per = ((u64) 2 * (l - 1) + 2 * l) * n;
    u64* temp1 = ws;
    u64* temp2 = ws + (u64) 2 * (l - 1) * n;
    const Mod* mods = c.plan_qp.mods;

    NttArgs a = c.ntt_args(0);
    a.in = ct; a.out = ct; a.mod_count = 1; a.mod_offset = l - 1; a.polys_per_item = 2;
    a.in_item_stride = a.out_item_stride = cs;
    a.poly_order = c.d32("new_input_locations") + (depth + P) * 2;
    TRY(ntt_launch(a, 2 * batch, true, st));
    if (c.fused_moddown) {
        a = c.ntt_args(0);
        a.in = ct; a.out = temp1; a.mod_count = l - 1; a.polys_per_item = 2 * (l - 1);
        a.in_item_stride = cs; a.out_item_stride = per;
        a.decomp_mods = l - 1; a.decomp_in_mul = l; a.decomp_in_add = l - 1;
        a.half_on = 1; a.half_src_mod = l - 1; a.half = c.h64("rescaled_half")[depth];
        a.half_mod = c.d64("rescaled_half_mod") + location;
        if (c.copy_along && !ntt_decomp_uses_multi(a, 2 * (l - 1) * batch)) {
            a.copy_src = ct; a.copy_src_item_stride = cs;
            a.copy_dst = temp2; a.copy_dst_item_stride = per;
            a.copy_part_limbs = l;
        } else {
            TRY(rns_copy_limbs(ct, (u64) l * n, cs, temp2, (u64) l * n, per, np, l - 1, 2, batch, st));
        }
        a.epi.on = 1;
        a.epi.ks = temp2; a.epi.ks_item_stride = per; a.epi.ks_part_limbs = l;
        a.epi.ct = nullptr; a.epi.ct_item_stride = 0;
        a.epi.out = ct; a.epi.out_item_stride = cs;
        a.epi.inv = c.d64("rescaled_last_q_modinv") + location;
        a.epi.limbs = l - 1;
        return ntt_launch(a, 2 * (l - 1) * batch, false, st);
    }
    TRY(rns_moddown_stage_one(ct, cs, temp1, per, mods, c.d64("rescaled_half") + depth,
                              c.d64("rescaled_half_mod") + location, np, l - 1, l - 1, batch, st));
    a = c.ntt_args(0);
    a.in = temp1; a.out = temp1; a.mod_count = l - 1; a.polys_per_item = 2 * (l - 1);
    a.in_item_stride = a.out_item_stride = per;
    TRY(ntt_launch(a, 2 * (l - 1) * batch, false, st));
    TRY(rns_copy_limbs(ct, (u64) l * n, cs, temp2, (u64) l * n, per, np, l - 1, 2, batch, st));
    return rns_moddown_stage_two(temp1, per, temp2, per, l, nullptr, 0, ct, cs, mods,
                                 c.d64("rescaled_last_q_modinv") + location, np, l - 1, 0, batch, st);
}

hipError_t op_ckks_apply_galois(const Context& c, const u64* ct, u64 cs, u64* out, u64 so, const u64* key,
                                int galois_elt, int depth, int batch, u64* ws, hipStream_t st)
{
    if (batch <= 0) return hipSuccess;
    if (c.P_size > 1) return ckks_keyswitch_II(c, ct, cs, 1, out, so, key, galois_elt, depth, batch, ws, st);
    const int np = c.n_power;
    const u64 n = c.n;
    const int Q = c.Q_size, Qp = c.Qp_size;
    const int l = Q - depth, rc = Qp - depth;
    const u64 per = ((u64) 2 * l + (u64) l * rc + 2 * rc) * n;
    u64* temp0 = ws;
    u64* temp2 = temp0 + (u64) 2 * l * n;
    u64* temp3 = temp2 + (u64) l * rc * n;

    if (c.fused_moddown && c.ntt_galois) {
        if (c.galois_scatter)
            return ckks_keyswitch_core(c, ct + (u64) l * n, cs, ct, cs, 1, out, so, key, depth, batch, temp2, temp3, per, st,
                                       RELIN_PHASE_ALL, galois_elt);
        TRY(ckks_keyswitch_core(c, ct + (u64) l * n, cs, ct, cs, 1, temp0, per, key, depth, batch, temp2, temp3, per, st,
                                RELIN_PHASE_ALL));
        return rns_permute_ntt(temp0, per, out, so, galois_elt, np, 2 * l, batch, st);
    }
    NttArgs a = c.ntt_args(0);
    a.in = ct; a.out = temp0; a.mod_count = l; a.polys_per_item = 2 * l;
    a.in_item_stride = cs; a.out_item_stride = per;
    TRY(ntt_launch(a, 2 * l * batch, true, st));
    a = c.ntt_args(0);
    a.in = temp0 + (u64) l * n; a.out = temp2; a.mod_count = rc; a.polys_per_item = l * rc; a.decomp_mods = rc;
    a.in_item_stride = a.out_item_stride = per;
    a.mod_order = c.d32("new_prime_locations") + triangle_offset(Qp, depth);
    TRY(keyswitch_ntt_mac(c, a, key, temp3, per, l, rc, l, depth, ct + (u64) l * n, cs, batch, st));
    return ckks_rotate_tail(c, temp3, temp0, per, out, so, galois_elt, depth, batch, st);
}

hipError_t op_bfv_multiply(const Context& c, const u64* ct1, u64 s1, const u64* ct2, u64 s2, u64* out, u64 so,
                           int batch, u64* ws, hipStream_t st)
{
    if (batch <= 0) return hipSuccess;
    const int np = c.n_power;
    const u64 n = c.n;
    const int L = c.Q_size + c.bsk_size;
    const u64 per = (u64) 7 * L * n;
    u64* temp1 = ws;
    u64* temp2 = ws + (u64) 4 * L * n;
    TRY(rns_fast_convertion(ct1, s1, ct2, s2, temp1, per, c.behz, np, batch, st));
    NttArgs a = c.ntt_args(1);
    a.in = temp1; a.out = temp1; a.mod_count = L; a.polys_per_item = 4 * L;
    a.in_item_stride = a.out_item_stride = per;
    TRY(ntt_launch(a, 4 * L * batch, false, st));
    a.in = temp2; a.out = temp2; a.polys_per_item = 3 * L;
    if (c.fused_tensor) {
        a.tensor_in = temp1; a.tensor_item_stride = per; a.tensor_limbs = L;
    } else {
        TRY(rns_cross_multiplication(temp1, per, temp1 + (u64) 2 * L * n, per, temp2, per, c.plan_merge.mods, np, L,
                                     batch, st));
    }
    TRY(ntt_launch(a, 3 * L * batch, true, st));
    return rns_fast_floor(temp2, per, out, so, c.behz, np, batch, st);
}

static hipError_t bfv_intt_moddown(const Context& c, u64* acc, u64 per, const u64* ct, u64 cs, int add_parts, u64* out,
                                   u64 so, int galois_elt, int batch, hipStream_t st)
{
    const u64 n = c.n;
    const int Q = c.Q_size, Qp = c.Qp_size;
    for (int part = 0; part < 2; part++) {
        NttArgs a = c.ntt_args(0);
        a.in = a.out = acc + (u64) (part * Qp + Q) * n;
        a.mod_count = 1; a.mod_offset = Q; a.polys_per_item = 1;
        a.in_item_stride = a.out_item_stride = per;
        TRY(ntt_launch(a, batch, true, st));
    }
    NttArgs a = c.ntt_args(0);
    a.in = a.out = acc; a.mod_count = Qp; a.polys_per_item = 2 * Qp;
    a.in_item_stride = a.out_item_stride = per;
    a.iepi.on = 1; a.iepi.limbs = Q; a.iepi.add_parts = add_parts; a.iepi.p_mod = Q; a.iepi.galois_elt = galois_elt;
    a.iepi.half = c.h64("half")[0]; a.iepi.half_mod = c.d64("half_mod"); a.iepi.inv = c.d64("last_q_modinv");
    a.iepi.ct = ct; a.iepi.ct_item_stride = cs;
    a.iepi.out = out; a.iepi.out_item_stride = so;
    return ntt_launch(a, 2 * Qp * batch, true, st);
}

static hipError_t bfv_intt_moddown_multi(const Context& c, u64* acc, u64* scratch, u64 per, const u64* ct, u64 cs,
                                         int add_parts, u64* out, u64 so, int galois_elt, int batch, hipStream_t st)
{
    const u64 n = c.n;
    const int Q = c.Q_size, Qp = c.Qp_size, P = c.P_size;
    for (int part = 0; part < 2; part++) {
        NttArgs a = c.ntt_args(0);
        a.in = a.out = acc + (u64) (part * Qp + Q) * n;
        a.mod_count = P; a.mod_offset = Q; a.polys_per_item = P;
        a.in_item_stride = a.out_item_stride = per;
        TRY(ntt_launch(a, P * batch, true, st));
    }
    TRY(rns_moddown_multi_stage_one(acc, per, scratch, per, c.plan_qp.mods, c.d64("half"), c.d64("half_mod"),
                                    c.d64("last_q_modinv"), c.d64("m2_md_G"), c.d64("m2_md_C"), c.n_power, Qp, Q, Qp, Q, P,
                                    batch, st));
    NttArgs a = c.ntt_args(0);
    a.in = a.out = acc; a.mod_count = Qp; a.polys_per_item = 2 * Qp;
    a.in_item_stride = a.out_item_stride = per;
    a.iepi.on = 1; a.iepi.limbs = Q; a.iepi.p_count = P; a.iepi.add_parts = add_parts; a.iepi.p_mod = Q;
    a.iepi.galois_elt = galois_elt;
    a.iepi.inv = c.d64("m2_md_W0");
    a.iepi.u = scratch; a.iepi.u_item_stride = per;
    a.iepi.ct = ct; a.iepi.ct_item_stride = cs;
    a.iepi.out = out; a.iepi.out_item_stride = so;
    return ntt_launch(a, 2 * Qp * batch, true, st);
}
// ... 375 lines not shown
```

Before: 7988.

## Fuse CKKS keyswitch moddown tail into row MAC kernel

Splits the fused row-MAC so the special-prime slot runs first. Its inverse NTT and the moddown forward column NTT then run, and the remaining Q slots finish the row NTT, subtract the moddown term, scale by q_last inverse, add the ciphertext and optionally apply a Galois permutation inside the MAC kernel. This removes a separate moddown row-NTT/epilogue pass and the round trip of accumulator data through global memory. In exchange it launches two MAC kernels, which adds a launch and more register pressure at occupancy 1, and it only applies when P_size==1 and digit splitting is off.

```diff
diff --git a/heongpu_amd/csrc/cabi.cpp b/heongpu_amd/csrc/cabi.cpp
--- a/heongpu_amd/csrc/cabi.cpp
+++ b/heongpu_amd/csrc/cabi.cpp
@@ -290,6 +290,7 @@
         c.single_pass = s.single_pass; c.ntt_galois = s.ntt_galois; c.galois_scatter = s.galois_scatter;
         c.digit_split = s.digit_split; c.copy_along = s.copy_along; c.fuse_inverse = s.fuse_inverse;
         c.fp_ntt = s.fp_ntt; c.behz_split = s.behz_split; c.fused_tensor = s.fused_tensor;
+        c.moddown_in_mac = s.moddown_in_mac;
         *out = h;
         return 0;
     });
diff --git a/heongpu_amd/csrc/context.cpp b/heongpu_amd/csrc/context.cpp
--- a/heongpu_amd/csrc/context.cpp
+++ b/heongpu_amd/csrc/context.cpp
@@ -712,6 +712,7 @@
     {"fuse_inverse", "HEGPU_FUSE_INVERSE", 0, 1},    {"copy_along", "HEGPU_COPY_ALONG", 0, 1},
     {"digit_split", "HEGPU_DIGIT_SPLIT", -1, 4},     {"fp_ntt", "HEGPU_FP_NTT", 0, 1},
     {"behz_split", "HEGPU_BEHZ_SPLIT", -1, 1},       {"fused_tensor", "HEGPU_FUSED_TENSOR", 0, 1},
+    {"moddown_in_mac", "HEGPU_MODDOWN_IN_MAC", 0, 1},
 };
 }
 
@@ -736,6 +737,7 @@
     else if (nm == "fuse_inverse") fuse_inverse = value != 0;
     else if (nm == "copy_along") copy_along = value != 0;
     else if (nm == "fused_tensor") fused_tensor = value != 0;
+    else if (nm == "moddown_in_mac") moddown_in_mac = value != 0;
     else if (nm == "digit_split") {
         if (value == 1 || value == 3) return 2;
         digit_split = value;
@@ -760,6 +762,7 @@
     else if (nm == "fuse_inverse") *value = fuse_inverse;
     else if (nm == "copy_along") *value = copy_along;
     else if (nm == "fused_tensor") *value = fused_tensor;
+    else if (nm == "moddown_in_mac") *value = moddown_in_mac;
     else if (nm == "digit_split") *value = digit_split;
     else if (nm == "behz_split") *value = behz_split;
     else return 1;
diff --git a/heongpu_amd/csrc/context.hpp b/heongpu_amd/csrc/context.hpp
--- a/heongpu_amd/csrc/context.hpp
+++ b/heongpu_amd/csrc/context.hpp
@@ -56,6 +56,7 @@
     int digit_split = -1;
     bool copy_along = true;
     bool fuse_inverse = true;
+    bool moddown_in_mac = true;
     bool fused_tensor = true;
     bool fp_ntt = true;
     int behz_split = -1;
diff --git a/heongpu_amd/csrc/ntt.hip b/heongpu_amd/csrc/ntt.hip
--- a/heongpu_amd/csrc/ntt.hip
+++ b/heongpu_amd/csrc/ntt.hip
@@ -341,6 +341,7 @@
     u64 slot = a.poly_order ? (u64) a.poly_order[j] : (u64) j;
     s.digit = a.decomp_mods ? udiv16(j, a.mg_decomp_mods) : -1;
     u64 in_slot = a.decomp_mods ? (u64) s.digit * (a.decomp_in_mul ? a.decomp_in_mul : 1) + a.decomp_in_add : slot;
+    if (a.decomp_out_mul) slot = (u64) s.digit * a.decomp_out_mul + (u64) (j - s.digit * a.decomp_mods);
     s.in_off = (u64) item * a.in_item_stride + (in_slot << a.n_power);
     s.out_off = (u64) item * a.out_item_stride + (slot << a.n_power);
     s.item = item;
@@ -941,8 +942,9 @@
 struct KsIdx { int item, tile, slot; bool valid; int d0, d1; };
 __host__ __device__ __forceinline__ unsigned ks_slots(const KsMacArgs& a, int kind)
 {
-    if (a.int_slot_count <= 0 || kind == 0) return (unsigned) a.rc;
-    return kind == 1 ? (unsigned) a.int_slot_count : (unsigned) (a.rc - a.int_slot_count);
+    const int all = a.slot_count ? a.slot_count : a.rc;
+    if (a.int_slot_count <= 0 || kind == 0) return (unsigned) all;
+    return kind == 1 ? (unsigned) a.int_slot_count : (unsigned) (all - a.int_slot_count);
 }
 template <bool SPLIT, int KIND = 0>
 __device__ __forceinline__ KsIdx ks_index(const KsMacArgs& a)
@@ -963,10 +965,13 @@
     int si = (int) (g - gt * nslots);
     if (KIND == 1 && a.int_slot_count > 0) {
         si = a.int_slots[r.valid ? si : 0];
-    } else if (KIND == 2 && a.int_slot_count > 0) {
-#pragma unroll
-        for (int q = 0; q < 8; q++)
-            if (q < a.int_slot_count && a.int_slots[q] <= si) si++;
+    } else {
+        si += a.slot_first;
+        if (KIND == 2 && a.int_slot_count > 0) {
+#pragma unroll
+            for (int q = 0; q < 8; q++)
+                if (q < a.int_slot_count && a.int_slots[q] <= si) si++;
+        }
     }
     r.slot = si;
     r.d0 = SPLIT ? (int) (sp * (unsigned) a.digits / splits) : 0;
@@ -974,8 +979,46 @@
     return r;
 }
 
+__device__ __forceinline__ void ks_tail_store(const KsMacArgs& a, int item, int slot, int p, u64 e0, const Mod& md, u64 inv,
+                                              const u64 (&acc)[16], const u64 (&tv)[16], bool with_ct, const u64 (&cv)[16])
+{
+    const KsMacArgs::Tail& e = a.tail;
+    u64* out = e.out + e.out_item_stride * item + ((u64) (p * e.limbs + slot) << a.n_power);
+    u64 r[16];
+#pragma unroll
+    for (int k = 0; k < 16; k++) r[k] = mul_barrett(sub_mod(acc[k], tv[k], md.q), inv, md);
+    if (with_ct) {
+#pragma unroll
+        for (int k = 0; k < 16; k++) r[k] = add_mod(cv[k], r[k], md.q);
+    }
+    if (e.galois_inv) {
+#pragma unroll
+        for (int k = 0; k < 16; k++) {
+            const u32 el = (u32) e0 + 16 * k;
+            const u32 ex = ((2u * (__brev(el) >> (32 - a.n_power)) + 1u) * e.galois_inv) & ((2u << a.n_power) - 1u);
+            out[__brev((ex - 1u) >> 1) >> (32 - a.n_power)] = r[k];
+        }
+    } else {
+#pragma unroll
+        for (int k = 0; k < 16; k++) out[e0 + 16 * k] = r[k];
+    }
+}
+__device__ __forceinline__ const u64* ks_tail_T(const KsMacArgs& a, int item, int slot, int tile, int p)
+{
+    return a.tail.T + a.tail.T_item_stride * item + ((u64) (p * a.rc + slot) << a.n_power) + (u64) tile * 4096;
+}
+__device__ __forceinline__ bool ks_tail_ct(const KsMacArgs& a, int item, int slot, int p, u64 e0, u64 (&cv)[16])
+{
+    const KsMacArgs::Tail& e = a.tail;
+    if (!e.ct || (e.ct_parts && p >= e.ct_parts)) return false;
+    const u64* c = e.ct + e.ct_item_stride * item + ((u64) (p * e.limbs + slot) << a.n_power) + e0;
+#pragma unroll
+    for (int k = 0; k < 16; k++) cv[k] = c[16 * k];
+    return true;
+}
+
 #define KS_TW_LDS_BYTES ((15 * 256 + 15 * 16) * 8)
-template <bool SPLIT>
+template <bool SPLIT, bool MD = false>
 __device__ __forceinline__ void ks_row_mac_int_body(const KsMacArgs& a, const KsIdx& ki, const Mod& md, int midx,
                                                     u64* lds, void* twbuf)
 {
@@ -1000,6 +1043,8 @@
     }
     wave_lds_fence();
 
+    const int item_s = MD ? __builtin_amdgcn_readfirstlane(item) : 0, slot_s = MD ? __builtin_amdgcn_readfirstlane(slot) : 0;
+    const int tile_s = MD ? __builtin_amdgcn_readfirstlane(tile) : 0, midx_s = MD ? __builtin_amdgcn_readfirstlane(midx) : 0;
     u64 h0[16], l0[16], h1[16], l1[16];
 #pragma unroll
     for (int k = 0; k < 16; k++) h0[k] = l0[k] = h1[k] = l1[k] = 0;
@@ -1022,6 +1067,39 @@
             acc128(h0[k], l0[k], x[k], k0[16 * k]);
             acc128(h1[k], l1[k], x[k], k1[16 * k]);
         }
+    }
+    if constexpr (MD) {
+        u64 acc0[16], acc1[16];
+#pragma unroll
+        for (int k = 0; k < 16; k++) {
+            acc0[k] = reduce128(h0[k], l0[k], md);
+            acc1[k] = reduce128(h1[k], l1[k], md);
+        }
+        int tt = threadIdx.x;
+        asm volatile("" : "+v"(tt));
+        const int trow = tt >> 4, ti0 = tt & 15;
+        const u64 e0 = (u64) tile_s * 4096 + trow * 256 + ti0;
+        const u64 inv = a.tail.inv[midx_s];
+        const bool lazy_t = row_stages_lazy(md, a.lazy_q_max);
+        const ulonglong2* __restrict__ ttb = a.twB + ((u64) midx_s * (15u << (a.n_power - 4))) + ((u64) (tile_s * 16 + trow) * 15 * 16 + ti0);
+        auto part = [&](int p, const u64 (&acc)[16]) {
+            u64 cv[16], x[16];
+            const bool with_ct = ks_tail_ct(a, item_s, slot_s, p, e0, cv);
+            const u64* pT = ks_tail_T(a, item_s, slot_s, tile_s, p);
+            if (lazy_t) {
+                ks_row_digit<true>(x, pT, lds, twa, ttb, qc, md, trow, ti0);
+#pragma unroll
+                for (int k = 0; k < 16; k++) x[k] = reduce64(x[k], md);
+            } else {
+                ks_row_digit<false>(x, pT, lds, twa, ttb, qc, md, trow, ti0);
+            }
+            ks_tail_store(a, item_s, slot_s, p, e0, md, inv, acc, x, with_ct, cv);
+        };
+        __builtin_amdgcn_sched_barrier(0);
+        part(0, acc0);
+        __builtin_amdgcn_sched_barrier(0);
+        part(1, acc1);
+        return;
     }
     u64* po = (SPLIT ? const_cast<u64*>(pin) + dig_off * ki.d0 - (u64) tile * 4096
                      : a.out + a.out_item_stride * item + ((u64) slot << a.n_power)) +
@@ -1048,6 +1126,129 @@
 }
 
 template <bool SPLIT>
+__device__ __forceinline__ void ks_fp_row(double (&x)[16], const u64 (&xr)[16], const double* twl, u64* lds, const FC& fc,
+                                          int s1, int row, int i0, int t)
+{
+    if constexpr (SPLIT) {
+#pragma unroll
+        for (int k = 0; k < 16; k++) x[k] = as_f64(xr[k]);
+#pragma unroll
+        for (int s = 0; s < 4; s++) {
+            const int half = 8 >> s;
+            FP_STAGE(fc, s1 + s);
+#pragma unroll
+            for (int b = 0; b < (1 << s); b++) {
+                const double w = twl[15 * 256 + ((1 << s) - 1 + b) * 16 + row];
+                const ulonglong2 wp = make_ulonglong2(as_bits(w), as_bits(w * fc.qi));
+#pragma unroll
+                for (int j = 0; j < half; j++) fp_ct_bfly(x[b * 2 * half + j], x[b * 2 * half + j + half], wp, fc);
+            }
+        }
+        FP_STAGE(fc, s1 + 4);
+#pragma unroll
+        for (int k = 0; k < 16; k++) x[k] = fp_reduce(x[k], fc);
+#pragma unroll
+        for (int k = 0; k < 16; k++) lds[row_phys(row * 256 + i0 + 16 * k)] = as_bits(x[k]);
+        wave_lds_fence();
+#pragma unroll
+        for (int k = 0; k < 8; k++) {
+            ulonglong2 v = *reinterpret_cast<const ulonglong2*>(&lds[row_phys(row * 256 + 16 * i0 + 2 * k)]);
+            x[2 * k] = as_f64(v.x);
+            x[2 * k + 1] = as_f64(v.y);
+        }
+#pragma unroll
+        for (int s = 0; s < 4; s++) {
+            const int half = 8 >> s;
+            FP_STAGE(fc, s1 + 4 + s);
+#pragma unroll
+            for (int b = 0; b < (1 << s); b++) {
+                const double wd = twl[((1 << s) - 1 + b) * 256 + t];
+                const ulonglong2 w = make_ulonglong2(as_bits(wd), as_bits(wd * fc.qi));
+#pragma unroll
+                for (int j = 0; j < half; j++) fp_ct_bfly(x[b * 2 * half + j], x[b * 2 * half + j + half], w, fc);
+            }
+        }
+    } else {
+        int row_o = row, t_o = t;
+        asm volatile("" : "+v"(row_o), "+v"(t_o));
+        const double* twa = twl + 15 * 256 + row_o;
+        const double* twb = twl + t_o;
+        double wn[8], wc[8];
+        wc[0] = twa[0];
+        wn[0] = twa[16];
+        wn[1] = twa[32];
+        __builtin_amdgcn_sched_barrier(0);
+#pragma unroll
+        for (int k = 0; k < 16; k++) x[k] = as_f64(xr[k]);
+#pragma unroll
+        for (int s = 0; s < 4; s++) {
+            const int half = 8 >> s;
+            FP_STAGE(fc, s1 + s);
+            if (s > 0) {
+#pragma unroll
+                for (int b = 0; b < (1 << s); b++) wc[b] = wn[b];
+            }
+            if (s < 3) {
+                if (s > 0) {
+#pragma unroll
+                    for (int b = 0; b < (2 << s); b++) wn[b] = twa[((2 << s) - 1 + b) * 16];
+                }
+            } else {
+                wn[0] = twb[0];
+            }
+            __builtin_amdgcn_sched_barrier(0);
+#pragma unroll
+            for (int b = 0; b < (1 << s); b++) {
+                const double w = wc[b];
+                const ulonglong2 wp = make_ulonglong2(as_bits(w), as_bits(w * fc.qi));
+#pragma unroll
+                for (int j = 0; j < half; j++) fp_ct_bfly(x[b * 2 * half + j], x[b * 2 * half + j + half], wp, fc);
+            }
+        }
+        FP_STAGE(fc, s1 + 4);
+#pragma unroll
+        for (int k = 0; k < 16; k++) x[k] = fp_reduce(x[k], fc);
+#pragma unroll
+        for (int k = 0; k < 16; k++) lds[row_phys(row * 256 + i0 + 16 * k)] = as_bits(x[k]);
+        wave_lds_fence();
+#pragma unroll
+        for (int k = 0; k < 8; k++) {
+            ulonglong2 v = *reinterpret_cast<const ulonglong2*>(&lds[row_phys(row * 256 + 16 * i0 + 2 * k)]);
+            x[2 * k] = as_f64(v.x);
+            x[2 * k + 1] = as_f64(v.y);
+        }
+#pragma unroll
+        for (int s = 0; s < 4; s++) {
+            const int half = 8 >> s;
+            FP_STAGE(fc, s1 + 4 + s);
+#pragma unroll
+            for (int b = 0; b < (1 << s); b++) wc[b] = wn[b];
+            if (s < 3) {
+#pragma unroll
+                for (int b = 0; b < (2 << s); b++) wn[b] = twb[((2 << s) - 1 + b) * 256];
+            }
+            __builtin_amdgcn_sched_barrier(0);
+#pragma unroll
+            for (int b = 0; b < (1 << s); b++) {
+                const double wd = wc[b];
+                const ulonglong2 w = make_ulonglong2(as_bits(wd), as_bits(wd * fc.qi));
+#pragma unroll
+                for (int j = 0; j < half; j++) fp_ct_bfly(x[b * 2 * half + j], x[b * 2 * half + j + half], w, fc);
+            }
+        }
+    }
+    wave_lds_fence();
+#pragma unroll
+    for (int k = 0; k < 8; k++)
+        *reinterpret_cast<ulonglong2*>(&lds[row_phys(row * 256 + 16 * i0 + 2 * k)]) =
+            make_ulonglong2(as_bits(x[2 * k]), as_bits(x[2 * k + 1]));
+    wave_lds_fence();
+#pragma unroll
+    for (int k = 0; k < 16; k++) x[k] = as_f64(lds[row_phys(row * 256 + i0 + 16 * k)]);
+    wave_lds_fence();
+}
+
+template <bool SPLIT, bool MD = false>
 __device__ __forceinline__ void ks_row_mac_fp_body(const KsMacArgs& a, const KsIdx& ki, const Mod& md, int midx,
                                                    u64* lds, void* twbuf)
 {
@@ -1074,6 +1275,8 @@
     }
     wave_lds_fence();
 
+    const int item_s = MD ? __builtin_amdgcn_readfirstlane(item) : 0, slot_s = MD ? __builtin_amdgcn_readfirstlane(slot) : 0;
+    const int tile_s = MD ? __builtin_amdgcn_readfirstlane(tile) : 0, midx_s = MD ? __builtin_amdgcn_readfirstlane(midx) : 0;
     double a0[16], a1[16];
 #pragma unroll
     for (int k = 0; k < 16; k++) a0[k] = a1[k] = 0.0;
@@ -1102,123 +1305,7 @@
 #pragma unroll
             for (int k = 0; k < 16; k++) x[k] = fp_reduce(fp_from_u64(xr[k]), fc);
         } else {
-            if constexpr (SPLIT) {
-#pragma unroll
-                for (int k = 0; k < 16; k++) x[k] = as_f64(xr[k]);
-#pragma unroll
-                for (int s = 0; s < 4; s++) {
-                    const int half = 8 >> s;
-                    FP_STAGE(fc, s1 + s);
-#pragma unroll
-                    for (int b = 0; b < (1 << s); b++) {
-                        const double w = twl[15 * 256 + ((1 << s) - 1 + b) * 16 + row];
-                        const ulonglong2 wp = make_ulonglong2(as_bits(w), as_bits(w * fc.qi));
-#pragma unroll
-                        for (int j = 0; j < half; j++) fp_ct_bfly(x[b * 2 * half + j], x[b * 2 * half + j + half], wp, fc);
-                    }
-                }
-                FP_STAGE(fc, s1 + 4);
-#pragma unroll
-                for (int k = 0; k < 16; k++) x[k] = fp_reduce(x[k], fc);
-#pragma unroll
-                for (int k = 0; k < 16; k++) lds[row_phys(row * 256 + i0 + 16 * k)] = as_bits(x[k]);
-                wave_lds_fence();
-#pragma unroll
-                for (int k = 0; k < 8; k++) {
-                    ulonglong2 v = *reinterpret_cast<const ulonglong2*>(&lds[row_phys(row * 256 + 16 * i0 + 2 * k)]);
-                    x[2 * k] = as_f64(v.x);
-                    x[2 * k + 1] = as_f64(v.y);
-                }
-#pragma unroll
-                for (int s = 0; s < 4; s++) {
-                    const int half = 8 >> s;
-                    FP_STAGE(fc, s1 + 4 + s);
-#pragma unroll
-                    for (int b = 0; b < (1 << s); b++) {
-                        const double wd = twl[((1 << s) - 1 + b) * 256 + t];
-                        const ulonglong2 w = make_ulonglong2(as_bits(wd), as_bits(wd * fc.qi));
-#pragma unroll
-                        for (int j = 0; j < half; j++) fp_ct_bfly(x[b * 2 * half + j], x[b * 2 * half + j + half], w, fc);
-                    }
-                }
-            } else {
-                int row_o = row, t_o = t;
-                asm volatile("" : "+v"(row_o), "+v"(t_o));
-                const double* twa = twl + 15 * 256 + row_o;
-                const double* twb = twl + t_o;
-                double wn[8], wc[8];
-                wc[0] = twa[0];
-                wn[0] = twa[16];
-                wn[1] = twa[32];
-                __builtin_amdgcn_sched_barrier(0);
-#pragma unroll
-                for (int k = 0; k < 16; k++) x[k] = as_f64(xr[k]);
-#pragma unroll
-                for (int s = 0; s < 4; s++) {
-                    const int half = 8 >> s;
-                    FP_STAGE(fc, s1 + s);
-                    if (s > 0) {
-#pragma unroll
-                        for (int b = 0; b < (1 << s); b++) wc[b] = wn[b];
-                    }
-                    if (s < 3) {
-                        if (s > 0) {
-#pragma unroll
-                            for (int b = 0; b < (2 << s); b++) wn[b] = twa[((2 << s) - 1 + b) * 16];
-                        }
-                    } else {
-                        wn[0] = twb[0];
-                    }
-                    __builtin_amdgcn_sched_barrier(0);
-#pragma unroll
-                    for (int b = 0; b < (1 << s); b++) {
-                        const double w = wc[b];
-                        const ulonglong2 wp = make_ulonglong2(as_bits(w), as_bits(w * fc.qi));
-#pragma unroll
-                        for (int j = 0; j < half; j++) fp_ct_bfly(x[b * 2 * half + j], x[b * 2 * half + j + half], wp, fc);
-                    }
-                }
-                FP_STAGE(fc, s1 + 4);
-#pragma unroll
-                for (int k = 0; k < 16; k++) x[k] = fp_reduce(x[k], fc);
-#pragma unroll
-                for (int k = 0; k < 16; k++) lds[row_phys(row * 256 + i0 + 16 * k)] = as_bits(x[k]);
-                wave_lds_fence();
-#pragma unroll
-                for (int k = 0; k < 8; k++) {
-                    ulonglong2 v = *reinterpret_cast<const ulonglong2*>(&lds[row_phys(row * 256 + 16 * i0 + 2 * k)]);
-                    x[2 * k] = as_f64(v.x);
-                    x[2 * k + 1] = as_f64(v.y);
-                }
-#pragma unroll
-                for (int s = 0; s < 4; s++) {
-                    const int half = 8 >> s;
-                    FP_STAGE(fc, s1 + 4 + s);
-#pragma unroll
-                    for (int b = 0; b < (1 << s); b++) wc[b] = wn[b];
-                    if (s < 3) {
-#pragma unroll
-                        for (int b = 0; b < (2 << s); b++) wn[b] = twb[((2 << s) - 1 + b) * 256];
-                    }
-                    __builtin_amdgcn_sched_barrier(0);
-#pragma unroll
-                    for (int b = 0; b < (1 << s); b++) {
-                        const double wd = wc[b];
-                        const ulonglong2 w = make_ulonglong2(as_bits(wd), as_bits(wd * fc.qi));
-#pragma unroll
-                        for (int j = 0; j < half; j++) fp_ct_bfly(x[b * 2 * half + j], x[b * 2 * half + j + half], w, fc);
-                    }
-                }
-            }
-            wave_lds_fence();
-#pragma unroll
-            for (int k = 0; k < 8; k++)
-                *reinterpret_cast<ulonglong2*>(&lds[row_phys(row * 256 + 16 * i0 + 2 * k)]) =
-                    make_ulonglong2(as_bits(x[2 * k]), as_bits(x[2 * k + 1]));
-            wave_lds_fence();
-#pragma unroll
-            for (int k = 0; k < 16; k++) x[k] = as_f64(lds[row_phys(row * 256 + i0 + 16 * k)]);
-            wave_lds_fence();
+            ks_fp_row<SPLIT>(x, xr, twl, lds, fc, s1, row, i0, t);
         }
 #pragma unroll
         for (int k = 0; k < 16; k++) {
@@ -1240,6 +1327,36 @@
             }
         }
     }
+    if constexpr (MD) {
+        int tt = threadIdx.x;
+        asm volatile("" : "+v"(tt));
+        const int trow = tt >> 4, ti0 = tt & 15;
+        const u64 e0 = (u64) tile_s * 4096 + trow * 256 + ti0;
+        const Mod mds = a.mods[midx_s];
+        const u64 inv = a.tail.inv[midx_s];
+        auto part = [&](int p, const double (&acc)[16]) {
+            const u64* pT = ks_tail_T(a, item_s, slot_s, tile_s, p);
+            u64 tr[16], cv[16];
+#pragma unroll
+            for (int k = 0; k < 16; k++) tr[k] = __builtin_nontemporal_load(&pT[trow * 256 + ti0 + 16 * k]);
+            const bool with_ct = ks_tail_ct(a, item_s, slot_s, p, e0, cv);
+            double x[16];
+            ks_fp_row<false>(x, tr, twl, lds, fc, s1, trow, ti0, tt);
+            FP_STAGE(fc, FP_STAGE_OUT);
+            u64 av[16], tv[16];
+#pragma unroll
+            for (int k = 0; k < 16; k++) {
+                av[k] = fp_to_u64(fp_canon(acc[k], fc));
+                tv[k] = fp_to_u64(fp_canon(x[k], fc));
+            }
+            ks_tail_store(a, item_s, slot_s, p, e0, mds, inv, av, tv, with_ct, cv);
+        };
+        __builtin_amdgcn_sched_barrier(0);
+        part(0, a0);
+        __builtin_amdgcn_sched_barrier(0);
+        part(1, a1);
+        return;
+    }
     u64* po = (SPLIT ? const_cast<u64*>(pin) + dig_off * ki.d0 - (u64) tile * 4096
                      : a.out + a.out_item_stride * item + ((u64) slot << a.n_power)) +
               (u64) tile * 4096 + row * 256 + i0;
@@ -1269,6 +1386,29 @@
     ks_row_mac_fp_body<SPLIT>(a, ki, md, midx, lds, twl);
 }
 
+__global__ __launch_bounds__(NTT_THREADS) void ks_row_mac_fp_moddown(KsMacArgs a)
+{
+    __shared__ __attribute__((aligned(16))) u64 lds[ROW_LDS_ELEMS];
+    __shared__ double twl[15 * 256 + 15 * 16];
+    const KsIdx ki = ks_index<false, 2>(a);
+    if (!ki.valid) return;
+    const int midx = a.mod_order ? a.mod_order[ki.slot] : ki.slot;
+    const Mod md = a.mods[midx];
+    if (!md.fp) return;
+    ks_row_mac_fp_body<false, true>(a, ki, md, midx, lds, twl);
+}
+__global__ __launch_bounds__(NTT_THREADS, 1) void ks_row_mac_moddown(KsMacArgs a)
+{
+    __shared__ __attribute__((aligned(16))) u64 lds[ROW_LDS_ELEMS];
+    __shared__ ulonglong2 twa[15 * 16];
+    const KsIdx ki = ks_index<false, 1>(a);
+    if (!ki.valid) return;
+    const int midx = a.mod_order ? a.mod_order[ki.slot] : ki.slot;
+    const Mod md = a.mods[midx];
+    if (md.fp) return;
+    ks_row_mac_int_body<false, true>(a, ki, md, midx, lds, twa);
+}
+
 __global__ __launch_bounds__(NTT_THREADS, 2) void ks_row_mac_split(KsMacArgs a)
 {
     __shared__ __attribute__((aligned(16))) u64 lds[ROW_LDS_ELEMS];
@@ -1285,6 +1425,9 @@
 {
     if (a.digits > 64 || items <= 0) return hipErrorInvalidValue;
     if (a.splits > 1 && a.digits < 2 * a.splits) return hipErrorInvalidValue;
+    if (a.tail.on && (a.splits > 1 || !a.tail.out || !a.tail.T || !a.tail.inv)) return hipErrorInvalidValue;
+    if (a.slot_first < 0 || a.slot_count < 0 || a.slot_first + (a.slot_count ? a.slot_count : a.rc) > a.rc)
+        return hipErrorInvalidValue;
     KsMacArgs k = a;
     k.items = items;
     if (k.int_slot_count < 0 || k.int_slot_count > 8) k.int_slot_count = 0;
@@ -1293,10 +1436,14 @@
     if (a.splits > 1) {
         hipLaunchKernelGGL(ks_row_mac_split, grid_of(0), dim3(NTT_THREADS), 0, st, k);
     } else {
-        if (!a.no_fp && ks_slots(k, 2) > 0)
-            hipLaunchKernelGGL(ks_row_mac_fp<false>, grid_of(2), dim3(NTT_THREADS), 0, st, k);
-        if (!a.no_int && ks_slots(k, 1) > 0)
-            hipLaunchKernelGGL(ks_row_mac<false>, grid_of(1), dim3(NTT_THREADS), 0, st, k);
+        if (!a.no_fp && ks_slots(k, 2) > 0) {
+            if (a.tail.on) hipLaunchKernelGGL(ks_row_mac_fp_moddown, grid_of(2), dim3(NTT_THREADS), 0, st, k);
+            else hipLaunchKernelGGL(ks_row_mac_fp<false>, grid_of(2), dim3(NTT_THREADS), 0, st, k);
+        }
+        if (!a.no_int && ks_slots(k, 1) > 0) {
+            if (a.tail.on) hipLaunchKernelGGL(ks_row_mac_moddown, grid_of(1), dim3(NTT_THREADS), 0, st, k);
+            else hipLaunchKernelGGL(ks_row_mac<false>, grid_of(1), dim3(NTT_THREADS), 0, st, k);
+        }
     }
     return hipGetLastError();
 }
@@ -1766,7 +1913,8 @@
         ps.item = item;
         ps.j = digit * rc + k;
         ps.in_off = 0;
-        ps.out_off = (u64) item * a.out_item_stride + ((u64) ps.j << a.n_power);
+        ps.out_off = (u64) item * a.out_item_stride +
+                     ((u64) (a.decomp_out_mul ? digit * a.decomp_out_mul + k : ps.j) << a.n_power);
         if (a.skip_identity && ps.mod == digit) continue;
         const Mod md = ld_const_mod(a.mods + ps.mod);
         if (!md.fp) continue;
diff --git a/heongpu_amd/csrc/ntt.hpp b/heongpu_amd/csrc/ntt.hpp
--- a/heongpu_amd/csrc/ntt.hpp
+++ b/heongpu_amd/csrc/ntt.hpp
@@ -64,6 +64,7 @@
     NttEpilogue epi;
     NttInvEpilogue iepi;
     int decomp_in_mul, decomp_in_add;
+    int decomp_out_mul;
     int half_on, half_src_mod;
     u64 half;
     const u64* half_mod;
@@ -112,6 +113,20 @@
     int no_fp, no_int;
     int int_slot_count;
     int int_slots[8];
+    int slot_first, slot_count;
+    struct Tail {
+        int on;
+        const u64* T;
+        u64 T_item_stride;
+        const u64* ct;
+        u64 ct_item_stride;
+        int ct_parts;
+        unsigned galois_inv;
+        u64* out;
+        u64 out_item_stride;
+        const u64* inv;
+        int limbs;
+    } tail;
 };
 hipError_t ks_row_mac_launch(const KsMacArgs& a, int items, hipStream_t st);
 
diff --git a/heongpu_amd/csrc/ops.cpp b/heongpu_amd/csrc/ops.cpp
--- a/heongpu_amd/csrc/ops.cpp
+++ b/heongpu_amd/csrc/ops.cpp
@@ -35,6 +35,11 @@
 {
     if (c.fused_row_mac >= 0) return c.fused_row_mac != 0;
     return (long) batch * rc * (long) (c.n >> 12) >= fused_row_mac_need(c);
+}
+static bool use_moddown_in_mac(const Context& c, const u64* key, int l, int rc, int batch)
+{
+    return c.moddown_in_mac && c.fused_moddown && key && c.P_size == 1 && use_fused_row_mac(c, rc, batch) &&
+           !fused_digit_splits(c, rc, l, batch) && (long) 2 * l * batch <= 65535;
 }
 
 static void fill_int_slots(const Context& c, NttArgs& a, const u64* order)
@@ -52,13 +57,15 @@
 
 static hipError_t keyswitch_ntt_mac(const Context& c, NttArgs a, const u64* key, u64* acc, u64 acc_stride,
                                     int digits, int rc, int split, int level, const u64* ident, u64 ident_stride,
-                                    int batch, hipStream_t st, int which = 3)
+                                    int batch, hipStream_t st, int which = 3, int slot_first = 0, int slot_count = 0,
+                                    const KsMacArgs::Tail* tail = nullptr)
 {
     const int ppi = digits * rc;
     const int skip_identity = ident ? 1 : 0;
     a.skip_identity = skip_identity;
     const int splits = fused_digit_splits(c, rc, digits, batch);
     if (!splits && !use_fused_row_mac(c, rc, batch)) {
+        if (slot_count || tail) return hipErrorInvalidValue;
         if (ident && c.fused_row_mac == 0)
             TRY(rns_copy_diag(ident, ident_stride, a.out, a.out_item_stride, c.n_power, digits, rc, batch, st));
         else a.skip_identity = 0;
@@ -86,6 +93,21 @@
         k.no_int = !a.plan_has_int || a.int_slot_count < 0;
         k.int_slot_count = a.int_slot_count > 0 ? a.int_slot_count : 0;
         for (int q = 0; q < 8; q++) k.int_slots[q] = a.int_slots[q];
+        k.slot_first = slot_first; k.slot_count = slot_count;
+        if (slot_count && a.int_slot_count > 0) {
+            int cnt = 0;
+            for (int q = 0; q < a.int_slot_count; q++)
+                if (a.int_slots[q] >= slot_first && a.int_slots[q] < slot_first + slot_count) k.int_slots[cnt++] = a.int_slots[q];
+            k.int_slot_count = cnt;
+            k.no_int = cnt == 0;
+            k.no_fp = k.no_fp || cnt == slot_count;
+        }
+        if (tail) {
+            k.tail = *tail;
+            k.tail.T += (u64) b0 * tail->T_item_stride;
+            if (tail->ct) k.tail.ct += (u64) b0 * tail->ct_item_stride;
+            k.tail.out += (u64) b0 * tail->out_item_stride;
+        }
         TRY(ks_row_mac_launch(k, nb, st));
         if (splits > 1)
             TRY(rns_sum_partials(ca.out, a.out_item_stride, k.out, acc_stride, c.plan_qp.mods, a.mod_order, c.n_power,
@@ -160,7 +182,11 @@
     dgt.single_decomp_ok = 1;
     a = dgt;
     const int which = ((phases & RELIN_PHASE_COLUMN) ? 1 : 0) | ((phases & RELIN_PHASE_ROW_MAC) ? 2 : 0);
-    if (which) TRY(keyswitch_ntt_mac(c, a, key, temp2, per, l, rc, l, depth, src, src_stride, batch, st, which));
+    const bool in_mac = use_moddown_in_mac(c, key, l, rc, batch);
+    if (which)
+        TRY(keyswitch_ntt_mac(c, a, key, temp2, per, l, rc, l, depth, src, src_stride, batch, st, which, in_mac ? l : 0,
+                              in_mac ? 1 : 0));
+    const NttArgs dgt_args = a;
     a = c.ntt_args(0);
     a.in = temp2; a.out = temp2; a.mod_count = 1; a.mod_offset = Q; a.polys_per_item = 2;
     a.in_item_stride = a.out_item_stride = per;
@@ -176,6 +202,25 @@
     if (phases & RELIN_PHASE_INTT_P) {
         if (fuse_inv_p) TRY(ntt_launch_inv_rows(a, 2 * batch, st));
         else TRY(ntt_launch(a, 2 * batch, true, st));
+    }
+    if (in_mac) {
+        if (phases & RELIN_PHASE_MODDOWN) {
+            a = md;
+            a.out = temp2; a.decomp_out_mul = l + 1;
+            a.half = c.h64("half")[0]; a.half_mod = c.d64("half_mod");
+            a.src_inv = fuse_inv_p ? 1 : 0;
+            TRY(ntt_launch_fwd_col(a, 2 * l * batch, st));
+        }
+        if (!(phases & RELIN_PHASE_ROW_MAC)) return hipSuccess;
+        KsMacArgs::Tail t{};
+        t.on = 1;
+        t.T = temp2; t.T_item_stride = per;
+        t.ct = add; t.ct_item_stride = add_stride; t.ct_parts = add_parts;
+        t.out = outp; t.out_item_stride = out_stride;
+        t.inv = c.d64("last_q_modinv");
+        t.limbs = l;
+        t.galois_inv = galois_elt ? (unsigned) inv_mod_2n((u64) galois_elt, 2 * c.n) : 0u;
+        return keyswitch_ntt_mac(c, dgt_args, key, temp2, per, l, rc, l, depth, src, src_stride, batch, st, 2, 0, l, &t);
     }
     if (!(phases & RELIN_PHASE_MODDOWN)) return hipSuccess;
     if (!c.fused_moddown)
```

Measured after the change: 8330 (median of 6 runs). +4.3%, better.
